# baurst/liso

Hardware: AMD Instinct MI355X
Metric: LISO train-step frames/sec (120k-pt clouds) (higher is better)
Workload: dtype bf16 (detector, BASELINE configs[2]) + f32 via bf16x3 MFMA (SLIM); north_star's 1e-3 on logits / flow is met by `parity_leg` (f32 via bf16x3 MFMA everywhere) and `fp32_exact_leg`, not by the bf16 detector

## Files before the change

include/liso_conv.h:

```cpp
#ifndef LISO_CONV_H
#define LISO_CONV_H

#include <stddef.h>
#include <stdint.h>

#ifdef __cplusplus
extern "C" {
#endif

#define LISO_CONV_MAX_TAPS 49
#define LISO_CONV_MAX_CLASSES 4
#define LISO_CONV_BF16 0
#define LISO_CONV_F32X3 1
#define LISO_CONV_F32 2
#define LISO_CONV_F16 3

#define LISO_ELEM_F32 0
#define LISO_ELEM_BF16 1
#define LISO_ELEM_F16 2

typedef struct {
    int batch, hi, wi, ci;
    int x_pix_stride;
    int ho, wo, co;
    int y_pix_stride, y_ch_off;
    int hv, wv;
    int isy, isx, osy, osx;
    int n_classes;
    int class_tap_begin[LISO_CONV_MAX_CLASSES + 1];
    int class_ooy[LISO_CONV_MAX_CLASSES], class_oox[LISO_CONV_MAX_CLASSES];
    int n_taps;
    int tap_dy[LISO_CONV_MAX_TAPS], tap_dx[LISO_CONV_MAX_TAPS];
    int tap_w[LISO_CONV_MAX_TAPS];
    int w_taps;
    int mode;
    int out_f32;
    int in_relu, out_relu;
    int in_affine_batch_stride;
    int wgrad_co;
} liso_conv_desc;

size_t liso_conv_packed_bytes(int k_channels, int n_channels, int taps, int mode);
int liso_conv_pack_weights(const float* src, int d0, int d1, int kh, int kw, int transposed, int for_dgrad, int mode,
                           void* dst, void* stream);

typedef struct {
    const float* src;
    void* dst;
    int d0, d1, kh, kw, transposed, for_dgrad, mode;
} liso_conv_pack_job;
int liso_conv_pack_weights_batched(const liso_conv_pack_job* jobs, int n_jobs, void* stream);

int liso_conv_stats_rows(const liso_conv_desc* d);

int liso_conv_kernel_kind(const liso_conv_desc* d);

int liso_conv_plan_info(const liso_conv_desc* d, int info[8]);

int liso_conv_forward(const liso_conv_desc* d, const void* x, const void* w_packed, const float* bias,
                      const float* in_scale, const float* in_shift, void* y, float* stats_partial,
                      const float* stats_shift, void* stream);

int liso_conv_forward_sparse(const liso_conv_desc* d, const void* x, const void* w_packed, const float* bias,
                             const float* in_scale, const float* in_shift, void* y, float* stats_partial,
                             const float* stats_shift, const float* occupancy, void* stream);

size_t liso_conv_wgrad_sparse_workspace_bytes(const liso_conv_desc* d);
int liso_conv_wgrad_sparse_f32(const liso_conv_desc* d, const float* x, const float* occupancy, const float* dy, int dy_pix_stride,
                               float* dw, float* dbias, void* workspace, size_t workspace_bytes, void* stream);

size_t liso_conv_wgrad_smallci_workspace_bytes(int batch, int h, int w, int co, int k);
int liso_conv_wgrad_smallci_f32(const float* x, long x_pix_stride, const float* dy, long dy_pix_stride, int batch, int h, int w, int co,
                                int k, float* dw, float* dbias, void* workspace, size_t workspace_bytes, void* stream);

size_t liso_conv_wgrad_workspace_bytes(const liso_conv_desc* d);
int liso_conv_wgrad(const liso_conv_desc* d, const void* x, const float* in_scale, const float* in_shift, const void* dy,
                    int dy_pix_stride, int transposed, float* dw, float* dbias, void* workspace, size_t workspace_bytes,
                    void* stream);

int liso_conv_bn_finalize(const float* stats_partial, int rows, int co, int co_pad, long n, const float* stats_shift,
                          const float* gamma, const float* beta, float* running_mean, float* running_var, float momentum,
                          float eps, float* stats, void* stream);

int liso_conv_in_finalize(const float* stats_partial, int rows_per_sample, int batch, int co, int co_pad, long n_per_sample,
                          const float* gamma, const float* beta, float eps, float* stats, void* stream);

int liso_residual_affine_relu_f32(const float* a, const float* a_scale, const float* a_shift, int a_stride, int a_relu, const float* b,
                                  const float* b_scale, const float* b_shift, int b_stride, int b_relu, float* out, int batch,
                                  long pixels, int c, void* stream);

#define LISO_CONV_OPT_SHARED_GPU 1
#define LISO_CONV_OPT_ROLES_CUS 2
int liso_conv_set_option(int option, int value);

int liso_sparse_conv_stat_groups(int hi, int wi, int co);
size_t liso_sparse_conv_workspace_bytes(int batch, int hi, int wi, int k, int co, int max_cells_per_sample, int for_dgrad);
int liso_sparse_conv_forward(const void* x, long x_pix_stride, int is_bf16, const float* occupancy, const void* w_packed,
                             const float* bias, int batch, int hi, int wi, int k, int co, int max_cells_per_sample, int relu, void* y,
                             float* stats_partial, const float* stats_shift, int* overflow, void* workspace, size_t workspace_bytes,
                             void* stream);
int liso_sparse_conv_dgrad(const void* dy, long dy_pix_stride, int is_bf16, const float* occupancy, const void* w_packed_dgrad, int batch,
                           int hi, int wi, int k, int co, int max_cells_per_sample, void* dx, long dx_pix_stride, int* overflow,
                           void* workspace, size_t workspace_bytes, int reuse_lists, void* stream);
size_t liso_sparse_stem_workspace_bytes(int batch, int hi, int wi, int max_cells_per_sample);
int liso_sparse_stem_forward_f32(const float* x, long x_pix_stride, const float* occupancy, const void* w_packed, const float* bias,
                                 int batch, int hi, int wi, int max_cells_per_sample, int relu, float* y, float* stats_partial,
                                 int* overflow, void* workspace, size_t workspace_bytes, void* stream);

#ifdef __cplusplus
}
#endif
#endif
```

liso_amd/_lib.py:

```python
import ctypes
import os

import torch

_HERE = os.path.dirname(os.path.abspath(__file__))
LIB_PATH = os.path.join(_HERE, "libliso_hip.so")

_lib = None


class LisoHipError(RuntimeError):
    pass


_ERRORS = {-1: "LISO_EINVAL (bad pointer/size)", -2: "LISO_EWORKSPACE (workspace too small)",
           -3: "LISO_ELAUNCH (HIP launch failed)"}


def _preload_torch_hip_runtime():
    tl = os.path.join(os.path.dirname(torch.__file__), "lib", "libamdhip64.so")
    if os.path.exists(tl):
        ctypes.CDLL(tl, mode=ctypes.RTLD_GLOBAL)


# ... 60 lines not shown

    def rows_view(t):
        assert t.dtype == torch.float32 and t.is_cuda
        if t.dim() == 1:
            assert t.stride(0) == 1 or t.numel() <= 1
            return 1, t.numel(), t.numel()
        inner = 1
        for k in range(t.dim() - 1, 0, -1):
            assert t.shape[k] == 1 or t.stride(k) == inner, (tuple(t.shape), t.stride())
            inner *= t.shape[k]
        return t.shape[0], inner, (t.stride(0) if t.shape[0] > 1 else inner)

    for i, (d, s_) in enumerate(jobs):
        assert tuple(d.shape) == tuple(s_.shape), (tuple(d.shape), tuple(s_.shape))
        r, c, dstr = rows_view(d)
        r2, c2, sstr = rows_view(s_)
        assert (r, c) == (r2, c2)
        dst[i], src[i], rows[i], rb[i], ds[i], ss[i] = d.data_ptr(), s_.data_ptr(), r, 4 * c, 4 * dstr, 4 * sstr
    with torch.cuda.device(jobs[0][0].device):
        check(lib().liso_multi_copy_rows(n, dst, src, rows, rb, ds, ss, stream_ptr()), "multi_copy_rows")


def require_cuda(*tensors):
    for t in tensors:
        if not t.is_cuda:
            raise LisoHipError("device op called with a CPU tensor; liso_amd has no CPU fallback")


_vp, _i, _f, _sz, _lg = ctypes.c_void_p, ctypes.c_int, ctypes.c_float, ctypes.c_size_t, ctypes.c_long

SIGNATURES = {
    "liso_iou3d_overlap_bev_f32": (_i, [_vp, _i, _vp, _i, _vp, _vp]),
    "liso_iou3d_iou_bev_f32": (_i, [_vp, _i, _vp, _i, _vp, _vp]),
    "liso_iou3d_nms_workspace_bytes": (_sz, [_i]),
    "liso_iou3d_nms_f32": (_i, [_vp, _i, _f, _vp, _vp, _vp, _sz, _vp]),
    "liso_iou3d_nms_normal_f32": (_i, [_vp, _i, _f, _vp, _vp, _vp, _sz, _vp]),
    "liso_iou3d_iou_bev_cpu_f32": (_i, [_vp, _i, _vp, _i, _vp]),
    "liso_pillars_voxelize_workspace_bytes": (_sz, [_vp, _i, _i]),
    "liso_pillars_voxelize_f32": (_i, [_vp, _vp, _i, _vp, _vp, _vp, _vp, _vp, _vp, _vp, _sz, _vp]),
    "liso_pfn_partials_bytes": (_sz, []),
    "liso_pfn_decorate_workspace_bytes": (_sz, [_i, _i]),
    "liso_pfn_decorate_f32": (_i, [_vp, _vp, _i, _vp, _vp, _vp, _vp, _vp, _vp, _vp, _vp, _sz, _vp]),
    "liso_pfn_bn_prepare_f32": (_i, [_vp, _vp, _vp, _i, _vp, _vp, _vp, _vp, _vp, _vp, _f, _f, _i, _vp, _vp, _vp, _vp]),
    "liso_pfn_forward_scatter": (_i, [_vp, _vp, _vp, _vp, _i, _vp, _vp, _vp, _vp, _i, _vp, _vp]),
    "liso_pfn_backward": (_i, [_vp, _vp, _vp, _vp, _i, _vp, _vp, _vp, _vp, _vp, _i, _vp, _i, _vp, _vp, _vp, _vp, _vp]),
    "liso_kabsch_workspace_bytes": (_sz, [_vp]),
    "liso_kabsch_trafos_f32": (_i, [_vp, _vp, _vp, _vp, _vp, _vp, _vp, _vp, _vp, _vp, _vp, _sz, _vp]),
    "liso_kabsch_trafos_counted_f32": (_i, [_vp, _vp, _vp, _vp, _vp, _vp, _vp, _vp, _vp, _vp, _vp, _vp, _sz, _vp]),
    "liso_symm_ortho_fwd_f64": (_i, [_vp, _i, _vp, _vp, _vp, _vp, _vp]),
    "liso_symm_ortho_bwd_f64": (_i, [_vp, _vp, _vp, _vp, _i, _vp, _vp]),
    "liso_weighted_moments_workspace_bytes": (_sz, [_i]),
    "liso_weighted_moments_fwd_f32": (_i, [_vp, _vp, _vp, _i, ctypes.c_long, _vp, _vp, _sz, _vp]),
    "liso_weighted_moments_bwd_f32": (_i, [_vp, _vp, _vp, _i, ctypes.c_long, _vp, _vp, _vp, _vp, _vp]),
    "liso_bev_dynamic_flow_workspace_bytes": (_sz, [_i, _i, _i]),
    "liso_bev_dynamic_flow_f32": (_i, [_vp, _i, _vp, _vp, _vp, _i, _vp, _i, _i, _i, _i, _vp, _vp, _vp, _sz, _vp]),
    "liso_odom_inverse_minus_eye_f64": (_i, [_vp, _i, _vp, _vp]),
    "liso_fit_box_z_workspace_bytes": (_sz, [_i, _i]),
    "liso_fit_box_z_f32": (_i, [_vp, _i, _i, _vp, _i, _vp, _i, _vp, _i, _f, _vp, _vp, _vp, _vp, _sz, _vp]),
    "liso_dbscan_components": (_i, [_vp, _vp, _vp, _vp, _vp, _vp, _vp, _vp, _vp]),
    "liso_dbscan_labels": (_i, [_vp, _vp, _vp, _vp, _vp, _vp, _vp, _vp, _vp, _vp]),
    "liso_region_props": (_i, [_vp, _i, _i, _i, _i, _vp, _vp, _vp]),
    "liso_region_props_workspace_bytes": (_sz, [_i, _i, _i, _i]),
    "liso_region_props_ws": (_i, [_vp, _i, _i, _i, _i, _vp, _vp, _vp, _sz, _vp]),
    "liso_corr_lookup_fwd_f32": (_i, [_vp, _vp, _vp, _vp, _vp, _vp]),
    "liso_corr_lookup_fwd_tiled_f32": (_i, [_vp, _vp, _vp, _vp, _vp, _vp]),
    "liso_corr_lookup_bwd_dvol_f32": (_i, [_vp, _vp, _vp, _vp, _vp]),
    "liso_corr_pyramid_fwd_f32": (_i, [_vp, _vp, _vp, _vp]),
    "liso_corr_pyramid_bwd_f32": (_i, [_vp, _vp, _vp, _vp]),
    "liso_corr_bwd_features_workspace_bytes": (_sz, [_vp]),
    "liso_corr_bwd_features_f32": (_i, [_vp, _i, _vp, _vp, _vp, _vp, _vp, _vp, _sz, _vp]),
    "liso_rows_combine_f32": (_i, [_lg, _i, _vp, _lg, _vp, _lg, _vp, _lg, _vp, _lg, _vp, _lg, _i, _vp]),
    "liso_gru_out_rows_train_f32": (_i, [_lg, _i, _vp, _lg, _vp, _vp, _lg, _vp, _lg, _vp]),
    "liso_gru_out_rows_bwd_f32": (_i, [_lg, _i, _vp, _lg, _vp, _vp, _lg, _vp, _lg, _vp, _lg, _vp, _vp, _vp]),
    "liso_gru_in_rows_bwd_f32": (_i, [_lg, _i, _vp, _lg, _vp, _lg, _vp, _vp, _vp, _lg, _vp, _lg, _vp, _vp]),
    "liso_raft_state_step_train_f32": (_i, [_i, _i, _vp, _vp, _vp, _vp, _vp, _vp, _vp, _vp, _vp]),
    "liso_raft_pack_output_grads_f32": (_i, [_lg, _i, _vp, _vp, _vp, _vp]),
    "liso_nearest_point_loss_fwd_f32": (_i, [_vp] * 8),
    "liso_nearest_point_loss_bwd_f32": (_i, [_vp] * 9),
    "liso_slim_decode_weights_fwd": (_i, [_vp] * 6 + [_i] + [_vp] * 4),
    "liso_slim_decode_weights_bwd": (_i, [_vp] * 9),
    "liso_slim_decode_points_fwd": (_i, [_vp] * 9),
    "liso_slim_decode_points_bwd": (_i, [_vp] * 11),
    "liso_slim_loss_workspace_bytes": (_sz, []),
    "liso_slim_static_points_loss_fwd": (_i, [_i, ctypes.c_long, _vp, _i, _vp, _vp, _vp, _vp, _vp, _vp, _sz, _vp]),
    "liso_slim_static_points_loss_bwd": (_i, [_i, ctypes.c_long, _vp, _i, _vp, _vp, _vp, _vp, _vp, _vp, _vp, _vp, _vp]),
    "liso_slim_knn_queries": (_i, [_i, _i, ctypes.c_long, _i, _vp, _i, _vp, _vp, _vp, _vp, _vp]),
    "liso_slim_nearest_point_loss_fwd": (_i, [_vp, _vp, _i, _vp, _vp, _vp, _i, _vp, _vp, _vp, _vp, _vp, _sz, _vp]),
    "liso_slim_nearest_point_loss_bwd": (_i, [_vp, _vp, _i, _vp, _vp, _vp, _i, _vp, _vp, _vp, _vp, _vp, _vp, _vp]),
    "liso_bev_gather_fwd_f32": (_i, [_vp, _vp, ctypes.c_long, _i, ctypes.c_float, _vp, _vp]),
    "liso_bev_gather_bwd_f32": (_i, [_vp, _vp, _vp, _vp, ctypes.c_long, _i, _vp, _vp, _vp]),
    "liso_gru_in_fwd_f32": (_i, [_vp, _vp, _vp, ctypes.c_long, _vp, _vp, _vp, _vp, _vp]),
    "liso_gru_in_bwd_f32": (_i, [_vp, _vp, ctypes.c_long, _vp, _vp, _vp, _vp, _vp, _vp, ctypes.c_long, _vp, _vp]),
    "liso_gru_out_fwd_f32": (_i, [ctypes.c_long, _vp, _vp, _vp, _vp, _vp]),
    "liso_gru_out_bwd_f32": (_i, [ctypes.c_long, _vp, _vp, _vp, _vp, _vp, _vp, _vp, _vp]),
    "liso_gru_in_rows_f32": (_i, [ctypes.c_long, _i, _vp, ctypes.c_long, _vp, ctypes.c_long, _vp, _vp, ctypes.c_long, _vp]),
    "liso_gru_out_rows_f32": (_i, [ctypes.c_long, _i, _vp, ctypes.c_long, _vp, _vp, ctypes.c_long, _vp]),
    "liso_multi_copy": (_i, [_i, _vp, _vp, _vp, _vp]),
    "liso_bev_lin_index": (_i, [_vp, _i, _vp, _i, ctypes.c_long, _i, _i, _vp, _vp]),
    "liso_channel_extrema_workspace_bytes": (_sz, []),
    "liso_channel_extrema_f32": (_i, [_vp, ctypes.c_long, _i, _i, _vp, _vp, _sz, _vp]),
    "liso_bev_plan_tile_lin": (_i, [_vp, _i, ctypes.c_long, _i, _i, _i, _i, _vp, _vp]),
    "liso_bev_plan_rank": (_i, [_vp, _vp, ctypes.c_long, _vp, _vp, _vp]),
    "liso_bev_plan_expand": (_i, [_vp, _vp, _vp, _i, ctypes.c_long, _i, _i, _i, _i, _vp, _vp, _vp, _vp]),
    "liso_raft_state_step_f32": (_i, [_i, _i, _vp, ctypes.c_long, _vp, _vp, _vp, _vp]),
    "liso_raft_upsample_scratch_bytes": (_sz, [_vp]),
    "liso_raft_upsample_outputs_fwd_f32": (_i, [_vp] * 5),
    "liso_raft_upsample_outputs_bwd_f32": (_i, [_vp, _vp, _vp, _sz, _vp, _vp, _vp]),
    "liso_centerloss_workspace_bytes": (_sz, [_vp]),
    "liso_centerloss_fwd_f32": (_i, [_vp] * 17 + [_sz, _vp]),
    "liso_centerloss_bwd_f32": (_i, [_vp] * 21),
    "liso_render_center_targets_f32": (_i, [_vp] * 12),
    "liso_conv_pack_weights_batched": (_i, [_vp, _i, _vp]),
    "liso_conv_in_finalize": (_i, [_vp, _i, _i, _i, _i, ctypes.c_long, _vp, _vp, _f, _vp, _vp]),
    "liso_residual_affine_relu_f32": (_i, [_vp, _vp, _vp, _i, _i, _vp, _vp, _vp, _i, _i, _vp, _i, ctypes.c_long, _i, _vp]),
    "liso_scan_workspace_bytes": (_sz, [_i, ctypes.c_long]),
    "liso_scan_inclusive_i32": (_i, [_vp, _i, ctypes.c_long, _vp, _vp, _sz, _vp]),
    "liso_mine_boxes_from_regions": (_i, [_vp, _i, _i, _vp, _i, _vp, _i, _f, _f, _vp, _vp, _vp, _vp, _vp, _vp]),
    "liso_mine_filter_compact": (_i, [_vp] * 21),
    "liso_mine_box_motion": (_i, [_vp, _i, _i, _vp, _vp, _vp, _vp]),
    "liso_mine_nms_workspace_bytes": (_sz, [_i, _i]),
    "liso_mine_nms_prepare": (_i, [_i, _i, _i] + [_vp] * 11 + [_sz, _vp]),
    "liso_mine_nms_finish": (_i, [_i, _i, _i] + [_vp] * 16),
    "liso_adamw_step_f32": (_i, [_vp, _vp, _vp, _vp, _sz] + [ctypes.c_double] * 5 + [ctypes.c_long, _vp]),
    "liso_adamw_step_scaled_f32": (_i, [_vp, _vp, _vp, _vp, _sz] + [ctypes.c_double] * 6 + [ctypes.c_long, _vp]),
    "liso_grad_nonfinite_f32": (_i, [_vp, _sz, _vp, _vp]),
    "liso_adamw_step_amp_f32": (_i, [_vp, _vp, _vp, _vp, _sz] + [ctypes.c_double] * 6 + [_vp, _vp]),
    "liso_loss_scale_update": (_i, [_vp, ctypes.c_double, ctypes.c_double, _i, _vp]),
    "liso_rmsprop_step_f32": (_i, [_vp, _vp, _vp, _sz] + [ctypes.c_double] * 4 + [_vp]),
    "liso_multi_copy_rows": (_i, [_i, _vp, _vp, _vp, _vp, _vp, _vp, _vp]),
    "liso_gather_f32": (_i, [_i, _vp, _vp, _vp, _vp]),
    "liso_bn_workspace_bytes": (_sz, [_i]),
    "liso_bn_relu_fwd": (_i, [_vp, _i, ctypes.c_long, _i, _vp, _vp, _vp, _vp, _f, _f, _i, _i, _vp, _vp, _vp, _sz, _vp]),
    "liso_in_workspace_bytes": (_sz, [_i, _i]),
    "liso_in_relu_fwd": (_i, [_vp, _i, _i, ctypes.c_long, _i, _vp, _vp, _f, _i, _vp, _vp, _vp, _sz, _vp]),
    "liso_in_relu_bwd": (_i, [_vp, _vp, _i, _i, ctypes.c_long, _i, _vp, _vp, _i, _vp, _vp, _vp, _vp, _sz, _vp]),
    "liso_in_relu_bwd_sum": (_i, [_vp, _vp, _i, _i, ctypes.c_long, _i, _vp, _vp, _i, _vp, _vp, _vp, _vp, _sz, _vp]),
    "liso_bn_relu_bwd": (_i, [_vp, _vp, _i, ctypes.c_long, _i, _vp, _vp, _i, _i, _vp, _vp, _vp, _vp, _sz, _vp]),
    "liso_bn_relu_bwd_strided": (_i, [_vp, ctypes.c_long, _vp, ctypes.c_long, _i, ctypes.c_long, _i, _vp, _vp, _i, _i, _vp, ctypes.c_long, _vp, _vp, _vp, _sz, _vp]),
    "liso_bn_relu_bwd_ticket": (_i, [_vp, _vp, _i, ctypes.c_long, _i, _vp, _vp, _i, _i, _vp, _vp, _vp, _vp, _sz, _vp, _vp]),
    "liso_knn_workspace_bytes": (_sz, [_vp, _i]),
    "liso_knn_build_f32": (_i, [_vp, _vp, _i, _i, _vp, _sz, _vp]),
    "liso_knn_sorted_ids": (_i, [_vp, _vp, _i, _vp, _vp]),
    "liso_knn_query_f32": (_i, [_vp, _vp, _vp, _vp, _i, _vp, _i, _i, _vp, _vp, _i, _vp]),
    "liso_conv_packed_bytes": (_sz, [_i, _i, _i, _i]),
    "liso_conv_pack_weights": (_i, [_vp, _i, _i, _i, _i, _i, _i, _i, _vp, _vp]),
    "liso_conv_stats_rows": (_i, [_vp]),
    "liso_conv_kernel_kind": (_i, [_vp]),
    "liso_conv_forward": (_i, [_vp] * 10),
    "liso_conv_set_option": (_i, [_i, _i]),
    "liso_conv_forward_sparse": (_i, [_vp] * 11),
    "liso_conv_plan_info": (_i, [_vp, _vp]),
    "liso_conv_wgrad_workspace_bytes": (_sz, [_vp]),
    "liso_conv_wgrad": (_i, [_vp, _vp, _vp, _vp, _vp, _i, _i, _vp, _vp, _vp, _sz, _vp]),
    "liso_conv_wgrad_sparse_workspace_bytes": (_sz, [_vp]),
    "liso_conv_wgrad_sparse_f32": (_i, [_vp, _vp, _vp, _vp, _i, _vp, _vp, _vp, _sz, _vp]),
    "liso_conv_wgrad_smallci_workspace_bytes": (_sz, [_i, _i, _i, _i, _i]),
    "liso_conv_wgrad_smallci_f32": (_i, [_vp, ctypes.c_long, _vp, ctypes.c_long, _i, _i, _i, _i, _i, _vp, _vp, _vp, _sz, _vp]),
    "liso_sparse_conv_stat_groups": (_i, [_i, _i, _i]),
    "liso_sparse_conv_workspace_bytes": (_sz, [_i, _i, _i, _i, _i, _i, _i]),
    "liso_sparse_conv_forward": (_i, [_vp, ctypes.c_long, _i, _vp, _vp, _vp, _i, _i, _i, _i, _i, _i, _i, _vp, _vp, _vp, _vp, _vp, _sz, _vp]),
    "liso_sparse_conv_dgrad": (_i, [_vp, ctypes.c_long, _i, _vp, _vp, _i, _i, _i, _i, _i, _i, _vp, ctypes.c_long, _vp, _vp, _sz, _i, _vp]),
    "liso_sparse_stem_workspace_bytes": (_sz, [_i, _i, _i, _i]),
    "liso_sparse_stem_forward_f32": (_i, [_vp, ctypes.c_long, _vp, _vp, _vp, _i, _i, _i, _i, _i, _vp, _vp, _vp, _vp, _sz, _vp]),
    "liso_conv_bn_finalize": (_i, [_vp, _i, _i, _i, ctypes.c_long, _vp, _vp, _vp, _vp, _vp, _f, _f, _vp, _vp]),
    "liso_points_in_boxes_workspace_bytes": (_sz, [_vp]),
    "liso_points_in_boxes_f32": (_i, [_vp] * 9 + [_sz, _vp]),
    "liso_match_greedy_f32": (_i, [_vp, ctypes.c_long, ctypes.c_long, _i, _i, _vp, _f, _vp, _vp, _vp, _vp, _vp, _vp, _vp]),
    "liso_fit_boxes_closeness_workspace_bytes": (_sz, [ctypes.c_long, _i]),
    "liso_fit_boxes_closeness_f32": (_i, [_vp, ctypes.c_long, _i, _vp, _vp, _i, _f, _vp, _vp, _vp, _sz, _vp]),
    "liso_bike_rollout_fwd_f32": (_i, [_i, _i, _vp, _vp, _vp, _vp, _f, _f, _f, _vp, _vp]),
    "liso_bike_rollout_bwd_f32": (_i, [_i, _i, _vp, _vp, _vp, _f, _f, _f, _vp, _vp, _vp, _vp, _vp, _vp]),
    "liso_smooth_tracks_jerk_f32": (_i, [_vp, _vp, _i, _i, _i, _f, _f, _vp, _vp]),
    "liso_flow_metrics_state_bytes": (_sz, []),
    "liso_flow_metrics_result_bytes": (_sz, []),
    "liso_flow_metrics_reset": (_i, [_vp, _vp]),
    "liso_flow_metrics_update": (_i, [_vp, _lg, _vp, _lg, _vp, _lg, _i, _vp, _lg, _vp, _lg, _vp, _lg, _vp, _vp, _vp, _vp, _i, _vp, _vp]),
    "liso_flow_metrics_read": (_i, [_vp, _vp, _vp]),
    "liso_bev_free_mask_workspace_bytes": (_sz, [_i, _i]),
    "liso_bev_free_mask": (_i, [_vp, ctypes.c_long, _i, _i, _i, _vp, _vp, _vp, _sz, _vp]),
    "liso_bev_select_free_cells": (_i, [_vp, _vp, _i, _i, _vp, _i, _vp, _vp]),
    "liso_snippet_paste": (_i, [_vp, ctypes.c_long, _vp, _vp, _vp, _vp, ctypes.c_double, ctypes.c_double, _i, _vp, _vp, _vp, _vp]),
}


CONV_MAX_TAPS, CONV_MAX_CLASSES, CONV_BF16, CONV_F32X3, CONV_F32, CONV_F16 = 49, 4, 0, 1, 2, 3
ELEM_F32, ELEM_BF16, ELEM_F16 = 0, 1, 2
_ELEM_CODES = {torch.float32: ELEM_F32, torch.bfloat16: ELEM_BF16, torch.float16: ELEM_F16}
LOSS_SCALE_STATE_BYTES = 32


def elem_code(dtype):
    code = _ELEM_CODES.get(dtype)
    if code is None:
        raise TypeError(f"no device kernel takes {dtype} tensors (float32, bfloat16 or float16)")
    return code


def is_half(dtype):
    return elem_code(dtype) != ELEM_F32
CONV_OPT_SHARED_GPU = 1
CONV_OPT_ROLES_CUS = 2


class ConvDesc(ctypes.Structure):
    _fields_ = [("batch", _i), ("hi", _i), ("wi", _i), ("ci", _i), ("x_pix_stride", _i), ("ho", _i), ("wo", _i), ("co", _i),
                ("y_pix_stride", _i), ("y_ch_off", _i), ("hv", _i), ("wv", _i), ("isy", _i), ("isx", _i), ("osy", _i), ("osx", _i),
                ("n_classes", _i), ("class_tap_begin", _i * (CONV_MAX_CLASSES + 1)), ("class_ooy", _i * CONV_MAX_CLASSES),
                ("class_oox", _i * CONV_MAX_CLASSES), ("n_taps", _i), ("tap_dy", _i * CONV_MAX_TAPS), ("tap_dx", _i * CONV_MAX_TAPS),
                ("tap_w", _i * CONV_MAX_TAPS), ("w_taps", _i), ("mode", _i), ("out_f32", _i), ("in_relu", _i), ("out_relu", _i),
                ("in_affine_batch_stride", _i), ("wgrad_co", _i)]


class ConvPackJob(ctypes.Structure):
    _fields_ = [("src", _vp), ("dst", _vp), ("d0", _i), ("d1", _i), ("kh", _i), ("kw", _i), ("transposed", _i), ("for_dgrad", _i),
                ("mode", _i)]


class KnnGrid(ctypes.Structure):
    _fields_ = [("x_min", _f), ("y_min", _f), ("cell", _f), ("nx", _i), ("ny", _i), ("z_min", _f), ("z_cell", _f), ("nz", _i)]


class CenterLossCfg(ctypes.Structure):
    _fields_ = [("batch", _i), ("h", _i), ("w", _i), ("res_x", _f), ("res_y", _f), ("z_min", _f), ("z_max", _f),
                ("sup_weight", _f), ("rot_reg_weight", _f)]


class NpLossCfg(ctypes.Structure):
    _fields_ = [("batch", _i), ("n", ctypes.c_long), ("n_b", ctypes.c_long), ("ext", _f * 4), ("fov_mode", _i), ("delta", _f)]


class SlimDecodeCfg(ctypes.Structure):
    _fields_ = [("samples", _i), ("n", ctypes.c_long), ("h", _i), ("w", _i), ("logit_mode", _i * 4), ("static_flow_zero", _i),
                ("dynamic_flow_zero", _i), ("overwrite_flow", _i), ("overwrite_logits", _i), ("non_rigid", _i), ("use_static_aggr", _i),
                ("dyn_grad_scale", _f), ("ext_lo", ctypes.c_double * 2), ("ext_span", ctypes.c_double * 2)]


class SlimDecodeOut(ctypes.Structure):
    FIELDS = ("dis_logit", "dis", "logits", "probs", "staticness", "dynamicness", "groundness", "dyn_flow", "stat_flow", "agg_flow", "saf_flow")
    _fields_ = [(k, _vp) for k in FIELDS] + [("flags", _vp)]


class SlimNpLossCfg(ctypes.Structure):
    _fields_ = [("samples", _i), ("clouds", _i), ("n", ctypes.c_long), ("n_b", ctypes.c_long), ("ext", _f * 4), ("fov_mode", _i), ("delta", _f)]


class BoxPtsCfg(ctypes.Structure):
    _fields_ = [("batch", _i), ("n", ctypes.c_long), ("k", _i), ("point_stride", _i), ("precision", _i), ("dims_bloat", _f)]


class GruCfg(ctypes.Structure):
    _fields_ = [("batch", _i), ("ch", _i), ("cx", _i), ("hw", ctypes.c_long)]


class UpsampleCfg(ctypes.Structure):
    _fields_ = [("n_it", _i), ("batch2", _i), ("dirs", _i), ("h", _i), ("w", _i), ("factor", _i), ("flow_scale", _f)]


class MineFilterCfg(ctypes.Structure):
    _fields_ = [("batch", _i), ("k", _i), ("min_points", _i), ("aspect_ratio_max", ctypes.c_double), ("max_box_len_m", ctypes.c_double),
                ("min_box_area_m2", ctypes.c_double), ("min_box_volume_m3", ctypes.c_double), ("park_invalid", _i)]


class TargetsCfg(ctypes.Structure):
    _fields_ = [("batch", _i), ("n_boxes", _i), ("h", _i), ("w", _i), ("range_x", _f), ("range_y", _f)]


class DbscanCfg(ctypes.Structure):
    _fields_ = [("batch", _i), ("gx", _i), ("gy", _i), ("window", _i), ("min_samples", _i), ("eps", _f), ("flow_weight", _f)]


class CorrCfg(ctypes.Structure):
    _fields_ = [("batch", _i), ("h", _i), ("w", _i), ("dim", _i), ("levels", _i), ("radius", _i)]


class KabschCfg(ctypes.Structure):
    _fields_ = [("batch", _i), ("n_points", _i), ("n_slots", _i), ("point_stride", _i), ("flow_stride", _i),
                ("slope", _f), ("scale_fg", _f), ("scale_bg", _f), ("softness", _i)]


class PillarCfg(ctypes.Structure):
    _fields_ = [("x_min", _f), ("y_min", _f), ("z_min", _f), ("vx", _f), ("vy", _f), ("vz", _f), ("gx", _i),
                ("gy", _i), ("max_points", _i), ("max_voxels", _i), ("n_channels", _i)]


class _Everything:
    def __contains__(self, name):
        return True


class KernelTimer:

    def __init__(self):
        self.enabled = set()
        self.events = {}
        self.units = {}
        self.bytes = {}
        self.weights = {}
        self.weight = 1.0

    def enable(self, name):
        self.enabled.add(name)
        self.events.setdefault(name, [])

    def enable_all(self):
        self.enabled = _Everything()

    def disable_all(self):
        self.enabled = set()

    def launch(self, name, fn, units=None, nbytes=None):
        if name not in self.enabled:
            return fn()
        a, b = torch.cuda.Event(enable_timing=True), torch.cuda.Event(enable_timing=True)
        a.record()
        r = fn()
        b.record()
        self.events.setdefault(name, []).append((a, b))
        self.weights.setdefault(name, []).append(float(self.weight))
        if units is not None:
            self.units.setdefault(name, []).append(units)
        if nbytes is not None:
            self.bytes.setdefault(name, []).append(nbytes)
        return r

    def mean_units(self, name):
        u = self.units.get(name, [])
        return sum(u) / len(u) if u else None

    def durations_ms(self, name):
        torch.cuda.synchronize()
        return [a.elapsed_time(b) for a, b in self.events.get(name, [])]

    def weighted_total_ms(self, name):
        return sum(d * w for d, w in zip(self.durations_ms(name), self.weights.get(name, [])))

    def reset(self):
        for k in self.events:
            self.events[k] = []
        self.units = {}
        self.bytes = {}
        self.weights = {}


TIMER = KernelTimer()


def _declare(l):
    for name, (res, args) in SIGNATURES.items():
        fn = getattr(l, name)
        fn.restype = res
        fn.argtypes = args
```

liso_amd/csrc/conv_wgrad.hip:

```cpp
#include <hip/hip_runtime.h>
#include <stdint.h>
#include <stdlib.h>

#include "../../include/liso_conv.h"
#include "../../include/liso_iou3d.h"
#include "elem16.h"
#include "per_device.h"

namespace {

typedef __bf16 bf8 __attribute__((ext_vector_type(8)));
typedef float f16v __attribute__((ext_vector_type(16)));
typedef short s4 __attribute__((ext_vector_type(4)));
typedef s4 __attribute__((address_space(3))) * lds_s4_ptr;

constexpr int kThreads = 256;
constexpr int TW = 32;
constexpr int CT = 64;
constexpr int PSB = CT * 2 + 64;
constexpr int PS32 = CT * 4 + 16;

struct WgArgs {
    const void* x;
    const float* in_scale;
    const float* in_shift;
    const void* dy;
    float* slab;
    float* bias_slab;
    int dy_pix_stride;
    int ci_t, co_t;
    int n_groups;
    int grp_cls[LISO_CONV_MAX_TAPS], grp_begin[LISO_CONV_MAX_TAPS], grp_cnt[LISO_CONV_MAX_TAPS];
    int cls_dy0[LISO_CONV_MAX_CLASSES], cls_dx0[LISO_CONV_MAX_CLASSES];
    int cls_inh[LISO_CONV_MAX_CLASSES], cls_inw[LISO_CONV_MAX_CLASSES];
    int tiles_x, tiles_y, n_tiles, splits;
    int x_plane_bytes;
    int psx;
    int th;
    int ci_w;
    int pipelined;
    int compact;
#ifdef LISO_WGRAD_STAMPS
    unsigned long long* stamps;
#endif
};

__device__ __forceinline__ unsigned pack_bf16(float a, float b) {
    const __bf16 x = (__bf16)a, y = (__bf16)b;
    return (unsigned)__builtin_bit_cast(unsigned short, x) | ((unsigned)__builtin_bit_cast(unsigned short, y) << 16);
}
__device__ __forceinline__ float bf16_lo(unsigned w) { return __uint_as_float(w << 16); }
__device__ __forceinline__ float bf16_hi(unsigned w) { return __uint_as_float(w & 0xffff0000u); }
__device__ __forceinline__ float round_bf16(float v) { return (float)(__bf16)v; }

__device__ __forceinline__ bf8 tr_pair(const unsigned char* p0, const unsigned char* p1) {
    const s4 a = __builtin_amdgcn_ds_read_tr16_b64_v4i16((lds_s4_ptr)p0);
    const s4 b = __builtin_amdgcn_ds_read_tr16_b64_v4i16((lds_s4_ptr)p1);
    typedef short s8 __attribute__((ext_vector_type(8)));
    const s8 v = {a[0], a[1], a[2], a[3], b[0], b[1], b[2], b[3]};
    return __builtin_bit_cast(bf8, v);
}

template <int MODE, int TG>
__global__ __launch_bounds__(kThreads, 2) void conv_wgrad_kernel(const liso_conv_desc d, const WgArgs a) {
    using E = typename liso_e16::Elem<MODE>::T;
    constexpr bool X3 = MODE == LISO_CONV_F32X3;
    constexpr bool F32 = MODE == LISO_CONV_F32;
    constexpr bool FIN = X3 || F32;
    constexpr int PLANES = X3 ? 2 : 1;
    constexpr int PSYM = F32 ? PS32 : PSB;
    constexpr int PSY = PSB;
    constexpr int XB = TG >= 9 ? 4 : 8;
    extern __shared__ __attribute__((aligned(16))) unsigned char smem[];
    const int tid = threadIdx.x, wave = tid >> 6, lane = tid & 63;
    int t = blockIdx.x;
    const int split = t % a.splits;
    t /= a.splits;
    const int cot = t % a.co_t;
    t /= a.co_t;
    const int cit = t % a.ci_t;
    const int grp = t / a.ci_t;
    const int cls = a.grp_cls[grp], tb = a.grp_begin[grp], tcnt = a.grp_cnt[grp];
    const int dy0 = a.cls_dy0[cls], dx0 = a.cls_dx0[cls], in_h = a.cls_inh[cls], in_w = a.cls_inw[cls];
    const int PSX = a.psx;
    const int npix = in_h * in_w;
    const float inv_w = 1.0f / (float)in_w;
    const int ooy = d.class_ooy[cls], oox = d.class_oox[cls];
    const int ci0 = cit * CT, co0 = cot * CT;

    unsigned char* xs = smem;
    unsigned char* ys = smem + a.x_plane_bytes * PLANES;
    const int TH = a.th, MPIX = TH * TW;
    const int y_plane = MPIX * PSYM;

    const int g = lane >> 4, q = (lane & 15) >> 2, p = lane & 3;
    const int ci_half = wave >> 1, co_half = wave & 1;
    const int a_lane = (8 * (g >> 1) + q) * d.isx * PSX + (ci_half * 32 + 16 * (g & 1) + 4 * p) * 2;
    const int b_lane = (8 * (g >> 1) + q) * PSY + (co_half * 32 + 16 * (g & 1) + 4 * p) * 2;

    f16v acc[TG];
#pragma unroll
    for (int i = 0; i < TG; i++)
#pragma unroll
        for (int e = 0; e < 16; e++) acc[i][e] = 0.0f;
    float bsum[8];
#pragma unroll
    for (int e = 0; e < 8; e++) bsum[e] = 0.0f;
    const bool want_bias = a.bias_slab != nullptr && cit == 0 && tb == d.class_tap_begin[cls];

    const int gdy = a.compact ? d.tap_dy[tb] - dy0 : 0;
    const int row_mul = a.compact ? d.isy : 1;
    const int row_step = a.compact ? 1 : d.isy;
    int toff[TG];
#pragma unroll
    for (int i = 0; i < TG; i++) {
        const int tp = tb + (i < tcnt ? i : 0);
        toff[i] = ((d.tap_dy[tp] - dy0 - gdy) * in_w + (d.tap_dx[tp] - dx0)) * PSX;
    }

    constexpr int YB = 4;
    const int c8 = tid & 7, p0 = tid >> 3, pstep = kThreads / 8;
    uint4 xv[XB], yv[YB];
    unsigned xok = 0u, yok = 0u;
    float sc[8], sh[8];
    const bool pro = !FIN && a.in_scale != nullptr;
    if constexpr (!FIN) {
        const int ch = ci0 + c8 * 8;
        if (pro) {
#pragma unroll
            for (int e = 0; e < 8; e++) {
                sc[e] = ch < d.ci ? a.in_scale[ch + e] : 0.0f;
                sh[e] = ch < d.ci ? a.in_shift[ch + e] : 0.0f;
            }
        }
    }
    auto tile_origin = [&](int tile, int& b, int& ty, int& tx) {
        tx = tile % a.tiles_x;
        tile /= a.tiles_x;
        ty = tile % a.tiles_y;
        b = tile / a.tiles_y;
    };
    auto load_x = [&](int tile, int pix_begin) {
        int b, ty, tx;
        tile_origin(tile, b, ty, tx);
        const int iy0 = ty * TH * d.isy + dy0, ix0 = tx * TW * d.isx + dx0;
        const int ch = ci0 + c8 * 8;
        const bool ch_ok = ch < d.ci;
        const unsigned short* xg = (const unsigned short*)a.x + (long)b * d.hi * d.wi * d.x_pix_stride;
        const int pfirst = pix_begin + p0;
        int ly = (int)(((float)pfirst + 0.5f) * inv_w);
        int lx = pfirst - ly * in_w;
        const int step_y = pstep / in_w, step_x = pstep - step_y * in_w;
        xok = 0u;
#pragma unroll
        for (int u = 0; u < XB; u++) {
// ... 152 lines not shown
    } else
    for (int tile = split; tile < a.n_tiles; tile += a.splits) {
        int tt = tile;
        const int tx = tt % a.tiles_x;
        tt /= a.tiles_x;
        const int ty = tt % a.tiles_y;
        const int b = tt / a.tiles_y;
        const int iy0 = ty * TH * d.isy + dy0, ix0 = tx * TW * d.isx + dx0;
        const long x_img = (long)b * d.hi * d.wi;
        const long y_img = (long)b * d.ho * d.wo * a.dy_pix_stride;
        __syncthreads();
        if constexpr (!FIN) {
            (void)iy0; (void)ix0; (void)x_img; (void)y_img;
            for (int pix0 = 0; pix0 < npix; pix0 += XB * pstep) {
                load_x(tile, pix0);
                store_x(pix0);
            }
            load_y(tile);
            store_y();
        } else {
            const int c4 = tid & 15, p0 = tid >> 4, pstep = kThreads / 16;
            const int ch = ci0 + c4 * 4;
            const bool ch_ok = ch < d.ci;
            const bool pro = a.in_scale != nullptr;
            float sc[4], sh[4];
            if (pro) {
#pragma unroll
                for (int e = 0; e < 4; e++) {
                    sc[e] = ch_ok ? a.in_scale[ch + e] : 0.0f;
                    sh[e] = ch_ok ? a.in_shift[ch + e] : 0.0f;
                }
            }
            const float* xg = (const float*)a.x + x_img * d.x_pix_stride;
            unsigned char* xs_lo = xs + a.x_plane_bytes;
            int ly = (int)(((float)p0 + 0.5f) * inv_w);
            int lx = p0 - ly * in_w;
            const int step_y = pstep / in_w, step_x = pstep - step_y * in_w;
            for (int pix0 = p0; pix0 < npix; pix0 += XB * pstep) {
                float4 v[XB];
                bool ok[XB];
#pragma unroll
                for (int u = 0; u < XB; u++) {
                    const int pix = pix0 + u * pstep;
                    const int iy = iy0 + gdy + ly * row_mul, ix = ix0 + lx;
                    ok[u] = pix < npix && ch_ok && (unsigned)iy < (unsigned)d.hi && (unsigned)ix < (unsigned)d.wi;
                    const int off = ok[u] ? (iy * d.wi + ix) * d.x_pix_stride + ch : 0;
                    lx += step_x;
                    ly += step_y;
                    if (lx >= in_w) {
                        lx -= in_w;
                        ly++;
                    }
                    v[u] = *reinterpret_cast<const float4*>(xg + off);
                }
#pragma unroll
                for (int u = 0; u < XB; u++) {
                    const int pix = pix0 + u * pstep;
                    if (pix >= npix) continue;
                    float f[4] = {v[u].x, v[u].y, v[u].z, v[u].w};
                    unsigned hi2[2], lo2[2];
#pragma unroll
                    for (int e = 0; e < 4; e++) {
                        if (pro) {
                            f[e] = fmaf(f[e], sc[e], sh[e]);
                            if (d.in_relu) f[e] = fmaxf(f[e], 0.0f);
                        }
                        if (!ok[u]) f[e] = 0.0f;
                    }
                    if constexpr (F32) {
                        *reinterpret_cast<float4*>(xs + pix * PSX + c4 * 16) = make_float4(f[0], f[1], f[2], f[3]);
                        continue;
                    }
#pragma unroll
                    for (int e = 0; e < 2; e++) {
                        const float h0 = round_bf16(f[2 * e]), h1 = round_bf16(f[2 * e + 1]);
                        hi2[e] = pack_bf16(h0, h1);
                        lo2[e] = pack_bf16(f[2 * e] - h0, f[2 * e + 1] - h1);
                    }
                    *reinterpret_cast<uint2*>(xs + pix * PSX + c4 * 8) = make_uint2(hi2[0], hi2[1]);
                    *reinterpret_cast<uint2*>(xs_lo + pix * PSX + c4 * 8) = make_uint2(lo2[0], lo2[1]);
                }
            }
            const float* yg = (const float*)a.dy;
            const int chy = co0 + c4 * 4;
            const bool chy_ok = chy < d.co;
            for (int u = 0; u < MPIX / (kThreads / 16); u++) {
                const int m = p0 + u * pstep;
                const int vy = ty * TH + (m >> 5), vx = tx * TW + (m & 31);
                const int oy = vy * d.osy + ooy, ox = vx * d.osx + oox;
                const bool ok = chy_ok && vy < d.hv && vx < d.wv && oy < d.ho && ox < d.wo;
                const int off = ok ? (oy * d.wo + ox) * a.dy_pix_stride + chy : 0;
                float4 v = *reinterpret_cast<const float4*>(yg + y_img + off);
                float f[4] = {v.x, v.y, v.z, v.w};
                unsigned hi2[2], lo2[2];
#pragma unroll
                for (int e = 0; e < 4; e++) {
                    if (!ok) f[e] = 0.0f;
                    if (want_bias) bsum[e] += f[e];
                }
                if constexpr (F32) {
                    *reinterpret_cast<float4*>(ys + m * PS32 + c4 * 16) = make_float4(f[0], f[1], f[2], f[3]);
                    continue;
                }
#pragma unroll
                for (int e = 0; e < 2; e++) {
                    const float h0 = round_bf16(f[2 * e]), h1 = round_bf16(f[2 * e + 1]);
                    hi2[e] = pack_bf16(h0, h1);
                    lo2[e] = pack_bf16(f[2 * e] - h0, f[2 * e + 1] - h1);
                }
                *reinterpret_cast<uint2*>(ys + m * PSY + c4 * 8) = make_uint2(hi2[0], hi2[1]);
                *reinterpret_cast<uint2*>(ys + y_plane + m * PSY + c4 * 8) = make_uint2(lo2[0], lo2[1]);
            }
        }
        __syncthreads();
        mfma_tile();
    }
    const int r = lane & 31, h = lane >> 5;
    const long cip = (long)a.ci_t * CT, cop = (long)a.co_t * CT;
#pragma unroll
    for (int i = 0; i < TG; i++) {
        if (i < tcnt) {
            const int wt = d.tap_w[tb + i];
            float* base = a.slab + (((long)split * d.w_taps + wt) * cip + ci0 + ci_half * 32) * cop + co0 + co_half * 32 + r;
            if (co0 + co_half * 32 + r < (d.wgrad_co > 0 ? d.wgrad_co : d.co)) {
                const int rows_left = d.ci - (ci0 + ci_half * 32);
#pragma unroll
                for (int e = 0; e < 16; e++) {
                    const int row = (e & 3) + 8 * (e >> 2) + 4 * h;
                    if (row < rows_left) base[(long)row * cop] = acc[i][e];
                }
            }
        }
    }
    if (want_bias) {
        __syncthreads();
        float* red = reinterpret_cast<float*>(smem);
        constexpr int NCH = FIN ? 4 : 8;
        constexpr int NGR = FIN ? 16 : 8;
#pragma unroll
        for (int e = 0; e < NCH; e++) red[tid * NCH + e] = bsum[e];
        __syncthreads();
        if (tid < CT) {
            const int grp_c = tid / NCH, e = tid % NCH;
            float s = 0.0f;
            for (int pp = 0; pp < kThreads / NGR; pp++) s += red[(pp * NGR + grp_c) * NCH + e];
            a.bias_slab[((long)cls * a.splits + split) * cop + co0 + tid] = s;
        }
    }
}

constexpr int kRsThreads = 512;
constexpr int RPS = 128;

template <int MODE, int TH, int S, int CIW>
__global__ __launch_bounds__(kRsThreads, 1) void conv_wgrad_rs3_kernel(const liso_conv_desc d, const WgArgs a) {
    using E = typename liso_e16::Elem<MODE>::T;
    constexpr bool X3 = MODE == LISO_CONV_F32X3;
    constexpr int PLANES = X3 ? 2 : 1;
    constexpr int IW = (TW - 1) * S + 3, IH = (TH - 1) * S + 3;
    constexpr int NPX = IH * IW;
    constexpr int NSLOT = (NPX + 3) / 4 * 4;
    constexpr int CPP = X3 ? 16 : 8;
    constexpr int PSL = 256 / CPP;
    constexpr int CPPX = CPP * CIW / 64;
    constexpr int PSLX = 256 / CPPX;
    constexpr int XB = (NPX + PSLX - 1) / PSLX;
    constexpr int YB = TH * TW / PSL;
    constexpr int X_PLANE = NSLOT * RPS, Y_PLANE = TH * TW * RPS;
    constexpr int X_BYTES = PLANES * X_PLANE;
    constexpr int BUF = X_BYTES + PLANES * Y_PLANE;
    constexpr int NE = X3 ? 4 : 8;
    extern __shared__ __attribute__((aligned(16))) unsigned char smem[];
    const int tid = threadIdx.x, wave = tid >> 6, lane = tid & 63;
    int t = blockIdx.x;
    const int split = t % a.splits;
    t /= a.splits;
    const int cot = t % a.co_t;
    const int cit = t / a.co_t;
    const int ci0 = cit * CIW, co0 = cot * CT;
    const long cip = (long)a.ci_t * CIW, cop = (long)a.co_t * CT;
    const int n_mine = split < a.n_tiles ? (a.n_tiles - split + a.splits - 1) / a.splits : 0;

    if (wave >= 4) {
        const int ltid = tid - 256;
        const int cc = ltid % CPP, p0 = ltid / CPP;
        const int ccx = ltid % CPPX, p0x = ltid / CPPX;
        uint4 xv[XB], yv[YB];
        unsigned xok = 0u, yok = 0u;
        float sc[NE], sh[NE];
        float bsum[NE];
#pragma unroll
        for (int e = 0; e < NE; e++) bsum[e] = 0.0f;
        const bool want_bias = a.bias_slab != nullptr && cit == 0;
        const bool pro = a.in_scale != nullptr;
        const int ch = ci0 + ccx * NE, chy = co0 + cc * NE;
        const bool ch_ok = ch < d.ci, chy_ok = chy < d.co;
        if (pro) {
#pragma unroll
            for (int e = 0; e < NE; e++) {
                sc[e] = ch_ok ? a.in_scale[ch + e] : 0.0f;
                sh[e] = ch_ok ? a.in_shift[ch + e] : 0.0f;
            }
        }
        int rel[XB];
        unsigned lyx[XB];
#pragma unroll
        for (int u = 0; u < XB; u++) {
            const int pix = p0x + u * PSLX;
            const int ly = pix / IW, lx = pix - ly * IW;
            rel[u] = (ly * d.wi + lx) * d.x_pix_stride;
            lyx[u] = (unsigned)ly | ((unsigned)lx << 8) | (pix < NPX && ch_ok ? 0x10000u : 0u);
        }
        auto load_tile = [&](int tile) {
            const int tx = tile % a.tiles_x;
            const int tq = tile / a.tiles_x;
            const int ty = tq % a.tiles_y, b = tq / a.tiles_y;
            const int iy0 = ty * TH * S - 1, ix0 = tx * TW * S - 1;
            const long xbase = (long)b * d.hi * d.wi * d.x_pix_stride + ch;
            const int org = (iy0 * d.wi + ix0) * d.x_pix_stride;
            const bool inner = iy0 >= 0 && iy0 + IH <= d.hi && ix0 >= 0 && ix0 + IW <= d.wi;
            xok = 0u;
#pragma unroll
            for (int u = 0; u < XB; u++) {
                bool ok = (lyx[u] >> 16) != 0u;
                if (!inner) {
                    const int iy = iy0 + (int)(lyx[u] & 0xffu), ix = ix0 + (int)((lyx[u] >> 8) & 0xffu);
                    ok = ok && (unsigned)iy < (unsigned)d.hi && (unsigned)ix < (unsigned)d.wi;
                }
                xok |= ok ? (1u << u) : 0u;
                const long off = xbase + (ok ? org + rel[u] : 0);
                if constexpr (X3)
                    xv[u] = *reinterpret_cast<const uint4*>((const float*)a.x + off);
                else
                    xv[u] = *reinterpret_cast<const uint4*>((const unsigned short*)a.x + off);
            }
            const long ybase = (long)b * d.ho * d.wo * a.dy_pix_stride + chy;
            yok = 0u;
#pragma unroll
            for (int u = 0; u < YB; u++) {
                const int m = p0 + u * PSL;
                const int oy = ty * TH + (m >> 5), ox = tx * TW + (m & 31);
                const bool ok = chy_ok && oy < d.ho && ox < d.wo;
                yok |= ok ? (1u << u) : 0u;
                const long off = ybase + (ok ? (long)(oy * d.wo + ox) * a.dy_pix_stride : 0);
                if constexpr (X3)
                    yv[u] = *reinterpret_cast<const uint4*>((const float*)a.dy + off);
                else
                    yv[u] = *reinterpret_cast<const uint4*>((const unsigned short*)a.dy + off);
            }
        };
        auto store_tile = [&](unsigned char* buf) {
            unsigned char* xs = buf;
            unsigned char* ys = buf + X_BYTES;
#pragma unroll
            for (int u = 0; u < XB; u++) {
                const int pix = p0x + u * PSLX;
                if (pix >= NPX) continue;
                const int swz = S == 1 ? ((pix >> 1) & 1) << 6 : ((pix >> 2) & 1) << 6;
                const int slot = S == 1 ? pix : pix ^ ((pix >> 1) & 1);
                if constexpr (X3) {
                    float f[4] = {__uint_as_float(xv[u].x), __uint_as_float(xv[u].y), __uint_as_float(xv[u].z), __uint_as_float(xv[u].w)};
                    unsigned hi2[2], lo2[2];
#pragma unroll
                    for (int e = 0; e < 4; e++) {
                        if (pro) {
                            f[e] = fmaf(f[e], sc[e], sh[e]);
                            if (d.in_relu) f[e] = fmaxf(f[e], 0.0f);
                        }
                        if (!((xok >> u) & 1u)) f[e] = 0.0f;
                    }
#pragma unroll
                    for (int e = 0; e < 2; e++) {
                        const float h0 = round_bf16(f[2 * e]), h1 = round_bf16(f[2 * e + 1]);
                        hi2[e] = pack_bf16(h0, h1);
                        lo2[e] = pack_bf16(f[2 * e] - h0, f[2 * e + 1] - h1);
                    }
                    *reinterpret_cast<uint2*>(xs + slot * RPS + ((ccx * 8) ^ swz)) = make_uint2(hi2[0], hi2[1]);
                    *reinterpret_cast<uint2*>(xs + X_PLANE + slot * RPS + ((ccx * 8) ^ swz)) = make_uint2(lo2[0], lo2[1]);
                } else {
                    uint4 o = xv[u];
                    if (pro) {
                        unsigned w[4] = {o.x, o.y, o.z, o.w};
#pragma unroll
                        for (int e = 0; e < 4; e++) {
                            float f0 = fmaf(E::lo(w[e]), sc[2 * e], sh[2 * e]);
                            float f1 = fmaf(E::hi(w[e]), sc[2 * e + 1], sh[2 * e + 1]);
                            if (d.in_relu) {
                                f0 = fmaxf(f0, 0.0f);
                                f1 = fmaxf(f1, 0.0f);
                            }
                            w[e] = E::pack(f0, f1);
                        }
                        o = make_uint4(w[0], w[1], w[2], w[3]);
                    }
                    if (!((xok >> u) & 1u)) o = make_uint4(0u, 0u, 0u, 0u);
                    *reinterpret_cast<uint4*>(xs + slot * RPS + ((ccx * 16) ^ swz)) = o;
                }
            }
#pragma unroll
            for (int u = 0; u < YB; u++) {
                const int m = p0 + u * PSL;
                const int swz = ((m >> 1) & 1) << 6;
                uint4 v = yv[u];
                if (!((yok >> u) & 1u)) v = make_uint4(0u, 0u, 0u, 0u);
                if constexpr (X3) {
                    const float f[4] = {__uint_as_float(v.x), __uint_as_float(v.y), __uint_as_float(v.z), __uint_as_float(v.w)};
                    unsigned hi2[2], lo2[2];
#pragma unroll
                    for (int e = 0; e < 2; e++) {
                        const float h0 = round_bf16(f[2 * e]), h1 = round_bf16(f[2 * e + 1]);
                        hi2[e] = pack_bf16(h0, h1);
                        lo2[e] = pack_bf16(f[2 * e] - h0, f[2 * e + 1] - h1);
                    }
                    *reinterpret_cast<uint2*>(ys + m * RPS + ((cc * 8) ^ swz)) = make_uint2(hi2[0], hi2[1]);
                    *reinterpret_cast<uint2*>(ys + Y_PLANE + m * RPS + ((cc * 8) ^ swz)) = make_uint2(lo2[0], lo2[1]);
                    if (want_bias) {
#pragma unroll
                        for (int e = 0; e < 4; e++) bsum[e] += f[e];
                    }
                } else {
                    *reinterpret_cast<uint4*>(ys + m * RPS + ((cc * 16) ^ swz)) = v;
                    if (want_bias) {
                        const unsigned w[4] = {v.x, v.y, v.z, v.w};
#pragma unroll
                        for (int e = 0; e < 4; e++) {
                            bsum[2 * e] += E::lo(w[e]);
                            bsum[2 * e + 1] += E::hi(w[e]);
                        }
                    }
                }
            }
        };
#ifdef LISO_WGRAD_STAMPS
        unsigned long long ws_store = 0, ws_load = 0, ws_bar = 0, ws_t;
        const unsigned long long ws_k0 = __builtin_amdgcn_s_memtime();
#define WSTAMP_BEGIN ws_t = __builtin_amdgcn_s_memtime();
#define WSTAMP_END(acc) { const unsigned long long ws_n = __builtin_amdgcn_s_memtime(); acc += ws_n - ws_t; ws_t = ws_n; }
#else
#define WSTAMP_BEGIN
#define WSTAMP_END(acc)
#endif
        if (n_mine > 0) {
            load_tile(split);
            store_tile(smem);
            if (n_mine > 1) load_tile(split + a.splits);
        }
        __syncthreads();
#ifdef LISO_WGRAD_STAMPS
        const unsigned long long ws_k1 = __builtin_amdgcn_s_memtime();
#endif
        for (int k = 0; k < n_mine; k++) {
            WSTAMP_BEGIN
            if (k + 1 < n_mine) {
                store_tile(smem + ((k + 1) & 1) * BUF);
                WSTAMP_END(ws_store)
                if (k + 2 < n_mine) load_tile(split + (k + 2) * a.splits);
                WSTAMP_END(ws_load)
            }
            __syncthreads();
            WSTAMP_END(ws_bar)
        }
#ifdef LISO_WGRAD_STAMPS
        if (ltid == 0 && a.stamps) {
            unsigned long long* o = a.stamps + (size_t)blockIdx.x * 16 + 8;
            o[0] = ws_k1 - ws_k0; o[1] = ws_store; o[2] = ws_load; o[3] = ws_bar; o[4] = (unsigned long long)n_mine;
        }
#endif
        if (want_bias) {
            float* red = reinterpret_cast<float*>(smem);
#pragma unroll
            for (int e = 0; e < NE; e++) red[ltid * NE + e] = bsum[e];
        }
        __syncthreads();
        if (want_bias && ltid < CT) {
            const float* red = reinterpret_cast<const float*>(smem);
            const int grp_c = ltid / NE, e = ltid % NE;
            float s_ = 0.0f;
            for (int pp = 0; pp < PSL; pp++) s_ += red[(pp * CPP + grp_c) * NE + e];
            a.bias_slab[(long)split * cop + co0 + ltid] = s_;
        }
        if constexpr (CIW == 32) __syncthreads();
        return;
    }
    const int g = lane >> 4, q = (lane & 15) >> 2, p = lane & 3;
    const int ci_half = CIW == 64 ? wave >> 1 : 0, co_half = wave & 1;
    const int c_lo = CIW == 64 ? 0 : wave >> 1, c_hi = CIW == 64 ? 2 : (wave >> 1) + 1;
    constexpr int NAL = S == 1 ? 4 : 8;
    int a_lane[NAL];
#pragma unroll
    for (int m = 0; m < NAL; m++) {
        const int off = S * (8 * (g >> 1) + q), pm = m + S * q;
        const int slot_off = S == 1 ? off : (off + ((pm ^ ((pm >> 1) & 1)) - pm));
        const int swz = S == 1 ? ((pm >> 1) & 1) << 6 : ((pm >> 2) & 1) << 6;
        a_lane[m] = slot_off * RPS + ((ci_half * 64 + 32 * (g & 1) + 8 * p) ^ swz);
    }
    const int b_lane = (8 * (g >> 1) + q) * RPS + ((co_half * 64 + 32 * (g & 1) + 8 * p) ^ (((q >> 1) & 1) << 6));

    f16v acc[9];
#pragma unroll
    for (int i = 0; i < 9; i++)
#pragma unroll
        for (int e = 0; e < 16; e++) acc[i][e] = 0.0f;

    auto mma = [&](int i, const bf8& ah, const bf8& al, const bf8& bh, const bf8& bl) {
        if constexpr (X3) {
            acc[i] = __builtin_amdgcn_mfma_f32_32x32x16_bf16(al, bh, acc[i], 0, 0, 0);
            acc[i] = __builtin_amdgcn_mfma_f32_32x32x16_bf16(ah, bl, acc[i], 0, 0, 0);
        }
        acc[i] = E::mfma(ah, bh, acc[i]);
    };

#ifdef LISO_WGRAD_STAMPS
    unsigned long long ms_mul = 0, ms_bar = 0, ms_t;
    const unsigned long long ms_k0 = __builtin_amdgcn_s_memtime();
#endif
    __syncthreads();
#ifdef LISO_WGRAD_STAMPS
    const unsigned long long ms_k1 = __builtin_amdgcn_s_memtime();
    ms_t = ms_k1;
#endif
    for (int k = 0; k < n_mine; k++) {
        const unsigned char* xs = smem + (k & 1) * BUF;
        const unsigned char* ys = xs + X_BYTES;
#pragma unroll
        for (int c = c_lo; c < c_hi; c++) {
            bf8 bf[3], bl[3];
#pragma unroll
            for (int r = 0; r < IH; r++) {
                bf8 af[3], al[3];
#pragma unroll
                for (int kx = 0; kx < 3; kx++) {
                    const int base = r * IW + 16 * S * c + kx;
                    const unsigned char* ap = xs + base * RPS + a_lane[base & (NAL - 1)];
                    af[kx] = tr_pair(ap, ap + 4 * S * RPS);
                    if constexpr (X3) al[kx] = tr_pair(ap + X_PLANE, ap + X_PLANE + 4 * S * RPS);
                }
                if ((S == 1 && r < TH) || (S == 2 && (r & 1) == 0 && r / 2 < TH)) {
                    const int o = r / S;
                    const unsigned char* bp = ys + (o * TW + 16 * c) * RPS + b_lane;
                    bf[o % 3] = tr_pair(bp, bp + 4 * RPS);
                    if constexpr (X3) bl[o % 3] = tr_pair(bp + Y_PLANE, bp + Y_PLANE + 4 * RPS);
                }
#pragma unroll
                for (int ky = 0; ky < 3; ky++) {
                    if ((r - ky) % S != 0) continue;
                    const int o = (r - ky) / S;
                    if (r - ky >= 0 && o < TH) {
#pragma unroll
                        for (int kx = 0; kx < 3; kx++) mma(ky * 3 + kx, af[kx], al[kx], bf[o % 3], bl[o % 3]);
                    }
                }
            }
        }
#ifdef LISO_WGRAD_STAMPS
        { const unsigned long long n_ = __builtin_amdgcn_s_memtime(); ms_mul += n_ - ms_t; ms_t = n_; }
#endif
        __syncthreads();
#ifdef LISO_WGRAD_STAMPS
        { const unsigned long long n_ = __builtin_amdgcn_s_memtime(); ms_bar += n_ - ms_t; ms_t = n_; }
#endif
    }
    __syncthreads();
#ifdef LISO_WGRAD_STAMPS
    const unsigned long long ms_k2 = __builtin_amdgcn_s_memtime();
#endif
    if constexpr (CIW == 32) {
        float* hand = reinterpret_cast<float*>(smem + 8192) + (size_t)(wave & 1) * 9 * 16 * 64;
        if (wave >= 2) {
#pragma unroll
            for (int i = 0; i < 9; i++)
#pragma unroll
                for (int e = 0; e < 16; e++) hand[(i * 16 + e) * 64 + lane] = acc[i][e];
        }
        __syncthreads();
        if (wave >= 2) return;
#pragma unroll
        for (int i = 0; i < 9; i++)
#pragma unroll
            for (int e = 0; e < 16; e++) acc[i][e] += hand[(i * 16 + e) * 64 + lane];
    }
    const int r = lane & 31, h = lane >> 5;
#pragma unroll
    for (int i = 0; i < 9; i++) {
        const int wt = d.tap_w[i];
        float* base = a.slab + (((long)split * d.w_taps + wt) * cip + ci0 + ci_half * 32) * cop + co0 + co_half * 32 + r;
        if (co0 + co_half * 32 + r < (d.wgrad_co > 0 ? d.wgrad_co : d.co)) {
            const int rows_left = d.ci - (ci0 + ci_half * 32);
#pragma unroll
            for (int e = 0; e < 16; e++) {
                const int row = (e & 3) + 8 * (e >> 2) + 4 * h;
                if (row < rows_left) base[(long)row * cop] = acc[i][e];
            }
        }
    }
#ifdef LISO_WGRAD_STAMPS
    __builtin_amdgcn_s_waitcnt(0x0F70);
    if (tid == 0 && a.stamps) {
        unsigned long long* o = a.stamps + (size_t)blockIdx.x * 16;
        const unsigned long long ms_k3 = __builtin_amdgcn_s_memtime();
        o[0] = ms_k1 - ms_k0; o[1] = ms_mul; o[2] = ms_bar; o[3] = ms_k2 - ms_k0; o[4] = ms_k3 - ms_k2; o[5] = ms_k3 - ms_k0;
    }
#endif
}

template <int PARTS>
__global__ __launch_bounds__(256) void wgrad_reduce_kernel(const float* __restrict__ slab, const float* __restrict__ bias_slab,
                                                           int splits, int bias_rows, int taps, int ci, int co, long cip, long cop,
                                                           int transposed, float* __restrict__ dw, float* __restrict__ dbias) {
    constexpr int RPB = 16 / PARTS;
    __shared__ float4 red[16][16];
    const int c4 = threadIdx.x & 15, part = PARTS == 16 ? threadIdx.x >> 4 : 0, rib = PARTS == 16 ? 0 : threadIdx.x >> 4;
    const int n_tiles = (co + 63) / 64;
    const long rows = (long)taps * ci;
    const long row_blocks = (rows + RPB - 1) / RPB;
    const long bid = blockIdx.x;
    const bool is_bias = bid >= row_blocks * n_tiles;
    if (is_bias && !dbias) return;
    const int ntile = (int)(is_bias ? bid - row_blocks * n_tiles : bid % n_tiles);
    const long row = is_bias ? 0 : (bid / n_tiles) * RPB + rib;
    const bool row_ok = is_bias ? rib == 0 : row < rows;
    const int k = (int)(row % ci), tap = (int)(row / ci);
    const int n = ntile * 64 + c4 * 4;
    const int count = is_bias ? bias_rows : splits;
    const float* src = is_bias ? bias_slab + n : slab + ((long)tap * cip + k) * cop + n;
    const long stride = is_bias ? cop : (long)taps * cip * cop;
    float4 s = make_float4(0.0f, 0.0f, 0.0f, 0.0f);
    if (n < co && row_ok) {
        int sp = part;
        for (; sp + 3 * PARTS < count; sp += 4 * PARTS) {
            const float4 v0 = *reinterpret_cast<const float4*>(src + (long)sp * stride);
            const float4 v1 = *reinterpret_cast<const float4*>(src + (long)(sp + PARTS) * stride);
            const float4 v2 = *reinterpret_cast<const float4*>(src + (long)(sp + 2 * PARTS) * stride);
            const float4 v3 = *reinterpret_cast<const float4*>(src + (long)(sp + 3 * PARTS) * stride);
            s.x = (((s.x + v0.x) + v1.x) + v2.x) + v3.x;
            s.y = (((s.y + v0.y) + v1.y) + v2.y) + v3.y;
            s.z = (((s.z + v0.z) + v1.z) + v2.z) + v3.z;
            s.w = (((s.w + v0.w) + v1.w) + v2.w) + v3.w;
        }
        for (; sp < count; sp += PARTS) {
            const float4 v = *reinterpret_cast<const float4*>(src + (long)sp * stride);
            s.x += v.x; s.y += v.y; s.z += v.z; s.w += v.w;
        }
    }
    if constexpr (PARTS == 16) {
        red[part][c4] = s;
        __syncthreads();
#pragma unroll
        for (int w = 8; w >= 1; w >>= 1) {
            if (part < w) {
                const float4 o = red[part + w][c4];
                s.x += o.x; s.y += o.y; s.z += o.z; s.w += o.w;
                red[part][c4] = s;
            }
            __syncthreads();
        }
    }
    if (part == 0 && n < co && row_ok) {
        const float v[4] = {s.x, s.y, s.z, s.w};
#pragma unroll
        for (int e = 0; e < 4; e++) {
            if (n + e >= co) break;
            if (is_bias)
                dbias[n + e] = v[e];
            else
                dw[transposed ? (((long)k * co + n + e) * taps + tap) : (((long)(n + e) * ci + k) * taps + tap)] = v[e];
        }
    }
}

int launch_reduce(const float* slab, const float* bias_slab, int splits, int bias_rows, int taps, int ci, int co_w, long cip, long cop,
                  int transposed, float* dw, float* dbias, hipStream_t st) {
    const long rows = (long)taps * ci;
    const int n_tiles = (co_w + 63) / 64;
    if (splits > 16) {
        const long blocks = (rows + (dbias ? 1 : 0)) * n_tiles;
        wgrad_reduce_kernel<16><<<(int)blocks, 256, 0, st>>>(slab, bias_slab, splits, bias_rows, taps, ci, co_w, cip, cop, transposed, dw, dbias);
    } else {
        const long blocks = ((rows + 15) / 16 + (dbias ? 1 : 0)) * n_tiles;
        wgrad_reduce_kernel<1><<<(int)blocks, 256, 0, st>>>(slab, bias_slab, splits, bias_rows, taps, ci, co_w, cip, cop, transposed, dw, dbias);
    }
    return hipGetLastError() == hipSuccess ? LISO_OK : LISO_ELAUNCH;
}

int round_up(int v, int m) { return (v + m - 1) / m * m; }

struct WgPlan {
    int tg, lds, splits, blocks;
    size_t slab_bytes, bias_bytes;
    WgArgs a;
};

bool make_plan_impl(const liso_conv_desc& d, WgPlan* p, bool compact) {
    if (d.mode == LISO_CONV_F16) {
        liso_conv_desc e = d;
        e.mode = LISO_CONV_BF16;
        return make_plan_impl(e, p, compact);
    }
    if (d.batch <= 0 || d.ci <= 0 || d.co <= 0 || d.n_classes < 1 || d.n_classes > LISO_CONV_MAX_CLASSES) return false;
    if (d.n_taps < 1 || d.n_taps > LISO_CONV_MAX_TAPS || d.class_tap_begin[0] != 0 || d.class_tap_begin[d.n_classes] != d.n_taps)
        return false;
    if (d.mode != LISO_CONV_BF16 && d.mode != LISO_CONV_F32X3 && d.mode != LISO_CONV_F32) return false;
    const bool f32 = d.mode == LISO_CONV_F32;
    const bool x3 = d.mode == LISO_CONV_F32X3 || f32;
    const int vec = x3 ? 4 : 8;
    if (d.ci % vec || d.co % vec || d.x_pix_stride % vec) return false;
    const int planes = (x3 && !f32) ? 2 : 1;
    const int psx = f32 ? PS32 : PSB, psy = f32 ? PS32 : PSB;
    WgArgs& a = p->a;
    a.ci_t = (d.ci + CT - 1) / CT;
    a.co_t = (d.co + CT - 1) / CT;
    a.tiles_x = (d.wv + TW - 1) / TW;
    int max_cls_taps = 0, TH = 4;
    int th_fit = 0;
    for (int pass = 0; pass < 2 && !th_fit; pass++)
        for (int th = 4; th >= 1 && !th_fit; th >>= 1) {
            int mp = 0;
            for (int c = 0; c < d.n_classes; c++) {
                int y0 = 1 << 30, y1 = -(1 << 30), x0 = 1 << 30, x1 = -(1 << 30);
                for (int t = d.class_tap_begin[c]; t < d.class_tap_begin[c + 1]; t++) {
                    y0 = d.tap_dy[t] < y0 ? d.tap_dy[t] : y0;
                    y1 = d.tap_dy[t] > y1 ? d.tap_dy[t] : y1;
                    x0 = d.tap_dx[t] < x0 ? d.tap_dx[t] : x0;
                    x1 = d.tap_dx[t] > x1 ? d.tap_dx[t] : x1;
                }
                const int np = (compact ? th : (th - 1) * d.isy + (y1 - y0) + 1) * ((TW - 1) * d.isx + (x1 - x0) + 1);
                mp = np > mp ? np : mp;
            }
            const int lds = planes * (round_up(mp * psx, 16) + th * TW * psy);
            if (lds <= (pass == 0 ? 79 : 158) * 1024) th_fit = th;
        }
    if (!th_fit) return false;
    TH = th_fit;
    a.th = TH;
    a.tiles_y = (d.hv + TH - 1) / TH;
    a.n_tiles = d.batch * a.tiles_y * a.tiles_x;
    int max_pix = 0;
    for (int c = 0; c < d.n_classes; c++) {
        int y0 = 1 << 30, y1 = -(1 << 30), x0 = 1 << 30, x1 = -(1 << 30);
        const int nt = d.class_tap_begin[c + 1] - d.class_tap_begin[c];
        if (nt < 1) return false;
        max_cls_taps = nt > max_cls_taps ? nt : max_cls_taps;
        for (int t = d.class_tap_begin[c]; t < d.class_tap_begin[c + 1]; t++) {
            y0 = d.tap_dy[t] < y0 ? d.tap_dy[t] : y0;
            y1 = d.tap_dy[t] > y1 ? d.tap_dy[t] : y1;
            x0 = d.tap_dx[t] < x0 ? d.tap_dx[t] : x0;
            x1 = d.tap_dx[t] > x1 ? d.tap_dx[t] : x1;
            if (d.tap_w[t] < 0 || d.tap_w[t] >= d.w_taps) return false;
        }
        a.cls_dy0[c] = y0;
        a.cls_dx0[c] = x0;
        a.cls_inh[c] = compact ? TH : (TH - 1) * d.isy + (y1 - y0) + 1;
        a.cls_inw[c] = (TW - 1) * d.isx + (x1 - x0) + 1;
        const int np = a.cls_inh[c] * a.cls_inw[c];
        max_pix = np > max_pix ? np : max_pix;
    }
    a.psx = psx;
    a.compact = compact ? 1 : 0;
    a.pipelined = 0;
    a.x_plane_bytes = round_up(max_pix * a.psx, 16);
    p->lds = planes * (a.x_plane_bytes + TH * TW * psy);
    const long cc = (long)a.ci_t * a.co_t;
    auto groups = [&](int tg) {
        int n = 0;
        for (int c = 0; c < d.n_classes; c++) n += (d.class_tap_begin[c + 1] - d.class_tap_begin[c] + tg - 1) / tg;
        return n;
    };
    const long slab_per_split = (long)d.w_taps * a.ci_t * CT * a.co_t * CT * sizeof(float);
    long slab_mb = 24;
    if (const char* e = getenv("LISO_WGRAD_SLAB_MB")) slab_mb = atol(e) > 0 ? atol(e) : slab_mb;
    long split_cap = (slab_mb << 20) / slab_per_split;
    long min_tiles = x3 ? 2 : 4;
    if (const char* e = getenv("LISO_WGRAD_MIN_TILES")) min_tiles = atol(e) > 0 ? atol(e) : min_tiles;
    const long by_tiles = a.n_tiles >= min_tiles ? a.n_tiles / min_tiles : 1;
    split_cap = split_cap < 1 ? 1 : (split_cap > by_tiles ? by_tiles : split_cap);
    long target = 512;
    if (const char* e = getenv("LISO_WGRAD_BLOCKS")) target = atol(e) > 0 ? atol(e) : target;
    const bool rows7 = max_cls_taps == 49 && d.n_classes == 1;
    const int tg_opts[3] = {rows7 ? 7 : 9, rows7 ? 1 : 3, 1};
    long best_blocks = -1;
    p->tg = 1;
    for (int k = ((!rows7 && (x3 || compact)) ? 1 : 0); k < 3; k++) {
        const int tg = tg_opts[k];
        if (tg > 1 && max_cls_taps == 1) continue;
        const long per_split = cc * groups(tg);
        long s = (target + per_split - 1) / per_split;
        s = s < 1 ? 1 : (s > split_cap ? split_cap : s);
        const long blocks = per_split * s;
        if (blocks >= 256 || (rows7 && tg == 7)) {
            p->tg = tg;
            break;
        }
        if (blocks > best_blocks) {
            best_blocks = blocks;
            p->tg = tg;
        }
    }
    if (const char* e = getenv("LISO_WGRAD_TG")) {
        const int v = atoi(e);
        if ((v == 9 && !x3 && !compact && !rows7) || (v == 3 && !rows7) || v == 1 || (v == 7 && rows7)) p->tg = v;
    }
    {
        const int xb = p->tg >= 9 ? 4 : 8;
        a.pipelined = (!x3 && max_pix <= xb * (kThreads / 8)) ? 1 : 0;
        if (const char* e = getenv("LISO_WGRAD_PIPE")) a.pipelined = a.pipelined && atoi(e) != 0;
    }
    a.n_groups = 0;
    for (int c = 0; c < d.n_classes; c++)
        for (int t = d.class_tap_begin[c]; t < d.class_tap_begin[c + 1]; t += p->tg) {
            if (a.n_groups >= LISO_CONV_MAX_TAPS) return false;
            a.grp_cls[a.n_groups] = c;
            a.grp_begin[a.n_groups] = t;
            const int left = d.class_tap_begin[c + 1] - t;
            a.grp_cnt[a.n_groups] = left < p->tg ? left : p->tg;
            if (compact)
                for (int q = 1; q < a.grp_cnt[a.n_groups]; q++)
                    if (d.tap_dy[t + q] != d.tap_dy[t]) return false;
            a.n_groups++;
        }
    const long per_split = cc * a.n_groups;
    long s = (target + per_split - 1) / per_split;
// ... 137 lines not shown
        __syncthreads();
        for (int j = 0; j < ns; j++) {
            const float xv = xs[j][ci];
            const float4 y0 = *reinterpret_cast<const float4*>(&ys[j][co8]), y1 = *reinterpret_cast<const float4*>(&ys[j][co8 + 4]);
            const float4 y2 = *reinterpret_cast<const float4*>(&ys[j][co8 + 8]), y3 = *reinterpret_cast<const float4*>(&ys[j][co8 + 12]);
            acc[0] = fmaf(xv, y0.x, acc[0]); acc[1] = fmaf(xv, y0.y, acc[1]); acc[2] = fmaf(xv, y0.z, acc[2]); acc[3] = fmaf(xv, y0.w, acc[3]);
            acc[4] = fmaf(xv, y1.x, acc[4]); acc[5] = fmaf(xv, y1.y, acc[5]); acc[6] = fmaf(xv, y1.z, acc[6]); acc[7] = fmaf(xv, y1.w, acc[7]);
            acc[8] = fmaf(xv, y2.x, acc[8]); acc[9] = fmaf(xv, y2.y, acc[9]); acc[10] = fmaf(xv, y2.z, acc[10]); acc[11] = fmaf(xv, y2.w, acc[11]);
            acc[12] = fmaf(xv, y3.x, acc[12]); acc[13] = fmaf(xv, y3.y, acc[13]); acc[14] = fmaf(xv, y3.z, acc[14]); acc[15] = fmaf(xv, y3.w, acc[15]);
        }
    }
    if (ci < d.ci) {
        float* o = a.slab + (((long)split * d.w_taps + d.tap_w[tap]) * 64 + ci) * 64 + co8;
#pragma unroll
        for (int e = 0; e < 16; e += 4)
            if (co8 + e < d.co) *reinterpret_cast<float4*>(o + e) = make_float4(acc[e], acc[e + 1], acc[e + 2], acc[e + 3]);
    }
}

__global__ __launch_bounds__(256) void dy_colsum_kernel(const float* __restrict__ dy, long n_pix, int pix_stride, int co, long per_block,
                                                        float* __restrict__ bias_slab) {
    __shared__ float4 red4[256];
    const long p0 = (long)blockIdx.x * per_block, p1 = p0 + per_block < n_pix ? p0 + per_block : n_pix;
    if ((co & 3) == 0 && (pix_stride & 3) == 0 && (((uintptr_t)dy) & 15) == 0) {
        const int lanes = co >> 2, rowsl = 256 / lanes;
        const int c4 = threadIdx.x % lanes, pr = threadIdx.x / lanes;
        float4 acc = make_float4(0.f, 0.f, 0.f, 0.f);
        if (pr < rowsl) {
            long p = p0 + pr;
            for (; p + 3L * rowsl < p1; p += 4L * rowsl) {
                float4 v[4];
#pragma unroll
                for (int u = 0; u < 4; u++) v[u] = *reinterpret_cast<const float4*>(dy + (p + (long)u * rowsl) * pix_stride + c4 * 4);
#pragma unroll
                for (int u = 0; u < 4; u++) { acc.x += v[u].x; acc.y += v[u].y; acc.z += v[u].z; acc.w += v[u].w; }
            }
            for (; p < p1; p += rowsl) {
                const float4 v = *reinterpret_cast<const float4*>(dy + p * pix_stride + c4 * 4);
                acc.x += v.x; acc.y += v.y; acc.z += v.z; acc.w += v.w;
            }
        }
        red4[threadIdx.x] = acc;
        __syncthreads();
        if ((int)threadIdx.x < 64) {
            float s_ = 0.0f;
            if ((int)threadIdx.x < co) {
                const int l = threadIdx.x >> 2, e = threadIdx.x & 3;
                for (int q = 0; q < rowsl; q++) {
                    const float4 v = red4[q * lanes + l];
                    s_ += e == 0 ? v.x : e == 1 ? v.y : e == 2 ? v.z : v.w;
                }
            }
            bias_slab[(long)blockIdx.x * 64 + threadIdx.x] = s_;
        }
        return;
    }
    float* red = reinterpret_cast<float*>(red4);
    const int c = threadIdx.x & 63, part = threadIdx.x >> 6;
    float s = 0.0f;
    if (c < co)
        for (long p = p0 + part; p < p1; p += 4) s += dy[p * pix_stride + c];
    red[part * 64 + c] = s;
    __syncthreads();
    if (part == 0) bias_slab[(long)blockIdx.x * 64 + c] = (red[c] + red[64 + c]) + (red[128 + c] + red[192 + c]);
}

constexpr int kSpBiasRows = 256;

size_t sparse_layout(const liso_conv_desc& d, size_t* off_rowcnt, size_t* off_rowoff, size_t* off_cells, size_t* off_slab, size_t* off_bias) {
    const size_t rows = (size_t)d.batch * d.hi;
    size_t o = 0;
    auto take = [&](size_t bytes) {
        const size_t at = o;
        o += (bytes + 255) / 256 * 256;
        return at;
    };
    *off_rowcnt = take(rows * 4);
    *off_rowoff = take((rows + 1) * 4);
    *off_cells = take(rows * d.wi * 4);
    *off_slab = take((size_t)kSpSplits * d.w_taps * 64 * 64 * 4);
    *off_bias = take((size_t)kSpBiasRows * 64 * 4);
    return o;
}

bool sparse_ok(const liso_conv_desc& d) {
    return d.batch > 0 && d.n_classes == 1 && d.osy == 1 && d.osx == 1 && d.ci <= 64 && d.co <= 64 && d.ci % 4 == 0 && d.co % 4 == 0 &&
           d.x_pix_stride % 4 == 0 && d.n_taps >= 1 && d.n_taps <= LISO_CONV_MAX_TAPS && d.n_taps == d.w_taps &&
           (d.mode == LISO_CONV_F32X3 || d.mode == LISO_CONV_F32) && (long)d.batch * d.hi * d.wi < (1l << 31) &&
           (long)d.batch * d.hi <= 1024l * 64 && d.in_affine_batch_stride == 0;
}

struct Rs3Plan {
    int th, stride, lds, blocks;
    size_t slab_bytes, bias_bytes;
    WgArgs a;
};

bool make_rs3_plan(const liso_conv_desc& d, Rs3Plan* p) {
    if (const char* e = getenv("LISO_WGRAD_RS3"))
        if (atoi(e) == 0) return false;
    if (d.mode == LISO_CONV_F16) {
        liso_conv_desc e = d;
        e.mode = LISO_CONV_BF16;
        return make_rs3_plan(e, p);
    }
    if ((d.mode != LISO_CONV_BF16 && d.mode != LISO_CONV_F32X3) || d.n_classes != 1 || d.n_taps != 9 || d.w_taps != 9) return false;
    const bool x3 = d.mode == LISO_CONV_F32X3;
    const int vec = x3 ? 4 : 8;
    const int S = d.isy;
    if ((S != 1 && S != 2) || d.isx != S || d.osy != 1 || d.osx != 1 || d.in_affine_batch_stride != 0) return false;
    if (S == 2 && (x3 || getenv("LISO_WGRAD_RS3_S2_OFF"))) return false;
    if (d.hv != d.ho || d.wv != d.wo || d.ho != (d.hi - 1) / S + 1 || d.wo != (d.wi - 1) / S + 1 || d.batch <= 0) return false;
    if (d.ci % vec || d.co % vec || d.x_pix_stride % vec || d.class_tap_begin[0] != 0 || d.class_tap_begin[1] != 9) return false;
    for (int t = 0; t < 9; t++)
        if (d.tap_dy[t] != t / 3 - 1 || d.tap_dx[t] != t % 3 - 1 || d.tap_w[t] < 0 || d.tap_w[t] >= 9) return false;
    WgArgs& a = p->a;
    a.ci_w = (S == 1 && d.ci <= 32) ? 32 : CT;
    if (const char* e = getenv("LISO_WGRAD_CIW")) a.ci_w = (atoi(e) == 32 && S == 1) ? 32 : CT;
    a.ci_t = (d.ci + a.ci_w - 1) / a.ci_w;
    a.co_t = (d.co + CT - 1) / CT;
    const long cc = (long)a.ci_t * a.co_t;
    long want = 256 / cc;
    if (const char* e = getenv("LISO_WGRAD_BLOCKS")) want = (atol(e) > 0 ? atol(e) : 256) / cc;
    want = want < 1 ? 1 : want;
    a.tiles_x = (d.wo + TW - 1) / TW;
    const long tiles8 = (long)d.batch * ((d.ho + 7) / 8) * a.tiles_x;
    int th = tiles8 >= 4 * want ? 8 : 4;
    if (const char* e = getenv("LISO_WGRAD_TH")) th = atoi(e) == 8 ? 8 : atoi(e) == 4 ? 4 : th;
    if (x3 || S == 2) th = 3;
    p->stride = S;
    a.th = th;
    a.tiles_y = (d.ho + th - 1) / th;
    a.n_tiles = d.batch * a.tiles_y * a.tiles_x;
    long min_tiles = 4;
    if (const char* e = getenv("LISO_WGRAD_RS3_MIN_TILES")) min_tiles = atol(e) > 0 ? atol(e) : min_tiles;
    long s = a.n_tiles / min_tiles;
    s = s > want ? want : s;
    s = s < 1 ? 1 : s;
    a.splits = (int)s;
    a.n_groups = 1;
    p->th = th;
    p->blocks = (int)(cc * s);
    const int npx = ((th - 1) * S + 3) * ((TW - 1) * S + 3);
    p->lds = 2 * (x3 ? 2 : 1) * ((npx + 3) / 4 * 4 + th * TW) * RPS;
    p->slab_bytes = (size_t)s * 9 * a.ci_t * a.ci_w * a.co_t * CT * sizeof(float);
    p->bias_bytes = (size_t)s * a.co_t * CT * sizeof(float);
    return true;
}

#ifdef LISO_WGRAD_STAMPS
unsigned long long* g_wgrad_stamps = nullptr;
#endif

template <int MODE, int TH, int S, int CIW = 64>
int launch_rs3(const liso_conv_desc& d, const Rs3Plan& p, hipStream_t st) {
    static liso_dev::PerDeviceFlag attr_set;
    if (!liso_dev::lds_opt_in(attr_set, (const void*)conv_wgrad_rs3_kernel<MODE, TH, S, CIW>, 160 * 1024)) return LISO_ELAUNCH;
#ifdef LISO_WGRAD_STAMPS
    if (!g_wgrad_stamps && hipMalloc((void**)&g_wgrad_stamps, 4096 * 16 * 8) != hipSuccess) return LISO_ELAUNCH;
    (void)hipMemsetAsync(g_wgrad_stamps, 0, 4096 * 16 * 8, st);
    Rs3Plan q = p;
    q.a.stamps = p.blocks <= 4096 ? g_wgrad_stamps : nullptr;
    conv_wgrad_rs3_kernel<MODE, TH, S, CIW><<<q.blocks, kRsThreads, q.lds, st>>>(d, q.a);
    return hipGetLastError() == hipSuccess ? LISO_OK : LISO_ELAUNCH;
#endif
    conv_wgrad_rs3_kernel<MODE, TH, S, CIW><<<p.blocks, kRsThreads, p.lds, st>>>(d, p.a);
    return hipGetLastError() == hipSuccess ? LISO_OK : LISO_ELAUNCH;
}

}

constexpr int kSmallCi = 4;

template <int K>
__global__ __launch_bounds__(256) void wgrad_smallci_kernel(const float* __restrict__ x, long xps, const float* __restrict__ dy, long gps,
                                                            int batch, int h, int w, int co, int rows_per_block,
                                                            float* __restrict__ partial, float* __restrict__ bias_partial) {
    extern __shared__ float4 xs[];
    constexpr int P = K / 2;
    const int lane = threadIdx.x & 63, ci = threadIdx.x >> 6;
    const int c = blockIdx.y * 64 + lane;
    const int wp = w + K - 1;
    float* gs = reinterpret_cast<float*>(xs + K * wp);
    float acc[K][K];
#pragma unroll
    for (int a = 0; a < K; a++)
#pragma unroll
        for (int b = 0; b < K; b++) acc[a][b] = 0.f;
    float bsum = 0.f;
    const long rows = (long)batch * h;
    const long r0 = (long)blockIdx.x * rows_per_block, r1 = r0 + rows_per_block < rows ? r0 + rows_per_block : rows;
    const float* xs_f = reinterpret_cast<const float*>(xs);
    for (long r = r0; r < r1; r++) {
        const int b = (int)(r / h), y = (int)(r % h);
        __syncthreads();
        const float* g = dy + (((long)b * h + y) * w) * gps;
        for (int i = threadIdx.x; i < w * 64; i += 256) {
            const int px = i >> 6, cc = blockIdx.y * 64 + (i & 63);
            gs[i] = cc < co ? g[(long)px * gps + cc] : 0.f;
        }
        for (int i = threadIdx.x; i < K * wp; i += 256) {
            const int ky = i / wp, px = i % wp;
            const int yy = y + ky - P, xx = px - P;
            float4 v = make_float4(0.f, 0.f, 0.f, 0.f);
            if (yy >= 0 && yy < h && xx >= 0 && xx < w) v = *reinterpret_cast<const float4*>(x + (((long)b * h + yy) * w + xx) * xps);
            xs[i] = v;
        }
        __syncthreads();
        float win[K][K];
#pragma unroll
        for (int ky = 0; ky < K; ky++)
#pragma unroll
            for (int col = 0; col < K - 1; col++) win[ky][col] = xs_f[(ky * wp + col) * 4 + ci];
        for (int px0 = 0; px0 < w; px0 += K) {
#pragma unroll
            for (int j = 0; j < K; j++) {
                const int col = px0 + j + K - 1;
                const int cc = col < wp ? col : wp - 1;
                const float gv = px0 + j < w ? gs[(px0 + j) * 64 + lane] : 0.f;
#pragma unroll
                for (int ky = 0; ky < K; ky++) win[ky][(j + K - 1) % K] = xs_f[(ky * wp + cc) * 4 + ci];
#pragma unroll
                for (int ky = 0; ky < K; ky++)
#pragma unroll
                    for (int kx = 0; kx < K; kx++) acc[ky][kx] = fmaf(win[ky][(j + kx) % K], gv, acc[ky][kx]);
                bsum += gv;
            }
        }
    }
    const int cop = gridDim.y * 64;
    float* pt = partial + (((size_t)blockIdx.x * kSmallCi + ci) * K * K) * cop + c;
#pragma unroll
    for (int ky = 0; ky < K; ky++)
#pragma unroll
        for (int kx = 0; kx < K; kx++) pt[(size_t)(ky * K + kx) * cop] = acc[ky][kx];
    if (ci == 0 && bias_partial) bias_partial[(size_t)blockIdx.x * cop + c] = bsum;
}

__global__ __launch_bounds__(512) void wgrad_smallci_reduce_kernel(const float* __restrict__ partial, const float* __restrict__ bias_partial,
                                                                   int nblk, int kk, int co, int cop, float* __restrict__ dw,
                                                                   float* __restrict__ db) {
    __shared__ float sm[8][64];
    const int i = blockIdx.x * 64 + threadIdx.x, q = threadIdx.y;
    const int n = kSmallCi * kk * cop;
    const float* src = nullptr;
    size_t stride = 0;
    if (i < n) { src = partial + i; stride = (size_t)n; }
    else if (bias_partial && i - n < cop) { src = bias_partial + (i - n); stride = (size_t)cop; }
    float s = 0.f;
    if (src) {
        int b = q;
        for (; b + 56 < nblk; b += 64) {
            float v[8];
#pragma unroll
            for (int u = 0; u < 8; u++) v[u] = src[(size_t)(b + 8 * u) * stride];
#pragma unroll
            for (int u = 0; u < 8; u++) s += v[u];
        }
        for (; b < nblk; b += 8) s += src[(size_t)b * stride];
    }
    sm[q][threadIdx.x] = s;
    __syncthreads();
    if (q != 0 || !src) return;
    s = 0.f;
#pragma unroll
    for (int u = 0; u < 8; u++) s += sm[u][threadIdx.x];
    if (i < n) {
        const int c = i % cop, t = (i / cop) % kk, ci = i / (cop * kk);
        if (c < co) dw[((size_t)c * kSmallCi + ci) * kk + t] = s;
    } else if (db && i - n < co) {
        db[i - n] = s;
    }
}

inline bool smallci_layout(int batch, int h, int w, int co, int k, int* nblk, int* rpb, size_t* part_bytes, size_t* bias_bytes, int* lds) {
    if (batch < 1 || h < 1 || w < 1 || co < 1 || co > 1024 || (k != 3 && k != 5 && k != 7)) return false;
    const long rows = (long)batch * h;
    long nb = rows < 512 ? rows : 512;
    const long per = (rows + nb - 1) / nb;
    nb = (rows + per - 1) / per;
    const int cop = (co + 63) / 64 * 64;
    *nblk = (int)nb;
    *rpb = (int)per;
    *part_bytes = (size_t)nb * kSmallCi * k * k * cop * sizeof(float);
    *bias_bytes = (size_t)nb * cop * sizeof(float);
    *lds = k * (w + k - 1) * (int)sizeof(float4) + w * 64 * (int)sizeof(float);
    return *lds <= 64 * 1024;
}


extern "C" {

size_t liso_conv_wgrad_workspace_bytes(const liso_conv_desc* d) {
    if (!d) return 0;
    Rs3Plan r;
    if (make_rs3_plan(*d, &r)) return r.slab_bytes + r.bias_bytes;
    WgPlan p;
    if (!make_plan(*d, &p)) return 0;
    return p.slab_bytes + p.bias_bytes;
}

size_t liso_conv_wgrad_sparse_workspace_bytes(const liso_conv_desc* d) {
    if (!d || !sparse_ok(*d)) return 0;
    size_t a, b, c, e, f;
    return sparse_layout(*d, &a, &b, &c, &e, &f);
}

int liso_conv_wgrad_sparse_f32(const liso_conv_desc* d, const float* x, const float* occupancy, const float* dy, int dy_pix_stride,
                               float* dw, float* dbias, void* workspace, size_t workspace_bytes, void* stream) {
    if (!d || !x || !occupancy || !dy || !dw || !workspace) return LISO_EINVAL;
    if (!sparse_ok(*d) || dy_pix_stride % 4 || dy_pix_stride < d->co || (((uintptr_t)x | (uintptr_t)dy) & 15)) return LISO_EINVAL;
    size_t o_cnt, o_off, o_cells, o_slab, o_bias;
    if (workspace_bytes < sparse_layout(*d, &o_cnt, &o_off, &o_cells, &o_slab, &o_bias)) return LISO_EWORKSPACE;
    hipStream_t st = (hipStream_t)stream;
    char* ws = (char*)workspace;
    const int rows = d->batch * d->hi;
    cells_count_kernel<<<rows, 256, 0, st>>>(occupancy, d->wi, (int*)(ws + o_cnt));
    cells_scan_kernel<<<1, 1024, 0, st>>>((const int*)(ws + o_cnt), rows, (int*)(ws + o_off));
    cells_fill_kernel<<<rows, 64, 0, st>>>(occupancy, d->wi, (const int*)(ws + o_off), (int*)(ws + o_cells));
    SpArgs a;
    a.x = x;
    a.dy = dy;
    a.cells = (const int*)(ws + o_cells);
    a.n_cells = (const int*)(ws + o_off) + rows;
    a.slab = (float*)(ws + o_slab);
    a.dy_pix_stride = dy_pix_stride;
    a.pad = 0;
    wgrad_sparse_kernel<<<dim3(d->n_taps, kSpSplits), 256, 0, st>>>(*d, a);
    if (dbias) {
        const long n_pix = (long)d->batch * d->ho * d->wo;
        const long per = (n_pix + kSpBiasRows - 1) / kSpBiasRows;
        dy_colsum_kernel<<<kSpBiasRows, 256, 0, st>>>(dy, n_pix, dy_pix_stride, d->co, per, (float*)(ws + o_bias));
    }
    if (hipGetLastError() != hipSuccess) return LISO_ELAUNCH;
    return launch_reduce((const float*)(ws + o_slab), (const float*)(ws + o_bias), kSpSplits, kSpBiasRows, d->w_taps, d->ci, d->co, 64, 64, 0,
                         dw, dbias, st);
}

int liso_conv_wgrad(const liso_conv_desc* d, const void* x, const float* in_scale, const float* in_shift, const void* dy,
                    int dy_pix_stride, int transposed, float* dw, float* dbias, void* workspace, size_t workspace_bytes,
                    void* stream) {
    if (!d || !x || !dy || !dw || !workspace) return LISO_EINVAL;
    if ((in_scale == nullptr) != (in_shift == nullptr)) return LISO_EINVAL;
    const bool h16 = d->mode == LISO_CONV_F16;
    const int vec = (d->mode == LISO_CONV_BF16 || h16) ? 8 : 4;
    if (dy_pix_stride % vec || dy_pix_stride < d->co || (((uintptr_t)x | (uintptr_t)dy) & 15)) return LISO_EINVAL;
    if (d->wgrad_co < 0 || d->wgrad_co > d->co) return LISO_EINVAL;
    Rs3Plan r3;
    if (make_rs3_plan(*d, &r3)) {
        if (workspace_bytes < r3.slab_bytes + r3.bias_bytes) return LISO_EWORKSPACE;
        r3.a.x = x;
        r3.a.in_scale = in_scale;
        r3.a.in_shift = in_shift;
        r3.a.dy = dy;
        r3.a.dy_pix_stride = dy_pix_stride;
        r3.a.slab = (float*)workspace;
        r3.a.bias_slab = dbias ? (float*)((char*)workspace + r3.slab_bytes) : nullptr;
        hipStream_t st3 = (hipStream_t)stream;
        int rc3;
        if (h16 && r3.a.ci_w == 32)
            rc3 = r3.th == 8 ? launch_rs3<LISO_CONV_F16, 8, 1, 32>(*d, r3, st3) : launch_rs3<LISO_CONV_F16, 4, 1, 32>(*d, r3, st3);
        else if (h16)
            rc3 = r3.stride == 2 ? launch_rs3<LISO_CONV_F16, 3, 2>(*d, r3, st3)
                  : r3.th == 8   ? launch_rs3<LISO_CONV_F16, 8, 1>(*d, r3, st3)
                                 : launch_rs3<LISO_CONV_F16, 4, 1>(*d, r3, st3);
        else if (r3.a.ci_w == 32)
            rc3 = d->mode == LISO_CONV_F32X3 ? launch_rs3<LISO_CONV_F32X3, 3, 1, 32>(*d, r3, st3)
                  : r3.th == 8           ? launch_rs3<LISO_CONV_BF16, 8, 1, 32>(*d, r3, st3)
                                         : launch_rs3<LISO_CONV_BF16, 4, 1, 32>(*d, r3, st3);
        else
            rc3 = d->mode == LISO_CONV_F32X3 ? launch_rs3<LISO_CONV_F32X3, 3, 1>(*d, r3, st3)
                  : r3.stride == 2       ? launch_rs3<LISO_CONV_BF16, 3, 2>(*d, r3, st3)
                  : r3.th == 8           ? launch_rs3<LISO_CONV_BF16, 8, 1>(*d, r3, st3)
                                         : launch_rs3<LISO_CONV_BF16, 4, 1>(*d, r3, st3);
        if (rc3 != LISO_OK) return rc3;
        const int co_w3 = d->wgrad_co > 0 ? d->wgrad_co : d->co;
        return launch_reduce(r3.a.slab, r3.a.bias_slab, r3.a.splits, r3.a.splits, d->w_taps, d->ci, co_w3, (long)r3.a.ci_t * r3.a.ci_w,
                             (long)r3.a.co_t * CT, transposed, dw, dbias, st3);
    }
    WgPlan p;
    if (!make_plan(*d, &p)) return LISO_EINVAL;
    if (workspace_bytes < p.slab_bytes + p.bias_bytes) return LISO_EWORKSPACE;
    p.a.x = x;
    p.a.in_scale = in_scale;
    p.a.in_shift = in_shift;
    p.a.dy = dy;
    p.a.dy_pix_stride = dy_pix_stride;
    p.a.slab = (float*)workspace;
    p.a.bias_slab = dbias ? (float*)((char*)workspace + p.slab_bytes) : nullptr;
    hipStream_t st = (hipStream_t)stream;
    int rc;
    if (d->mode == LISO_CONV_F32)
        rc = p.tg == 7 ? launch<LISO_CONV_F32, 7>(*d, p, st) : p.tg == 3 ? launch<LISO_CONV_F32, 3>(*d, p, st) : launch<LISO_CONV_F32, 1>(*d, p, st);
    else if (d->mode == LISO_CONV_F32X3)
        rc = p.tg == 7   ? launch<LISO_CONV_F32X3, 7>(*d, p, st)
             : p.tg == 3 ? launch<LISO_CONV_F32X3, 3>(*d, p, st)
                         : launch<LISO_CONV_F32X3, 1>(*d, p, st);
    else if (h16)
        rc = p.tg == 9   ? launch<LISO_CONV_F16, 9>(*d, p, st)
             : p.tg == 7 ? launch<LISO_CONV_F16, 7>(*d, p, st)
             : p.tg == 3 ? launch<LISO_CONV_F16, 3>(*d, p, st)
                         : launch<LISO_CONV_F16, 1>(*d, p, st);
    else
        rc = p.tg == 9   ? launch<LISO_CONV_BF16, 9>(*d, p, st)
             : p.tg == 7 ? launch<LISO_CONV_BF16, 7>(*d, p, st)
             : p.tg == 3 ? launch<LISO_CONV_BF16, 3>(*d, p, st)
                         : launch<LISO_CONV_BF16, 1>(*d, p, st);
    if (rc != LISO_OK) return rc;
    if (d->wgrad_co < 0 || d->wgrad_co > d->co) return LISO_EINVAL;
    const int co_w = d->wgrad_co > 0 ? d->wgrad_co : d->co;
    return launch_reduce(p.a.slab, p.a.bias_slab, p.splits, p.splits * d->n_classes, d->w_taps, d->ci, co_w, (long)p.a.ci_t * CT,
                         (long)p.a.co_t * CT, transposed, dw, dbias, st);
}

size_t liso_conv_wgrad_smallci_workspace_bytes(int batch, int h, int w, int co, int k) {
    int nblk, rpb, lds;
    size_t pb, bb;
    if (!smallci_layout(batch, h, w, co, k, &nblk, &rpb, &pb, &bb, &lds)) return 0;
    return pb + bb;
}

int liso_conv_wgrad_smallci_f32(const float* x, long x_pix_stride, const float* dy, long dy_pix_stride, int batch, int h, int w, int co,
                                int k, float* dw, float* dbias, void* workspace, size_t workspace_bytes, void* stream) {
    int nblk, rpb, lds;
    size_t pb, bb;
    if (!x || !dy || !dw || !workspace || x_pix_stride < kSmallCi || dy_pix_stride < co || (((uintptr_t)x) & 15) || (x_pix_stride & 3))
        return LISO_EINVAL;
    if (!smallci_layout(batch, h, w, co, k, &nblk, &rpb, &pb, &bb, &lds)) return LISO_EINVAL;
    if (workspace_bytes < pb + bb) return LISO_EWORKSPACE;
    float* partial = (float*)workspace;
    float* bias_partial = dbias ? (float*)((char*)workspace + pb) : nullptr;
    const int tiles = (co + 63) / 64, cop = tiles * 64;
    hipStream_t st = (hipStream_t)stream;
    const dim3 grid((unsigned)nblk, (unsigned)tiles);
#define LISO_SMALLCI(K) \
    hipLaunchKernelGGL(wgrad_smallci_kernel<K>, grid, dim3(256), lds, st, x, x_pix_stride, dy, dy_pix_stride, batch, h, w, co, rpb, partial, bias_partial)
    if (k == 7) LISO_SMALLCI(7);
    else if (k == 5) LISO_SMALLCI(5);
    else LISO_SMALLCI(3);
#undef LISO_SMALLCI
    const int n = kSmallCi * k * k * cop + (dbias ? cop : 0);
    hipLaunchKernelGGL(wgrad_smallci_reduce_kernel, dim3((n + 63) / 64), dim3(64, 8), 0, st, partial, bias_partial, nblk, k * k, co, cop, dw, dbias);
    return hipGetLastError() == hipSuccess ? LISO_OK : LISO_ELAUNCH;
}

}

#ifdef LISO_WGRAD_STAMPS
extern "C" int liso_wgrad_stamps_read(unsigned long long* host_out, int blocks) {
    if (!g_wgrad_stamps || blocks > 4096) return LISO_EINVAL;
    return hipMemcpy(host_out, g_wgrad_stamps, (size_t)blocks * 16 * 8, hipMemcpyDeviceToHost) == hipSuccess ? LISO_OK : LISO_ELAUNCH;
}
#endif
```

liso_amd/trainer.py:

```python
import contextlib
import os

import torch
import torch.distributed as dist

from liso_amd import _lib as L

from liso_amd.losses.centerpoint_loss import centerpoint_loss, rotation_vec_on_unit_circle
from liso_amd.networks.simple_net.simple_net import BoxLearner


def get_optimizer_scheduler(cfg, box_predictor, total_steps=None, flat=False):
    if flat:
        from liso_amd.utils.flat_adamw import FlatAdamW

        opt = FlatAdamW(box_predictor.parameters(), lr=cfg.optimization.learning_rate, weight_decay=0.01)
    else:
        opt = torch.optim.AdamW(box_predictor.parameters(), lr=cfg.optimization.learning_rate, weight_decay=0.01)
    common = dict(optimizer=opt, max_lr=cfg.optimization.learning_rate, pct_start=0.4, base_momentum=0.85, max_momentum=0.95,
                  div_factor=10.0)
    source = cfg.data.setdefault("train_on_box_source", "gt")
    if source == "gt":
        sched = torch.optim.lr_scheduler.OneCycleLR(total_steps=(total_steps or cfg.optimization.num_training_steps) + 2, **common)
    elif source == "mined":
        assert cfg.optimization.rounds.active, "assuming this"
        rounds = cfg.optimization.rounds
        sched = torch.optim.lr_scheduler.OneCycleLR(
            total_steps=(total_steps or rounds.steps_per_round * rounds.drop_net_weights_every_nth_round) + 2, final_div_factor=10,
            **common)
    else:
        raise NotImplementedError(source)
    return opt, sched


def get_slim_optimizer_scheduler(slim_cfg, params, flat=False):
    from liso_amd.utils.learning_rate import get_polynomial_decay_schedule_with_warmup

    if slim_cfg.optimizer == "rmsprop" and flat:
        from liso_amd.utils.flat_adamw import FlatRMSprop

        opt = FlatRMSprop(list(params), lr=slim_cfg.learning_rate.initial)
    elif slim_cfg.optimizer == "rmsprop":
        opt = torch.optim.RMSprop(params, lr=slim_cfg.learning_rate.initial)
    elif slim_cfg.optimizer == "adam":
        opt = torch.optim.Adam(params, lr=slim_cfg.learning_rate.initial)
    else:
        raise AssertionError("only rmsprop/adam supported")
    sched = get_polynomial_decay_schedule_with_warmup(
        optimizer=opt, num_warmup_steps=slim_cfg.learning_rate.warm_up.step_length,
        num_training_steps=slim_cfg.iterations.train, lr_end=slim_cfg.learning_rate.initial * 0.05)
    return opt, sched


def gather_gradients(device, params, add=False):
    from liso_amd import _lib as L
    import ctypes

    jobs = []
    for p_, flat in params:
        g = p_.grad
        p_.grad = flat
        if g is None or g is flat:
            continue
        if add or g.dtype != torch.float32 or g.stride() != flat.stride() or g.shape != flat.shape:
            flat.add_(g) if add else flat.copy_(g)
            continue
        jobs.append((g, flat))
    if not jobs:
        return []
    n = len(jobs)
    src = (ctypes.c_void_p * n)(*[g.data_ptr() for g, _ in jobs])
    dst = (ctypes.c_void_p * n)(*[f.data_ptr() for _, f in jobs])
    cnt = (ctypes.c_size_t * n)(*[g.numel() for g, _ in jobs])
    with torch.cuda.device(device):
        L.check(L.lib().liso_gather_f32(n, src, dst, cnt, L.stream_ptr()), "gather_f32")
    return [g for g, _ in jobs]


_SIDE_STREAMS = {}


def side_stream(device, role, priority=0):
    key = (device.index if device.index is not None else torch.cuda.current_device(), role)
    st = _SIDE_STREAMS.get(key)
    if st is None:
        st = _SIDE_STREAMS[key] = torch.cuda.Stream(device=device, priority=priority)
    return st


class DetectorTrainer:
    def __init__(self, cfg, device, compute_dtype=torch.float32, total_steps=None, fused_loss=None, use_graph=False, exact=None,
                 grad_buckets=None, loss_scale="default"):
        from liso_amd.losses import fused_centerpoint

        self.cfg, self.device = cfg, device
        if device.type == "cuda":
            from liso_amd.utils import mfma_conv as _MC
            _MC._sparse_flag(device)
        self.use_graph = bool(use_graph) and device.type == "cuda"
        self._graph, self._graph2, self._graph_sig, self._capture_stream = None, None, None, None
        self._wgrad_stream = None
        self.fused_loss = (fused_centerpoint.supports(cfg) and device.type == "cuda") if fused_loss is None else fused_loss
        self.net = BoxLearner(cfg).to(device)
        self.net.model.set_compute_dtype(compute_dtype)
        from liso_amd.utils import mfma_conv as MC
        if exact is not None:
            MC.set_fp32_mode("exact" if exact else "x3")
        if self.use_graph and not self.fused_loss:
            from liso_amd.utils.graph_safety import require_node_replay

            require_node_replay("DetectorTrainer(use_graph=True) without the fused loss")
        self.model = self.net
        self.world = dist.get_world_size() if dist.is_available() and dist.is_initialized() else 1
        self.optimizer, self.lr_scheduler = get_optimizer_scheduler(cfg, self.net, total_steps, flat=device.type == "cuda")
        self.loss_scaler = None
        if loss_scale == "default":
            loss_scale = "dynamic" if compute_dtype == torch.float16 else None
        if loss_scale is not None:
            if compute_dtype != torch.float16:
                raise ValueError(f"loss scaling is for fp16 training (compute_dtype {compute_dtype})")
            if device.type != "cuda":
                raise ValueError("fp16 training runs on the device kernels only")
            from liso_amd.utils.loss_scale import DeviceLossScale

            if loss_scale == "dynamic":
                self.loss_scaler = DeviceLossScale(device)
            elif isinstance(loss_scale, (int, float)) and not isinstance(loss_scale, bool):
                self.loss_scaler = DeviceLossScale(device, init_scale=float(loss_scale), dynamic=False)
            else:
                raise ValueError(f"loss_scale: 'dynamic', a number or None, got {loss_scale!r}")
            self.optimizer.loss_scale = self.loss_scaler
        if self.world > 1 and not self.use_graph:
            self.model = torch.nn.parallel.DistributedDataParallel(
                self.net, device_ids=[device.index] if device.type == "cuda" else None, bucket_cap_mb=64,
                broadcast_buffers=False, gradient_as_bucket_view=device.type != "cuda")
        self.n_grad_buckets = 1
        if self.use_graph:
            self._flat_grad = self.optimizer.flat_grad
            if self.world > 1:
                for t in list(self.net.parameters()) + list(self.net.buffers()):
                    dist.broadcast(t.data, src=0)
                self.optimizer.grad_scale = 1.0 / self.world
                self._setup_gradient_buckets(grad_buckets)
            elif grad_buckets == 2:
                self._setup_gradient_buckets(2)
        from liso_amd.networks.centerpoint.fused_bn import defer_batch_counters
        self._bn_counters = defer_batch_counters(self.net.model.rpn) + defer_batch_counters(self.net.model.center_head)

    def _setup_gradient_buckets(self, grad_buckets):
        from liso_amd.utils import mfma_conv as MC

        rpn = self.net.model.rpn
        if grad_buckets is None:
            grad_buckets = int(os.environ.get("LISO_GRAD_BUCKETS", "2"))
        if grad_buckets < 2 or len(rpn.blocks) < 2 or not hasattr(self.optimizer, "offsets"):
            return
        first = next(rpn.blocks[1].parameters())
        split = self.optimizer.offsets[id(first)]
        order = [id(p_) for p_ in self.net.parameters() if p_.requires_grad]
        assert all(self.optimizer.offsets[i] < split for i in order[:order.index(id(first))])
        assert all(self.optimizer.offsets[i] >= split for i in order[order.index(id(first)):])
        self._bucket_split = int(split)
        self._grad_cut = MC.GradCut()
        self.n_grad_buckets = 2

    def _reduce_gradients(self, rest_of_backward):
        if getattr(self, "skip_collective", False):
            rest_of_backward()
            return
        if self.n_grad_buckets < 2:
            rest_of_backward()
            dist.all_reduce(self._flat_grad)
            return
        w1 = dist.all_reduce(self._flat_grad[self._bucket_split:], async_op=True)
        rest_of_backward()
        w2 = dist.all_reduce(self._flat_grad[:self._bucket_split], async_op=True)
        w1.wait()
        w2.wait()

    def loss(self, pcls, targets, canvas=None):
        if self.model.training:
            from liso_amd.networks.centerpoint.fused_bn import step_batch_counters
            step_batch_counters(self._bn_counters)
        cfg = self.cfg
        sup = cfg.loss.supervised.supervised_on_clusters
        gt_maps = {a: targets[a] for a in sup.attrs}
        mask = targets["center_bool_mask"]
        if self.fused_loss:
            from liso_amd.losses.fused_centerpoint import fused_centerpoint_loss

            _, _, raw, _ = self.model(None, pcls, None, centermaps_gt=None, decode=False, canvas=canvas)
            total, losses = fused_centerpoint_loss(
                cfg=cfg, raw_box_maps=raw, gt_maps=gt_maps, gt_center_mask=mask,
                ignore_region_is_true_mask=targets.get("ignore_region_is_true_mask", None),
                pillar_center_coors_m=self.net.pillar_center_coors_m)
            return total, losses, None
        pred_boxes, decoded, activated, aux = self.model(None, pcls, None, centermaps_gt=None)
        ignore = targets.get("ignore_region_is_true_mask", torch.zeros_like(mask))
        losses = centerpoint_loss(loss_cfg=cfg.loss, raw_activated_pred_box_maps=activated, decoded_pred_box_maps=decoded,
                                  gt_maps=gt_maps, gt_center_mask=mask,
                                  rotation_loss_weights_map=torch.ones_like(gt_maps["probs"]),
                                  box_prediction_cfg=cfg.box_prediction, ignore_region_is_true_mask=ignore)
        total = 0.0
        for v in losses.values():
            total = total + sup.weight * v
        rr = cfg.box_prediction.rotation_representation
        if rr.method == "vector":
            total = total + rotation_vec_on_unit_circle(activated) * rr.regul_weight
        return total, losses, pred_boxes

    def step(self, pcls, targets, prep=None):
        self.model.train()
        if self.use_graph:
            return self._graph_step(pcls, targets, prep)
        self.optimizer.zero_grad(set_to_none=True)
        total, losses, _ = self.loss(pcls, targets)
        self._backward(total)
        self.optimizer.step()
        self.lr_scheduler.step()
        return total.detach()

    def _backward(self, total):
        if self.loss_scaler is None:
            total.backward()
        else:
            total.backward(self.loss_scaler.seed)

    def loss_scale_stats(self):
        return None if self.loss_scaler is None else self.loss_scaler.stats()

    def eager_pass(self, pcls, targets):
        self.model.train()
        saved = [p.grad for p in self.net.parameters()]
        for p in self.net.parameters():
            p.grad = None
        bufs = {k: v.clone() for k, v in self.net.state_dict().items() if "running" in k or "num_batches" in k}
        ctx = self.model.no_sync() if hasattr(self.model, "no_sync") else contextlib.nullcontext()
        with ctx:
            total, _, _ = self.loss(pcls, targets)
            self._backward(total)
        with torch.no_grad():
            for k, v in self.net.state_dict().items():
                if k in bufs:
                    v.copy_(bufs[k])
        for p, g in zip(self.net.parameters(), saved):
            p.grad = g
        return total.detach()

    def _pillars(self, pcls, out=None, prep=None):
        bev, occ = self.net.model.pfn(pcl_t0=pcls, img_t0=None, out=out, prep=prep)
        return bev, occ

    def _capture(self, pcls, targets):
        dev = self.device
        buffers = {k: v.clone() for k, v in self.net.state_dict().items() if v.is_floating_point() or v.dtype == torch.long}
        with torch.no_grad():
            bev, occ = self._pillars(pcls)
        self._static_bev = bev.detach().clone().requires_grad_(True)
        self._static_occ = occ.detach().clone()
        self._static_bev.grad = None
        self._static_targets = {k: v.to(dev).clone() for k, v in targets.items()}
        quiet = hasattr(torch.autograd.graph, "set_warn_on_accumulate_grad_stream_mismatch")
        if quiet:
            torch.autograd.graph.set_warn_on_accumulate_grad_stream_mismatch(False)
        if self._capture_stream is None:
            self._capture_stream = side_stream(dev, "flow")
        if self._wgrad_stream is None and os.environ.get("LISO_WGRAD_SIDE", "0") == "1":
            self._wgrad_stream = side_stream(dev, "wgrad")
        side = self._capture_stream
        side.wait_stream(torch.cuda.current_stream(dev))

        from liso_amd.utils import mfma_conv as MC

        self._pack_jobs = None
        self._gather_params = None

        cut = self._grad_cut if self.n_grad_buckets == 2 else None
        rpn = self.net.model.rpn

        def body(part=None):
            if part in (None, 1):
                self._flat_grad.zero_()
                self._static_bev.grad = None
                if self._pack_jobs:
                    self._step_packs = MC.batched_pack(self._pack_jobs)
            MC.set_step_packs(getattr(self, "_step_packs", None))
            det_cus = MC.roles_cus(getattr(self, "roles_cus", 0))
            det_cus.__enter__()
            MC.set_direct_grads(True, keep_touched=part == 2)
            gathered = self._gather_params or []
            for p_, _ in gathered:
                p_.grad = None
            try:
                if part in (None, 1):
                    rpn.grad_cut = cut
                    try:
                        total, _, _ = self.loss(None, self._static_targets, canvas=(self._static_bev, self._static_occ))
                    finally:
                        rpn.grad_cut = None
                    with MC.wgrad_side(self._wgrad_stream):
                        self._backward(total)
                    self._body_loss = total.detach()
                if cut is not None and part in (None, 2):
                    with MC.wgrad_side(self._wgrad_stream):
                        cut.finish()
            finally:
                det_cus.__exit__(None, None, None)
                MC.set_step_packs(None)
                MC.set_direct_grads(False, keep_touched=True)
                self._gather_gradients(gathered, add=part == 2)
            return self._body_loss

        self._gather_params = None
        with torch.cuda.stream(side):
            MC.record_pack_jobs(True)
            body()
            self._pack_jobs = MC.record_pack_jobs(False)
            if os.environ.get("LISO_GATHER_GRADS", "1") != "0":
                in_place = MC.direct_touched()
                outside = {id(p_) for p_ in self.net.model.pfn.parameters()}
                self._gather_params = [(p_, p_.grad) for p_ in self.net.parameters()
                                       if p_.requires_grad and p_.grad is not None and id(p_) not in in_place and id(p_) not in outside]
            body()
        torch.cuda.current_stream(dev).wait_stream(side)
        with torch.no_grad():
            for k, v in self.net.state_dict().items():
                if k in buffers:
                    v.copy_(buffers[k])
        self._graph, self._graph2 = torch.cuda.CUDAGraph(), None
        if cut is None:
            with torch.cuda.graph(self._graph, stream=side):
                self._static_loss = body()
        else:
            with torch.cuda.graph(self._graph, stream=side):
                self._static_loss = body(1)
            self._graph2 = torch.cuda.CUDAGraph()
            with torch.cuda.graph(self._graph2, stream=side, pool=self._graph.pool()):
                body(2)
        with torch.no_grad():
            for k, v in self.net.state_dict().items():
                if k in buffers:
                    v.copy_(buffers[k])
        if quiet:
            torch.autograd.graph.set_warn_on_accumulate_grad_stream_mismatch(True)

    def _gather_gradients(self, params, add=False):
        self._gather_keepalive = gather_gradients(self.device, params, add)

    def _graph_step(self, pcls, targets, prep=None):
        tsig = targets.shapes() if isinstance(targets, _BatchedTargets) else tuple((k, tuple(v.shape), v.dtype) for k, v in sorted(targets.items()))
        sig = (len(pcls), tsig)
        if self._graph is None or sig != self._graph_sig:
            self._graph = None
            self._capture(pcls, targets)
            self._graph_sig = sig
        bev, occ = self._pillars(pcls, out=(self._static_bev.detach().permute(0, 2, 3, 1), self._static_occ), prep=prep)
        with torch.no_grad():
            stage = []
            if isinstance(targets, _BatchedTargets):
                off = {}
                for t in targets.per_sample:
                    for k, v in t.items():
                        o = off.get(k, 0)
                        stage.append((self._static_targets[k][o:o + v.shape[0]], v))
                        off[k] = o + v.shape[0]
            else:
                for k, v in targets.items():
                    stage.append((self._static_targets[k], v))
            L.multi_copy(stage)
        self._graph.replay()

        def rest_of_backward():
            if self._graph2 is not None:
                self._graph2.replay()
            if bev.requires_grad:
                bev.backward(self._static_bev.grad)

        if self.world > 1:
            self._reduce_gradients(rest_of_backward)
        else:
            rest_of_backward()
        self.optimizer.step()
        self.lr_scheduler.step()
        return self._static_loss.clone()


class SlimTrainer:

    def __init__(self, cfg, device, num_train_samples=1000, use_graph=False, channels_last=False, exact=None):
        from liso_amd.slim.model.slim import SLIM
        if exact is not None:
            from liso_amd.utils import mfma_conv as MC
            MC.set_fp32_mode("exact" if exact else "x3")
        self.cfg, self.slim_cfg, self.device = cfg, cfg.SLIM, device
        if device.type == "cuda":
            from liso_amd.utils import mfma_conv as _MC
            _MC._sparse_flag(device)
        self.net = SLIM(cfg, num_train_samples=num_train_samples).to(device)
        if channels_last:
            self.net.raft_network.to(memory_format=torch.channels_last)
        self.model = self.net
        self.use_graph = bool(use_graph) and device.type == "cuda"
        self.world = dist.get_world_size() if dist.is_available() and dist.is_initialized() else 1
        if self.world > 1 and not self.use_graph:
            self.model = torch.nn.parallel.DistributedDataParallel(
                self.net, device_ids=[device.index] if device.type == "cuda" else None, bucket_cap_mb=64,
                broadcast_buffers=False, gradient_as_bucket_view=True)
        flat = device.type == "cuda" and self.model is self.net and os.environ.get("LISO_FLAT_RMSPROP", "1") != "0"
        self.optimizer, self.lr_scheduler = get_slim_optimizer_scheduler(self.slim_cfg, self.net.parameters(), flat=flat)
        self._flat_opt = hasattr(self.optimizer, "flat_grad")
        import numpy as np
        half = 0.5 * np.array(cfg.data.bev_range_m, dtype=np.float32)
        self.bev_extent = np.concatenate([-half, half], axis=0)
        self._graph, self._graph_sig = None, None
        if self.use_graph:
            from liso_amd.utils.graph_safety import require_node_replay

            require_node_replay("SlimTrainer(use_graph=True)")
            self.net.raft_network.defer_update_block_wgrad = "direct"
            params = [p for p in self.net.parameters() if p.requires_grad]
            if self._flat_opt:
                self._flat_grad = self.optimizer.flat_grad
            else:
                self._flat_grad = torch.zeros(sum(p.numel() for p in params), dtype=torch.float32, device=device)
                off = 0
                for p in params:
                    p.grad = self._flat_grad[off:off + p.numel()].view_as(p)
                    off += p.numel()
            outside = {id(p) for p in self.net.raft_network.pp_layer.parameters()} if hasattr(self.net.raft_network, "pp_layer") else set()
            self._gather_params = [(p, p.grad) for p in params if id(p) not in outside] \
                if os.environ.get("LISO_GATHER_GRADS", "1") != "0" else []
            if self.world > 1:
                for t in list(self.net.parameters()) + list(self.net.buffers()):
                    dist.broadcast(t.data, src=0)

    def _inputs(self, sample_t0, sample_t1):
        pc1, m1 = sample_t0["pcl_ta"]["pcl"].to(self.device), sample_t0["pcl_ta"]["pcl_is_valid"].to(self.device)
        pc2, m2 = sample_t1["pcl_ta"]["pcl"].to(self.device), sample_t1["pcl_ta"]["pcl_is_valid"].to(self.device)
        return pc1, m1, pc2, m2

    def loss(self, sample_t0, sample_t1, all_valid=None, canvases=None, gather_plan=None):
        from liso_amd.slim.slim_loss.knn_graph import KnnIndex
        from liso_amd.slim.slim_loss.slim_loss_adaptor import selfsupervisedSlimSingleScaleLoss

        pc1, m1, pc2, m2 = self._inputs(sample_t0, sample_t1)
        if all_valid is None:
            all_valid = (bool(m1.all()), bool(m2.all()))
        ext = [float(v) for v in self.bev_extent]
        idx1 = [KnnIndex(pc1[b][:, :3], extent=ext, all_rows_finite=True) for b in range(pc1.shape[0])] if all_valid[0] else None
        idx2 = [KnnIndex(pc2[b][:, :3], extent=ext, all_rows_finite=True) for b in range(pc2.shape[0])] if all_valid[1] else None
        if canvases is None:
            preds_fw, preds_bw = self.model(sample_t0, sample_t1, None)
        else:
            preds_fw, preds_bw = self.model(sample_t0, sample_t1, None, canvases=canvases, gather_plan=gather_plan)
        kw = dict(moving_thresh_module=self.net.moving_dynamicness_threshold, loss_cfg=self.slim_cfg.losses.unsupervised,
                  model_cfg=self.slim_cfg.model, bev_extent=self.bev_extent, metrics_collector={})
        stacked = getattr(self.net, "stacked_predictions", None)
# ... 785 lines not shown
```

liso_amd/utils/mfma_conv.py:

```python
import ctypes
import os
import weakref

import torch

from liso_amd import _lib as L


def on_device(x):
    if not x.is_cuda:
        return False
    L.elem_code(x.dtype)
    return True


class ConvSpec:

    def __init__(self, kh, kw, stride=1, padding=0, transposed=False):
        self.kh, self.kw, self.stride, self.padding, self.transposed = int(kh), int(kw), int(stride), int(padding), bool(transposed)

    @staticmethod
    def of(conv):
        st = conv.stride[0] if isinstance(conv.stride, (tuple, list)) else conv.stride
        pd = conv.padding[0] if isinstance(conv.padding, (tuple, list)) else conv.padding
# ... 7 lines not shown


_FP32_MODE = "exact" if os.environ.get("LISO_CONV_FP32", "x3") == "exact" else "x3"


def set_fp32_mode(mode):
    global _FP32_MODE
    assert mode in ("x3", "exact"), mode
    prev, _FP32_MODE = _FP32_MODE, mode
    return prev


def fp32_mode():
    return _FP32_MODE


class fp32_arithmetic:

    def __init__(self, mode):
        self.mode = mode

    def __enter__(self):
        self.prev = set_fp32_mode(self.mode)
        return self

    def __exit__(self, *exc):
        set_fp32_mode(self.prev)
        return False


def _mode(dtype):
    if dtype == torch.bfloat16:
        return L.CONV_BF16
    if dtype == torch.float16:
        return L.CONV_F16
    if dtype == torch.float32:
        return L.CONV_F32 if _FP32_MODE == "exact" else L.CONV_F32X3
    raise L.LisoHipError(f"mfma conv: unsupported dtype {dtype}")


def _base_desc(B, hi, wi, ci, x_ps, ho, wo, co, y_ps, y_off, mode, out_f32, in_relu, out_relu, w_taps):
    d = L.ConvDesc()
    d.batch, d.hi, d.wi, d.ci, d.x_pix_stride = B, hi, wi, ci, x_ps
    d.ho, d.wo, d.co, d.y_pix_stride, d.y_ch_off = ho, wo, co, y_ps, y_off
    d.mode, d.out_f32, d.in_relu, d.out_relu, d.w_taps = mode, int(out_f32), int(in_relu), int(out_relu), w_taps
    return d


_DESC_CACHE = {}
_COPY_LOG = None


def _cached(fn):
    def wrapper(spec, *args, **kw):
        key = (fn.__name__, spec.kh, spec.kw, spec.stride, spec.padding, spec.transposed, args, tuple(sorted(kw.items())))
        d = _DESC_CACHE.get(key)
        if d is None:
            d = _DESC_CACHE[key] = fn(spec, *args, **kw)
        return d
    return wrapper


@_cached
def gather_desc(spec, B, hi, wi, ci, x_ps, ho, wo, co, y_ps, y_off, mode, out_f32=False, in_relu=False, out_relu=False):
    d = _base_desc(B, hi, wi, ci, x_ps, ho, wo, co, y_ps, y_off, mode, out_f32, in_relu, out_relu, spec.kh * spec.kw)
    d.hv, d.wv, d.isy, d.isx, d.osy, d.osx = ho, wo, spec.stride, spec.stride, 1, 1
    d.n_classes = 1
    d.class_tap_begin[0], d.class_tap_begin[1] = 0, spec.kh * spec.kw
    d.n_taps = spec.kh * spec.kw
    assert d.n_taps <= L.CONV_MAX_TAPS
    for ky in range(spec.kh):
        for kx in range(spec.kw):
            t = ky * spec.kw + kx
            d.tap_dy[t], d.tap_dx[t], d.tap_w[t] = ky - spec.padding, kx - spec.padding, t
    return d


@_cached
def scatter_desc(spec, B, hi, wi, ci, x_ps, ho, wo, co, y_ps, y_off, mode, out_f32=False, in_relu=False, out_relu=False):
    s, p = spec.stride, spec.padding
    d = _base_desc(B, hi, wi, ci, x_ps, ho, wo, co, y_ps, y_off, mode, out_f32, in_relu, out_relu, spec.kh * spec.kw)
    d.hv, d.wv = (ho + s - 1) // s, (wo + s - 1) // s
    d.isy, d.isx, d.osy, d.osx = 1, 1, s, s
    n, cls = 0, 0
    d.class_tap_begin[0] = 0
    for py in range(s):
        for px in range(s):
            taps = [(ky, kx) for ky in range(spec.kh) for kx in range(spec.kw) if (py + p - ky) % s == 0 and (px + p - kx) % s == 0]
            if not taps:
                continue
            for ky, kx in taps:
                assert n < L.CONV_MAX_TAPS
                d.tap_dy[n], d.tap_dx[n], d.tap_w[n] = (py + p - ky) // s, (px + p - kx) // s, ky * spec.kw + kx
                n += 1
            d.class_ooy[cls], d.class_oox[cls] = py, px
            cls += 1
            d.class_tap_begin[cls] = n
    assert cls <= L.CONV_MAX_CLASSES
    d.n_classes, d.n_taps = cls, n
    d.sparse_output = cls < s * s
    return d


def _pix_stride(v):
    B, H, W, C = v.shape
    if W > 1:
        return v.stride(2)
    if H > 1:
        return v.stride(1)
    if B > 1:
        return v.stride(0)
    return C


def as_nhwc(t, vec):
    v = t.permute(0, 2, 3, 1)
    B, H, W, C = v.shape
    ps = _pix_stride(v)
    regular = (v.stride(3) == 1 or C == 1) and ps >= C and (W == 1 or v.stride(2) == ps) and (H == 1 or v.stride(1) == W * ps) and \
        (B == 1 or v.stride(0) == H * W * ps) and ps % vec == 0 and v.data_ptr() % 16 == 0
    if not regular:
        if _COPY_LOG is not None:
            import traceback
            fr = [f"{f.name}:{f.lineno}" for f in traceback.extract_stack(limit=7)[:-1] if "mfma_conv" not in f.filename][-3:]
            _COPY_LOG[(tuple(t.shape), tuple(t.stride()), tuple(fr))] = _COPY_LOG.get((tuple(t.shape), tuple(t.stride()), tuple(fr)), 0) + 1
        v = t.contiguous(memory_format=torch.channels_last).permute(0, 2, 3, 1)
        if v.stride(3) != 1 and C > 1:
            v = v.contiguous()
        ps = C
    return v, ps


_PACK_CACHE = {}


_SHARED_DEPTH = [0]


class shared_gpu:

    def __enter__(self):
        _SHARED_DEPTH[0] += 1
        if _SHARED_DEPTH[0] == 1:
            L.check(L.lib().liso_conv_set_option(L.CONV_OPT_SHARED_GPU, 1), "conv_set_option")
        return self

    def __exit__(self, *exc):
        _SHARED_DEPTH[0] -= 1
        if _SHARED_DEPTH[0] == 0:
            L.check(L.lib().liso_conv_set_option(L.CONV_OPT_SHARED_GPU, 0), "conv_set_option")
        return False


_WGRAD_SIDE = None


class wgrad_side:

    def __init__(self, stream):
        self.stream = stream

    def __enter__(self):
        global _WGRAD_SIDE
        self.prev = _WGRAD_SIDE
        _WGRAD_SIDE = {"stream": self.stream, "keep": [], "used": False} if self.stream is not None else None
        return self

    def __exit__(self, *exc):
        global _WGRAD_SIDE
        st, _WGRAD_SIDE = _WGRAD_SIDE, self.prev
        if st is not None and st["used"]:
            torch.cuda.current_stream(st["stream"].device).wait_stream(st["stream"])
            st["keep"].clear()
        return False


class roles_cus:

    def __init__(self, n):
        self.n = int(n)

    def __enter__(self):
        if self.n:
            L.check(L.lib().liso_conv_set_option(L.CONV_OPT_ROLES_CUS, self.n), "conv_set_option")
        return self

    def __exit__(self, *exc):
        if self.n:
            L.check(L.lib().liso_conv_set_option(L.CONV_OPT_ROLES_CUS, 0), "conv_set_option")
        return False


_PACK_RECORD = None
_STEP_PACKS = None


def record_pack_jobs(on=True):
    global _PACK_RECORD
    if on:
        _PACK_RECORD = {}
        return None
    jobs, _PACK_RECORD = list((_PACK_RECORD or {}).values()), None
    return jobs


def batched_pack(jobs):
    out, arr = {}, (L.ConvPackJob * len(jobs))()
    keep = []
    for i, (key, weight, spec, for_dgrad, mode) in enumerate(jobs):
        w = weight.detach()
        if w.dtype != torch.float32 or not w.is_contiguous():
            w = w.float().contiguous()
        keep.append(w)
        d0, d1 = w.shape[0], w.shape[1]
        same = spec.transposed == bool(for_dgrad)
        K, N = (d1, d0) if same else (d0, d1)
        dst = torch.empty(L.lib().liso_conv_packed_bytes(K, N, spec.kh * spec.kw, mode), dtype=torch.uint8, device=w.device)
        arr[i] = L.ConvPackJob(w.data_ptr(), dst.data_ptr(), d0, d1, spec.kh, spec.kw, int(spec.transposed), int(bool(for_dgrad)), mode)
        out[key] = dst
    if jobs:
        with torch.cuda.device(jobs[0][1].device):
            L.check(L.lib().liso_conv_pack_weights_batched(arr, len(jobs), L.stream_ptr()), "conv_pack_weights_batched")
    return out


def set_step_packs(packs):
    global _STEP_PACKS
    _STEP_PACKS = packs


def pack_weights(weight, spec, for_dgrad, mode):
    L.require_cuda(weight)
    if not isinstance(weight, torch.nn.Parameter):
        return _pack_weights(weight, spec, for_dgrad, mode)
    pkey = (id(weight), spec.kh, spec.kw, spec.transposed, bool(for_dgrad), mode)
    if _STEP_PACKS is not None and pkey in _STEP_PACKS:
        return _STEP_PACKS[pkey]
    if _PACK_RECORD is not None:
        _PACK_RECORD[pkey] = (pkey, weight, spec, bool(for_dgrad), mode)
    if weight.requires_grad and torch.cuda.is_current_stream_capturing():
        return _pack_weights(weight, spec, for_dgrad, mode)
    key = (id(weight), spec.transposed, bool(for_dgrad), mode)
    hit = _PACK_CACHE.get(key)
    if hit is not None and hit[0]() is weight and hit[1] == weight._version and hit[2] == weight.data_ptr():
        return hit[3]
    out = _pack_weights(weight, spec, for_dgrad, mode)
    _PACK_CACHE[key] = (weakref.ref(weight, lambda _r, k=key: _PACK_CACHE.pop(k, None)), weight._version, weight.data_ptr(), out)
    return out


def _pack_weights(weight, spec, for_dgrad, mode):
    w = weight.detach()
    if w.dtype != torch.float32 or not w.is_contiguous():
        w = w.float().contiguous()
    d0, d1 = w.shape[0], w.shape[1]
    same = spec.transposed == bool(for_dgrad)
    K, N = (d1, d0) if same else (d0, d1)
    nbytes = L.lib().liso_conv_packed_bytes(K, N, spec.kh * spec.kw, mode)
    out = torch.empty(nbytes, dtype=torch.uint8, device=w.device)
    with torch.cuda.device(w.device):
        L.check(L.lib().liso_conv_pack_weights(L.ptr(w), d0, d1, spec.kh, spec.kw, int(spec.transposed), int(bool(for_dgrad)), mode,
                                               L.ptr(out), L.stream_ptr()), "conv_pack_weights")
    return out


def _half_mode(mode):
    return mode in (L.CONV_BF16, L.CONV_F16)


def _vec(mode):
    return 8 if _half_mode(mode) else 4


def _timer_name(mode, kind, d=None):
    name = ("conv_bf16_" if mode == L.CONV_BF16 else "conv_f16_" if mode == L.CONV_F16 else "conv_f32x3_" if mode == L.CONV_F32X3
            else "conv_f32_") + kind
    if d is not None and L.TIMER.enabled:
        kind = L.lib().liso_conv_kernel_kind(ctypes.byref(d))
        name += "_roles" if kind == 1 else "_direct" if kind in (2, 3) else ""
    return name


def _flops(d):
    taps = d.n_taps if d.n_classes == 1 else d.n_taps / d.n_classes
    return 2.0 * d.batch * d.ho * d.wo * d.co * d.ci * taps


def _bytes(d, wgrad=False):
    es = 2 if _half_mode(d.mode) else 4
    w = d.w_taps * d.ci * d.co
    if wgrad:
        return d.batch * (d.hi * d.wi * d.ci + d.ho * d.wo * d.co) * es + 4 * w
    out_es = 4 if (d.out_f32 or not _half_mode(d.mode)) else 2
    return d.batch * (d.hi * d.wi * d.ci * es + d.ho * d.wo * d.co * out_es) + w * (2 if _half_mode(d.mode) else 4)


def conv_forward(x, weight, bias, spec, in_scale=None, in_shift=None, in_relu=False, out_relu=False, out_dtype=None,
                 want_stats=False, stats_shift=None, packed=None, affine_batch_stride=0, occupancy=None, out=None):
    L.require_cuda(x, weight)
    mode = _mode(x.dtype)
    xv, xps = as_nhwc(x, _vec(mode))
    B, hi, wi, ci = xv.shape
    co = weight.shape[1] if spec.transposed else weight.shape[0]
    ho, wo = spec.out_hw(hi, wi)
    out_dtype = out_dtype or x.dtype
    if not _half_mode(mode):
        assert out_dtype == torch.float32
    else:
        assert out_dtype in (x.dtype, torch.float32), "16-bit convolutions write their own dtype or fp32"
    out_f32 = out_dtype == torch.float32
    if out is not None:
        buf, y_off = out
        assert buf.is_contiguous() and tuple(buf.shape[:3]) == (B, ho, wo) and buf.dtype == out_dtype and y_off + co <= buf.shape[3], \
            (tuple(buf.shape), (B, ho, wo, co), y_off)
        y_ps = buf.shape[3]
        assert y_ps % _vec(mode) == 0 and y_off % 8 == 0
        y_base, y = buf, buf[..., y_off:y_off + co]
    else:
        y = torch.empty((B, ho, wo, co), dtype=out_dtype, device=x.device)
        y_base, y_ps, y_off = y, co, 0
    build = scatter_desc if spec.transposed else gather_desc
    d = build(spec, B, hi, wi, ci, xps, ho, wo, co, y_ps, y_off, mode, out_f32, in_relu, out_relu)
    if affine_batch_stride:
        d = L.ConvDesc.from_buffer_copy(d)
        d.in_affine_batch_stride = int(affine_batch_stride)
    if packed is None:
        packed = pack_weights(weight, spec, False, mode)
    lib = L.lib()
    stats = None
    if want_stats:
        rows = lib.liso_conv_stats_rows(ctypes.byref(d))
        if rows <= 0:
            raise L.LisoHipError("conv_forward: unsupported geometry")
        stats = torch.empty((rows, 2, (co + 63) // 64 * 64), dtype=torch.float32, device=x.device)
    b = bias.detach() if bias is not None else None
    if b is not None and (b.dtype != torch.float32 or not b.is_contiguous()):
        b = b.float().contiguous()
    occ = None
    if occupancy is not None and in_scale is None and spec.transposed is False:
        occ = occupancy
        assert occ.dtype == torch.float32 and occ.is_contiguous() and occ.numel() == B * hi * wi, (occ.shape, occ.dtype)
    with torch.cuda.device(x.device):
        L.check(L.TIMER.launch(_timer_name(mode, "fwd", d), lambda: lib.liso_conv_forward_sparse(
            ctypes.byref(d), L.ptr(xv), L.ptr(packed), L.ptr(b) if b is not None else None,
            L.ptr(in_scale) if in_scale is not None else None, L.ptr(in_shift) if in_shift is not None else None, L.ptr(y_base),
            L.ptr(stats) if stats is not None else None, L.ptr(stats_shift) if stats_shift is not None else None,
            L.ptr(occ) if occ is not None else None, L.stream_ptr()),
            units=_flops(d), nbytes=_bytes(d)), "conv_forward")
    return y.permute(0, 3, 1, 2), stats


def _pad_out_channels(dy, weight, spec, vec):
    co = dy.shape[1]
    pad = (-co) % vec
    if pad == 0:
        return dy, weight
    dy = torch.nn.functional.pad(dy, (0, 0, 0, 0, 0, pad))
    if weight is not None:
        weight = torch.nn.functional.pad(weight.detach(), (0, 0, 0, 0, 0, pad) if spec.transposed else (0, 0, 0, 0, 0, 0, 0, pad))
    return dy, weight


def conv_dgrad(dy, weight, spec, x_shape, out_dtype=None, packed=None):
    L.require_cuda(dy, weight)
    mode = _mode(dy.dtype)
    dy, weight = _pad_out_channels(dy, weight if packed is None else None, spec, _vec(mode))
    gv, gps = as_nhwc(dy, _vec(mode))
    B, ho, wo, co = gv.shape
    _, ci, hi, wi = x_shape
    out_dtype = out_dtype or dy.dtype
    out_f32 = out_dtype == torch.float32
    build = gather_desc if spec.transposed else scatter_desc
    d = build(spec, B, ho, wo, co, gps, hi, wi, ci, ci, 0, mode, out_f32, False, False)
    alloc = torch.zeros if getattr(d, "sparse_output", False) else torch.empty
    if not spec.transposed and ((ho - 1) * spec.stride - spec.padding + spec.kh < hi or (wo - 1) * spec.stride - spec.padding + spec.kw < wi):
        alloc = torch.zeros
    dx = alloc((B, hi, wi, ci), dtype=out_dtype, device=dy.device)
    if packed is None:
        packed = pack_weights(weight, spec, True, mode)
    with torch.cuda.device(dy.device):
        L.check(L.TIMER.launch(_timer_name(mode, "dgrad", d), lambda: L.lib().liso_conv_forward(
            ctypes.byref(d), L.ptr(gv), L.ptr(packed), None, None, None, L.ptr(dx), None, None, L.stream_ptr()), units=_flops(d), nbytes=_bytes(d)),
            "conv_dgrad")
    return dx.permute(0, 3, 1, 2)


def conv_wgrad(x, dy, weight_shape, spec, in_scale=None, in_shift=None, in_relu=False, want_bias=True, out_dw=None, out_db=None,
               co_true=None):
    L.require_cuda(x, dy)
    if (x.shape[1] == 4 and x.dtype == torch.float32 and not spec.transposed and spec.stride == 1 and spec.kh == spec.kw and spec.kh in (5, 7)
            and spec.padding == spec.kh // 2 and in_scale is None and tuple(weight_shape[1:]) == (4, spec.kh, spec.kw)
            and os.environ.get("LISO_WGRAD_SMALLCI", "1") != "0"):
        res = _conv_wgrad_smallci(x, dy, weight_shape, spec, want_bias, out_dw, out_db, co_true)
        if res is not None:
            return res
    mode = _mode(x.dtype)
    if dy.dtype != x.dtype:
        dy = dy.to(x.dtype)
    if co_true is None:
        co_true = dy.shape[1]
        dy, _ = _pad_out_channels(dy, None, spec, _vec(mode))
    xv, xps = as_nhwc(x, _vec(mode))
    gv, gps = as_nhwc(dy, _vec(mode))
    B, hi, wi, ci = xv.shape
    _, ho, wo, co = gv.shape
    build = scatter_desc if spec.transposed else gather_desc
    d = build(spec, B, hi, wi, ci, xps, ho, wo, co, co, 0, mode, True, in_relu, False)
    if co != co_true:
        d = L.ConvDesc.from_buffer_copy(d)
        d.wgrad_co = co_true
    lib = L.lib()
    nbytes = lib.liso_conv_wgrad_workspace_bytes(ctypes.byref(d))
    if nbytes == 0:
        return None
    ws = torch.empty(nbytes, dtype=torch.uint8, device=x.device)
    dw = out_dw if out_dw is not None else torch.empty(weight_shape, dtype=torch.float32, device=x.device)
    db = (out_db if out_db is not None else torch.empty(co_true, dtype=torch.float32, device=x.device)) if want_bias else None
    with torch.cuda.device(x.device):
        L.check(L.TIMER.launch(_timer_name(mode, "wgrad"), lambda: lib.liso_conv_wgrad(
            ctypes.byref(d), L.ptr(xv), L.ptr(in_scale) if in_scale is not None else None,
            L.ptr(in_shift) if in_shift is not None else None, L.ptr(gv), gps, int(spec.transposed), L.ptr(dw),
            L.ptr(db) if db is not None else None, L.ptr(ws), nbytes, L.stream_ptr()), units=_flops(d), nbytes=_bytes(d, True)), "conv_wgrad")
    return dw, db


def _conv_wgrad_smallci(x, dy, weight_shape, spec, want_bias, out_dw, out_db, co_true):
    if dy.dtype != torch.float32:
        dy = dy.float()
    xv, xps = as_nhwc(x, 4)
    gv, gps = as_nhwc(dy, 4)
    B, hi, wi, _ = xv.shape
    co = co_true if co_true is not None else gv.shape[3]
    if gv.shape[1:3] != (hi, wi) or weight_shape[0] != co:
        return None
    lib = L.lib()
    nbytes = lib.liso_conv_wgrad_smallci_workspace_bytes(B, hi, wi, co, spec.kh)
    if nbytes == 0:
        return None
    ws = torch.empty(nbytes, dtype=torch.uint8, device=x.device)
    dw = out_dw if out_dw is not None else torch.empty(weight_shape, dtype=torch.float32, device=x.device)
    db = (out_db if out_db is not None else torch.empty(co, dtype=torch.float32, device=x.device)) if want_bias else None
    with torch.cuda.device(x.device):
        L.check(L.TIMER.launch("conv_wgrad_smallci", lambda: lib.liso_conv_wgrad_smallci_f32(
            L.ptr(xv), xps, L.ptr(gv), gps, B, hi, wi, co, spec.kh, L.ptr(dw), L.ptr(db) if db is not None else None, L.ptr(ws), nbytes,
            L.stream_ptr()), units=2.0 * B * hi * wi * co * 4 * spec.kh * spec.kw), "conv_wgrad_smallci")
    return dw, db


def conv_wgrad_sparse(x, occupancy, dy, weight_shape, spec, want_bias=True):
    L.require_cuda(x, dy, occupancy)
    if x.dtype != torch.float32 or spec.transposed or occupancy.dtype != torch.float32:
        return None
    if dy.dtype != torch.float32:
        dy = dy.float()
    xv, xps = as_nhwc(x, 4)
    gv, gps = as_nhwc(dy, 4)
    B, hi, wi, ci = xv.shape
    _, ho, wo, co = gv.shape
    occ = occupancy.contiguous()
    if occ.numel() != B * hi * wi:
        return None
    d = gather_desc(spec, B, hi, wi, ci, xps, ho, wo, co, co, 0, _mode(x.dtype), True, False, False)
    lib = L.lib()
    nbytes = lib.liso_conv_wgrad_sparse_workspace_bytes(ctypes.byref(d))
    if nbytes == 0:
        return None
    ws = torch.empty(nbytes, dtype=torch.uint8, device=x.device)
    dw = torch.empty(weight_shape, dtype=torch.float32, device=x.device)
    db = torch.empty(co, dtype=torch.float32, device=x.device) if want_bias else None
    with torch.cuda.device(x.device):
        L.check(L.TIMER.launch("conv_wgrad_sparse", lambda: lib.liso_conv_wgrad_sparse_f32(
            ctypes.byref(d), L.ptr(xv), L.ptr(occ), L.ptr(gv), gps, L.ptr(dw), L.ptr(db) if db is not None else None, L.ptr(ws), nbytes,
            L.stream_ptr()), units=_flops(d), nbytes=_bytes(d, True)), "conv_wgrad_sparse")
    return dw, db


def supported(x, weight, spec):
    if not x.is_cuda or x.dtype not in (torch.bfloat16, torch.float16, torch.float32):
        return False
    vec = 8 if L.is_half(x.dtype) else 4
    ci = x.shape[1]
    co = weight.shape[1] if spec.transposed else weight.shape[0]
    if ci % vec or spec.kh * spec.kw > L.CONV_MAX_TAPS:
        return False
    if spec.transposed and (spec.kh != spec.stride or spec.padding != 0):
        return False
    return co >= 1


class BnFold:

    def __init__(self, groups, relu=True, training=True):
        self.groups, self.relu, self.training = list(groups), bool(relu), bool(training)
        self._ss = None

    @property
    def channels(self):
        return sum(g["gamma"].shape[0] for g in self.groups)

    def scale_shift(self):
        if self._ss is None:
            if len(self.groups) == 1:
                st, C = self.groups[0]["stats"], self.groups[0]["gamma"].shape[0]
                self._ss = (st[:C], st[C:2 * C])
            else:
                self._ss = (torch.cat([g["stats"][:g["gamma"].shape[0]] for g in self.groups]).contiguous(),
                            torch.cat([g["stats"][g["gamma"].shape[0]:2 * g["gamma"].shape[0]] for g in self.groups]).contiguous())
        return self._ss

    def group(self, k):
        return BnFold([self.groups[k]], self.relu, self.training)

    @staticmethod
    def cat(folds):
        assert all(f.relu == folds[0].relu and f.training == folds[0].training for f in folds)
        return BnFold([g for f in folds for g in f.groups], folds[0].relu, folds[0].training)

    def params(self):
        return [t for g in self.groups for t in (g["gamma"], g["beta"])]


def finalize_bn(stats_partial, n_pixels, bn, stats_shift=None, channel_offset=0):
    C = bn.num_features
    stats = torch.empty(4 * C, dtype=torch.float32, device=stats_partial.device)
    rows, _, cop = stats_partial.shape
    mom = bn.momentum if bn.momentum is not None else 0.1
    track = bn.track_running_stats and bn.training
    part = ctypes.c_void_p(stats_partial.data_ptr() + 4 * channel_offset)
    with torch.cuda.device(stats_partial.device):
        L.check(L.lib().liso_conv_bn_finalize(
            part, rows, C, cop, int(n_pixels), L.ptr(stats_shift) if stats_shift is not None else None,
            L.ptr(bn.weight), L.ptr(bn.bias), L.ptr(bn.running_mean) if track else None, L.ptr(bn.running_var) if track else None,
            float(mom), float(bn.eps), L.ptr(stats), L.stream_ptr()), "conv_bn_finalize")
    return BnFold([{"stats": stats, "gamma": bn.weight, "beta": bn.bias}], True, True)


def eval_bn_fold(bn, relu=True):
    with torch.no_grad():
        invstd = torch.rsqrt(bn.running_var.float() + bn.eps)
        scale = bn.weight.detach().float() * invstd
        shift = bn.bias.detach().float() - bn.running_mean.float() * scale
        stats = torch.cat([scale, shift, bn.running_mean.float(), invstd]).contiguous()
    return BnFold([{"stats": stats, "gamma": bn.weight, "beta": bn.bias}], relu, False)


_DIRECT_GRADS = False
_DIRECT_TOUCHED = set()


def set_direct_grads(on, keep_touched=False):
    global _DIRECT_GRADS
    _DIRECT_GRADS = bool(on)
    if not keep_touched:
        _DIRECT_TOUCHED.clear()


def direct_touched():
    return set(_DIRECT_TOUCHED)


def _direct_target(p):
    if not _DIRECT_GRADS or not isinstance(p, torch.nn.Parameter):
        return None
    g = p.grad
    if g is None or g.dtype != torch.float32 or not g.is_contiguous() or g.shape != p.shape or id(p) in _DIRECT_TOUCHED:
        return None
    _DIRECT_TOUCHED.add(id(p))
    return g


_BN_TICKETS = {}


def _bn_ticket(key, device):
    if os.environ.get("LISO_BN_TICKET", "0") != "1":
        return None
    ent = _BN_TICKETS.get(device.index)
    if ent is None:
        if torch.cuda.is_current_stream_capturing():
            return None
        ent = _BN_TICKETS[device.index] = [torch.zeros(4096, dtype=torch.int32, device=device), {}]
    slot = ent[1].get(key)
    if slot is None:
        if len(ent[1]) >= ent[0].numel():
            return None
        slot = ent[1][key] = len(ent[1])
    return ent[0][slot:slot + 1]


def _rows_view(t, vec):
    v = t.permute(0, 2, 3, 1)
    B, H, W, C = v.shape
    ps = _pix_stride(v)
    regular = (v.stride(3) == 1 or C == 1) and ps >= C and (W == 1 or v.stride(2) == ps) and (H == 1 or v.stride(1) == W * ps) and \
        (B == 1 or v.stride(0) == H * W * ps) and ps % vec == 0 and v.data_ptr() % 16 == 0
    return (v, ps) if regular else (None, 0)


def _bn_backward_group(g, x_raw, grp, relu, training, out=None):
    C = grp["gamma"].shape[0]
    vec = 8 if L.is_half(x_raw.dtype) else 4
    xv, xs = _rows_view(x_raw, vec)
    if xv is None:
        xv, xs = x_raw.permute(0, 2, 3, 1).contiguous(), C
    if g.dtype != xv.dtype:
        g = g.to(xv.dtype)
    gv, gs = _rows_view(g, vec)
    if gv is None:
        gv, gs = g.permute(0, 2, 3, 1).contiguous(), C
    M = xv.numel() // C
    lib = L.lib()
    dxv, ds = _rows_view(out, vec) if out is not None else (None, 0)
    if dxv is None:
        dxv, ds = torch.empty(xv.shape, dtype=xv.dtype, device=xv.device), C
    tg, tb = _direct_target(grp["gamma"]), _direct_target(grp["beta"])
    direct = tg is not None and tb is not None
    gg = tg if direct else torch.empty(C, dtype=torch.float32, device=xv.device)
    gb = tb if direct else torch.empty(C, dtype=torch.float32, device=xv.device)
    nbytes = lib.liso_bn_workspace_bytes(C)
    ws = torch.empty(nbytes, dtype=torch.uint8, device=xv.device)
    bf = L.elem_code(xv.dtype)
    units = 5 * M * C * xv.element_size()
    with torch.cuda.device(xv.device):
        if (xs, gs, ds) != (C, C, C):
            L.check(L.TIMER.launch("bn_bwd", lambda: lib.liso_bn_relu_bwd_strided(
                L.ptr(gv), gs, L.ptr(xv), xs, bf, M, C, L.ptr(grp["gamma"]), L.ptr(grp["stats"]), int(training), int(relu), L.ptr(dxv), ds,
                L.ptr(gg), L.ptr(gb), L.ptr(ws), nbytes, L.stream_ptr()), units=units), "bn_relu_bwd_strided")
        else:
            args = (L.ptr(gv), L.ptr(xv), bf, M, C, L.ptr(grp["gamma"]), L.ptr(grp["stats"]), int(training), int(relu), L.ptr(dxv), L.ptr(gg),
                    L.ptr(gb), L.ptr(ws), nbytes)
            ticket = _bn_ticket(grp.get("ticket_key", id(grp["gamma"])), xv.device)
            if ticket is not None:
                L.check(L.TIMER.launch("bn_bwd", lambda: lib.liso_bn_relu_bwd_ticket(*args, L.ptr(ticket), L.stream_ptr()), units=units),
                        "bn_relu_bwd_ticket")
            else:
                L.check(L.TIMER.launch("bn_bwd", lambda: lib.liso_bn_relu_bwd(*args, L.stream_ptr()), units=units), "bn_relu_bwd")
    return dxv.permute(0, 3, 1, 2), (None if direct else gg), (None if direct else gb)


def _bn_backward(g, x_raw, fold):
    if len(fold.groups) == 1:
        dx, gg, gb = _bn_backward_group(g, x_raw, fold.groups[0], fold.relu, fold.training)
        return dx, [gg, gb]
    Cs = [grp["gamma"].shape[0] for grp in fold.groups]
    if sum(Cs) > 256:
        B, _, H, W = x_raw.shape
        dx_full = torch.empty((B, H, W, sum(Cs)), dtype=x_raw.dtype, device=x_raw.device).permute(0, 3, 1, 2)
        grads, a = [], 0
        for grp in fold.groups:
            C = grp["gamma"].shape[0]
            dx, gg, gb = _bn_backward_group(g[:, a:a + C], x_raw[:, a:a + C], grp, fold.relu, fold.training, out=dx_full[:, a:a + C])
            if dx.data_ptr() != dx_full[:, a:a + C].data_ptr():
                dx_full[:, a:a + C].copy_(dx)
            grads += [gg, gb]
            a += C
        return dx_full, grads
    gam = torch.cat([grp["gamma"].detach() for grp in fold.groups])
    stats = torch.cat([grp["stats"][k * c:(k + 1) * c] for k in range(4) for grp, c in zip(fold.groups, Cs)])
    dx, gg, gb = _bn_backward_group(g, x_raw, {"gamma": gam, "beta": None, "stats": stats, "ticket_key": id(fold.groups[0]["gamma"])},
                                    fold.relu, fold.training)
    grads, a = [], 0
    for c in Cs:
        grads += [gg[a:a + c], gb[a:a + c]]
        a += c
    return dx, grads


class _FusedConv(torch.autograd.Function):
    @staticmethod
    def forward(ctx, x_raw, weight, bias, meta, *fold_params):
        spec, fold = meta["spec"], meta["fold"]
        sc, sh = fold.scale_shift() if fold is not None else (None, None)
        occ = meta.get("occupancy") if fold is None else None
        res = None
        if occ is not None and meta.get("out_dtype") in (None, x_raw.dtype):
            res = _sparse_stem(x_raw, occ, weight, bias, spec, "batch" if meta.get("want_stats", False) else "none",
                               meta.get("out_relu", False), stats_shift=meta.get("stats_shift"))
        sparse_ws = None
        if res is not None:
            y, part, sparse_ws = res
        else:
            y, part = conv_forward(x_raw, weight, bias, spec, sc, sh, in_relu=fold.relu if fold is not None else False,
                                   out_relu=meta.get("out_relu", False), out_dtype=meta.get("out_dtype"),
                                   want_stats=meta.get("want_stats", False), stats_shift=meta.get("stats_shift"), occupancy=occ,
                                   out=meta.get("out"))
        meta["stats_partial"] = part
        relu = bool(meta.get("out_relu", False))
        ctx.save_for_backward(x_raw, weight, y if relu else None)
        ctx.meta = {"spec": spec, "fold": fold, "has_bias": bias is not None, "n_fold_params": len(fold_params), "relu": relu,
                    "bias_param": bias if isinstance(bias, torch.nn.Parameter) else None, "occupancy": occ, "sparse_ws": sparse_ws}
        return y

    @staticmethod
    def backward(ctx, dy):
        x_raw, weight, y = ctx.saved_tensors
        spec, fold = ctx.meta["spec"], ctx.meta["fold"]
        if dy.dtype != x_raw.dtype:
            dy = dy.to(x_raw.dtype)
        if ctx.meta["relu"]:
            dy = torch.ops.aten.threshold_backward(dy, y, 0.0)
        sc, sh = fold.scale_shift() if fold is not None else (None, None)
        dw = db = dx = None
        fold_grads = [None] * ctx.meta["n_fold_params"]
        co_true = dy.shape[1]
        if co_true % _vec(_mode(dy.dtype)):
            dy, _ = _pad_out_channels(dy, None, spec, _vec(_mode(dy.dtype)))
        if ctx.needs_input_grad[1] or (ctx.meta["has_bias"] and ctx.needs_input_grad[2]):
            tw = _direct_target(weight)
            tb = _direct_target(ctx.meta["bias_param"]) if tw is not None and ctx.meta["has_bias"] else None
            if ctx.meta["has_bias"] and tb is None:
                tw = None
            res = None
            if ctx.meta.get("occupancy") is not None and co_true == dy.shape[1]:
                res = conv_wgrad_sparse(x_raw, ctx.meta["occupancy"], dy, tuple(weight.shape), spec, want_bias=ctx.meta["has_bias"])
                tw = None if res is not None else tw
            if res is None:
                side = _WGRAD_SIDE if (tw is not None and dy.is_cuda) else None
                if side is not None:
                    ev = torch.cuda.Event()
                    ev.record(torch.cuda.current_stream(dy.device))
                    with torch.cuda.stream(side["stream"]):
                        side["stream"].wait_event(ev)
                        res = conv_wgrad(x_raw, dy, tuple(weight.shape), spec, sc, sh, in_relu=fold.relu if fold is not None else False,
                                         want_bias=ctx.meta["has_bias"], out_dw=tw, out_db=tb, co_true=co_true)
                    side["keep"].append((x_raw, dy, sc, sh))
                    side["used"] = True
                else:
                    res = conv_wgrad(x_raw, dy, tuple(weight.shape), spec, sc, sh, in_relu=fold.relu if fold is not None else False,
                                     want_bias=ctx.meta["has_bias"], out_dw=tw, out_db=tb, co_true=co_true)
            if res is None:
                raise NotImplementedError(f"liso_amd: no device weight-gradient kernel for {tuple(weight.shape)} stride {spec.stride} "
                                          f"on {tuple(x_raw.shape)} {x_raw.dtype}")
            else:
                dw, db = res
                if tw is not None and dw is tw:
                    dw, db = None, None
            if dw is not None:
                dw = dw.to(weight.dtype)
            if db is not None:
                db = db.to(weight.dtype)
        if ctx.needs_input_grad[0] or any(ctx.needs_input_grad[4:]):
            g = None
            if ctx.meta.get("occupancy") is not None and fold is None and co_true == dy.shape[1]:
                g = _sparse_dgrad(dy, ctx.meta["occupancy"], weight, spec, tuple(x_raw.shape), x_raw.dtype, lists=ctx.meta.get("sparse_ws"))
            if g is None:
                g = conv_dgrad(dy, weight, spec, tuple(x_raw.shape))
            if fold is not None:
                dx, fold_grads = _bn_backward(g, x_raw, fold)
            else:
                dx = g
        return (dx, dw, db, None, *fold_grads)


def fused_conv(x_raw, fold, conv, out_bn=None, out_dtype=None, out_relu=False, spec=None, occupancy=None, out=None):
    convs = list(conv) if isinstance(conv, (list, tuple)) else [conv]
    bns = (list(out_bn) if isinstance(out_bn, (list, tuple)) else [out_bn]) if out_bn is not None else None
    spec = spec or ConvSpec.of(convs[0])
    if len(convs) == 1:
        weight, bias = convs[0].weight, convs[0].bias
    elif torch.is_grad_enabled() and any(c.weight.requires_grad for c in convs):
        weight = torch.cat([c.weight for c in convs], dim=0)
        bias = torch.cat([c.bias for c in convs], dim=0) if convs[0].bias is not None else None
    else:
        key = tuple((id(c), c.weight._version, c.weight.data_ptr(), None if c.bias is None else c.bias._version) for c in convs)
        hit = getattr(convs[0], "_liso_merged_weights", None)
        if hit is None or hit[0] != key:
            w = torch.nn.Parameter(torch.cat([c.weight.detach() for c in convs], dim=0), requires_grad=False)
            b = torch.cat([c.bias.detach() for c in convs], dim=0) if convs[0].bias is not None else None
            hit = convs[0]._liso_merged_weights = (key, w, b)
        weight, bias = hit[1], hit[2]
    training_bn = bns is not None and (bns[0].training or not bns[0].track_running_stats)
    meta = {"spec": spec, "fold": fold, "out_dtype": out_dtype, "want_stats": training_bn, "out_relu": out_relu, "occupancy": occupancy,
            "out": out if occupancy is None else None}
    if training_bn and len(bns) == 1 and bns[0].track_running_stats:
        meta["stats_shift"] = bns[0].running_mean
    params = fold.params() if fold is not None else []
    y = _FusedConv.apply(x_raw, weight, bias, meta, *params)
    if bns is None:
        return y, None
    if not training_bn:
        return y, BnFold.cat([eval_bn_fold(b, relu=True) for b in bns])
    n = y.shape[0] * y.shape[2] * y.shape[3]
    folds, off = [], 0
    for b in bns:
        if b.training and b.track_running_stats and not getattr(b, "_liso_counter_deferred", False):
            b.num_batches_tracked += 1
        folds.append(finalize_bn(meta["stats_partial"], n, b, meta.get("stats_shift"), channel_offset=off))
        off += b.num_features
    return y, BnFold.cat(folds)


class InFold:

    def __init__(self, stats, channels, relu=True):
        self.stats, self.channels, self.relu = stats, int(channels), bool(relu)

    @property
    def scale(self):
        return self.stats

    @property
    def shift(self):
        return self.stats[:, self.channels:]

    @property
    def stride(self):
        return 4 * self.channels


def _norm_kind(norm):
    if isinstance(norm, torch.nn.Sequential) and len(norm) == 0:
        return "none"
    if isinstance(norm, torch.nn.InstanceNorm2d) and not norm.track_running_stats:
        return "instance"
    return None


@torch.no_grad()
def conv_in(x_raw, fold, conv, norm, relu=True, spec=None, occupancy=None):
    spec = spec or ConvSpec.of(conv)
    kind = _norm_kind(norm)
    kw = {}
    if fold is not None:
        kw = dict(in_scale=fold.scale, in_shift=fold.shift, in_relu=fold.relu, affine_batch_stride=fold.stride)
    if fold is None and occupancy is not None:
        res = _sparse_stem(x_raw, occupancy, conv.weight, conv.bias, spec, kind, relu)
        if res is not None:
            y, part, _ = res
            if kind == "none":
                return y, None
            return y, _in_fold_from_partial(y, part, norm, relu)
        kw["occupancy"] = occupancy
    if kind == "none":
        y, _ = conv_forward(x_raw, conv.weight, conv.bias, spec, out_relu=relu, **kw)
        return y, None
    y, part = conv_forward(x_raw, conv.weight, conv.bias, spec, want_stats=True, **kw)
    return y, _in_fold_from_partial(y, part, norm, relu)


def _in_fold_from_partial(y, part, norm, relu):
    B, C, H, W = y.shape
    stats = torch.empty((B, 4 * C), dtype=torch.float32, device=y.device)
    rows, _, cop = part.shape
    with torch.cuda.device(y.device):
        L.check(L.lib().liso_conv_in_finalize(L.ptr(part), rows // B, B, C, cop, H * W,
                                              L.ptr(norm.weight) if norm.affine else None, L.ptr(norm.bias) if norm.affine else None,
                                              float(norm.eps), L.ptr(stats), L.stream_ptr()), "conv_in_finalize")
    return InFold(stats, C, relu)


SPARSE_STEM_MAX_CELLS = 40960
_SPARSE_OVERFLOW = {}


def sparse_stem_overflowed(device):
    t = _SPARSE_OVERFLOW.get(_dev_index(torch.device(device)))
    return bool(t is not None and int(t.item()) != 0)


def reset_sparse_stem_overflow(device):
    t = _SPARSE_OVERFLOW.get(_dev_index(torch.device(device)))
    if t is not None:
        t.zero_()


def _dev_index(dev):
    return dev.index if dev.index is not None else torch.cuda.current_device()


def _sparse_mode(el):
    return {L.ELEM_BF16: L.CONV_BF16, L.ELEM_F16: L.CONV_F16}.get(int(el), L.CONV_F32X3)


def _sparse_geometry(x_raw, weight, spec):
    if os.environ.get("LISO_SPARSE_STEM", "1") == "0" or spec.transposed or x_raw.dim() != 4:
        return None
    B, C, H, W = x_raw.shape
    geo = (spec.kh, spec.kw, spec.stride, spec.padding, weight.shape[0])
    bf = L.elem_code(x_raw.dtype) if x_raw.dtype in (torch.bfloat16, torch.float16) else 0
    if C != 64 or tuple(weight.shape[1:]) != (64, spec.kh, spec.kw) or H % 2 or W % 64:
        return None
    if geo == (7, 7, 2, 3, 32) and x_raw.dtype == torch.float32 and fp32_mode() == "x3":
# ... 225 lines not shown
```

Measured before the change: 999.7.

## Defer conv weight-gradients and launch them as grouped rs3 and reduce kernels

Conv weight-gradient calls whose targets are the parameter grads are recorded during backward instead of launched. They are then issued at the end as one grouped rs3 kernel plus one grouped reduce kernel, with per-layer descriptors looked up by block index. This replaces the optional side-stream wgrad path and cuts many small launches, letting small layers fill the GPU together. The cost is that wgrad work can no longer overlap with dgrad, and recorded tensors must stay alive until the grouped launch runs.

```diff
diff --git a/include/liso_conv.h b/include/liso_conv.h
--- a/include/liso_conv.h
+++ b/include/liso_conv.h
@@ -78,6 +78,21 @@
                     int dy_pix_stride, int transposed, float* dw, float* dbias, void* workspace, size_t workspace_bytes,
                     void* stream);
 
+#define LISO_CONV_WGRAD_GROUP_MAX 64
+typedef struct {
+    const liso_conv_desc* d;
+    const void* x;
+    const float* in_scale;
+    const float* in_shift;
+    const void* dy;
+    int dy_pix_stride;
+    int transposed;
+    float* dw;
+    float* dbias;
+} liso_conv_wgrad_item;
+size_t liso_conv_wgrad_grouped_workspace_bytes(const liso_conv_wgrad_item* items, int n_items);
+int liso_conv_wgrad_grouped(const liso_conv_wgrad_item* items, int n_items, void* workspace, size_t workspace_bytes, void* stream);
+
 int liso_conv_bn_finalize(const float* stats_partial, int rows, int co, int co_pad, long n, const float* stats_shift,
                           const float* gamma, const float* beta, float* running_mean, float* running_var, float momentum,
                           float eps, float* stats, void* stream);
diff --git a/liso_amd/_lib.py b/liso_amd/_lib.py
--- a/liso_amd/_lib.py
+++ b/liso_amd/_lib.py
@@ -236,6 +236,8 @@
     "liso_conv_plan_info": (_i, [_vp, _vp]),
     "liso_conv_wgrad_workspace_bytes": (_sz, [_vp]),
     "liso_conv_wgrad": (_i, [_vp, _vp, _vp, _vp, _vp, _i, _i, _vp, _vp, _vp, _sz, _vp]),
+    "liso_conv_wgrad_grouped_workspace_bytes": (_sz, [_vp, _i]),
+    "liso_conv_wgrad_grouped": (_i, [_vp, _i, _vp, _sz, _vp]),
     "liso_conv_wgrad_sparse_workspace_bytes": (_sz, [_vp]),
     "liso_conv_wgrad_sparse_f32": (_i, [_vp, _vp, _vp, _vp, _i, _vp, _vp, _vp, _sz, _vp]),
     "liso_conv_wgrad_smallci_workspace_bytes": (_sz, [_i, _i, _i, _i, _i]),
@@ -295,6 +297,14 @@
                 ("in_affine_batch_stride", _i), ("wgrad_co", _i)]
 
 
+class ConvWgradItem(ctypes.Structure):
+    _fields_ = [("d", _vp), ("x", _vp), ("in_scale", _vp), ("in_shift", _vp), ("dy", _vp), ("dy_pix_stride", _i), ("transposed", _i),
+                ("dw", _vp), ("dbias", _vp)]
+
+
+CONV_WGRAD_GROUP_MAX = 64
+
+
 class ConvPackJob(ctypes.Structure):
     _fields_ = [("src", _vp), ("dst", _vp), ("d0", _i), ("d1", _i), ("kh", _i), ("kw", _i), ("transposed", _i), ("for_dgrad", _i),
                 ("mode", _i)]
diff --git a/liso_amd/csrc/conv_wgrad.hip b/liso_amd/csrc/conv_wgrad.hip
--- a/liso_amd/csrc/conv_wgrad.hip
+++ b/liso_amd/csrc/conv_wgrad.hip
@@ -1,6 +1,8 @@
 #include <hip/hip_runtime.h>
 #include <stdint.h>
 #include <stdlib.h>
+
+#include <type_traits>
 
 #include "../../include/liso_conv.h"
 #include "../../include/liso_iou3d.h"
@@ -459,8 +461,42 @@
 constexpr int kRsThreads = 512;
 constexpr int RPS = 128;
 
-template <int MODE, int TH, int S, int CIW>
-__global__ __launch_bounds__(kRsThreads, 1) void conv_wgrad_rs3_kernel(const liso_conv_desc d, const WgArgs a) {
+struct Rs3Layer {
+    const void* x;
+    const float* in_scale;
+    const float* in_shift;
+    const void* dy;
+    float* slab;
+    float* bias_slab;
+#ifdef LISO_WGRAD_STAMPS
+    unsigned long long* stamps;
+#endif
+    int hi, wi, ci, x_pix_stride, ho, wo, co, dy_pix_stride, in_relu, wgrad_co, w_taps;
+    int ci_t, co_t, tiles_x, tiles_y, n_tiles, splits;
+    int first_block;
+    int tap_w[9];
+};
+struct Rs3One {
+    Rs3Layer l;
+    __device__ const Rs3Layer& layer(int block, int& local) const {
+        local = block;
+        return l;
+    }
+};
+constexpr int kRsGroupMax = 20;
+struct Rs3Group {
+    int n;
+    Rs3Layer l[kRsGroupMax];
+    __device__ const Rs3Layer& layer(int block, int& local) const {
+        int i = 0;
+        while (i + 1 < n && block >= l[i + 1].first_block) i++;
+        local = block - l[i].first_block;
+        return l[i];
+    }
+};
+
+template <int MODE, int TH, int S, int CIW, class Args>
+__global__ __launch_bounds__(kRsThreads, 1) void conv_wgrad_rs3_kernel(const Args args) {
     using E = typename liso_e16::Elem<MODE>::T;
     constexpr bool X3 = MODE == LISO_CONV_F32X3;
     constexpr int PLANES = X3 ? 2 : 1;
@@ -479,14 +515,15 @@
     constexpr int NE = X3 ? 4 : 8;
     extern __shared__ __attribute__((aligned(16))) unsigned char smem[];
     const int tid = threadIdx.x, wave = tid >> 6, lane = tid & 63;
-    int t = blockIdx.x;
-    const int split = t % a.splits;
-    t /= a.splits;
-    const int cot = t % a.co_t;
-    const int cit = t / a.co_t;
+    int t;
+    const Rs3Layer& L = args.layer(blockIdx.x, t);
+    const int split = t % L.splits;
+    t /= L.splits;
+    const int cot = t % L.co_t;
+    const int cit = t / L.co_t;
     const int ci0 = cit * CIW, co0 = cot * CT;
-    const long cip = (long)a.ci_t * CIW, cop = (long)a.co_t * CT;
-    const int n_mine = split < a.n_tiles ? (a.n_tiles - split + a.splits - 1) / a.splits : 0;
+    const long cip = (long)L.ci_t * CIW, cop = (long)L.co_t * CT;
+    const int n_mine = split < L.n_tiles ? (L.n_tiles - split + L.splits - 1) / L.splits : 0;
 
     if (wave >= 4) {
         const int ltid = tid - 256;
@@ -498,15 +535,15 @@
         float bsum[NE];
 #pragma unroll
         for (int e = 0; e < NE; e++) bsum[e] = 0.0f;
-        const bool want_bias = a.bias_slab != nullptr && cit == 0;
-        const bool pro = a.in_scale != nullptr;
+        const bool want_bias = L.bias_slab != nullptr && cit == 0;
+        const bool pro = L.in_scale != nullptr;
         const int ch = ci0 + ccx * NE, chy = co0 + cc * NE;
-        const bool ch_ok = ch < d.ci, chy_ok = chy < d.co;
+        const bool ch_ok = ch < L.ci, chy_ok = chy < L.co;
         if (pro) {
 #pragma unroll
             for (int e = 0; e < NE; e++) {
-                sc[e] = ch_ok ? a.in_scale[ch + e] : 0.0f;
-                sh[e] = ch_ok ? a.in_shift[ch + e] : 0.0f;
+                sc[e] = ch_ok ? L.in_scale[ch + e] : 0.0f;
+                sh[e] = ch_ok ? L.in_shift[ch + e] : 0.0f;
             }
         }
         int rel[XB];
@@ -515,45 +552,45 @@
         for (int u = 0; u < XB; u++) {
             const int pix = p0x + u * PSLX;
             const int ly = pix / IW, lx = pix - ly * IW;
-            rel[u] = (ly * d.wi + lx) * d.x_pix_stride;
+            rel[u] = (ly * L.wi + lx) * L.x_pix_stride;
             lyx[u] = (unsigned)ly | ((unsigned)lx << 8) | (pix < NPX && ch_ok ? 0x10000u : 0u);
         }
         auto load_tile = [&](int tile) {
-            const int tx = tile % a.tiles_x;
-            const int tq = tile / a.tiles_x;
-            const int ty = tq % a.tiles_y, b = tq / a.tiles_y;
+            const int tx = tile % L.tiles_x;
+            const int tq = tile / L.tiles_x;
+            const int ty = tq % L.tiles_y, b = tq / L.tiles_y;
             const int iy0 = ty * TH * S - 1, ix0 = tx * TW * S - 1;
-            const long xbase = (long)b * d.hi * d.wi * d.x_pix_stride + ch;
-            const int org = (iy0 * d.wi + ix0) * d.x_pix_stride;
-            const bool inner = iy0 >= 0 && iy0 + IH <= d.hi && ix0 >= 0 && ix0 + IW <= d.wi;
+            const long xbase = (long)b * L.hi * L.wi * L.x_pix_stride + ch;
+            const int org = (iy0 * L.wi + ix0) * L.x_pix_stride;
+            const bool inner = iy0 >= 0 && iy0 + IH <= L.hi && ix0 >= 0 && ix0 + IW <= L.wi;
             xok = 0u;
 #pragma unroll
             for (int u = 0; u < XB; u++) {
                 bool ok = (lyx[u] >> 16) != 0u;
                 if (!inner) {
                     const int iy = iy0 + (int)(lyx[u] & 0xffu), ix = ix0 + (int)((lyx[u] >> 8) & 0xffu);
-                    ok = ok && (unsigned)iy < (unsigned)d.hi && (unsigned)ix < (unsigned)d.wi;
+                    ok = ok && (unsigned)iy < (unsigned)L.hi && (unsigned)ix < (unsigned)L.wi;
                 }
                 xok |= ok ? (1u << u) : 0u;
                 const long off = xbase + (ok ? org + rel[u] : 0);
                 if constexpr (X3)
-                    xv[u] = *reinterpret_cast<const uint4*>((const float*)a.x + off);
+                    xv[u] = *reinterpret_cast<const uint4*>((const float*)L.x + off);
                 else
-                    xv[u] = *reinterpret_cast<const uint4*>((const unsigned short*)a.x + off);
-            }
-            const long ybase = (long)b * d.ho * d.wo * a.dy_pix_stride + chy;
+                    xv[u] = *reinterpret_cast<const uint4*>((const unsigned short*)L.x + off);
+            }
+            const long ybase = (long)b * L.ho * L.wo * L.dy_pix_stride + chy;
             yok = 0u;
 #pragma unroll
             for (int u = 0; u < YB; u++) {
                 const int m = p0 + u * PSL;
                 const int oy = ty * TH + (m >> 5), ox = tx * TW + (m & 31);
-                const bool ok = chy_ok && oy < d.ho && ox < d.wo;
+                const bool ok = chy_ok && oy < L.ho && ox < L.wo;
                 yok |= ok ? (1u << u) : 0u;
-                const long off = ybase + (ok ? (long)(oy * d.wo + ox) * a.dy_pix_stride : 0);
+                const long off = ybase + (ok ? (long)(oy * L.wo + ox) * L.dy_pix_stride : 0);
                 if constexpr (X3)
-                    yv[u] = *reinterpret_cast<const uint4*>((const float*)a.dy + off);
+                    yv[u] = *reinterpret_cast<const uint4*>((const float*)L.dy + off);
                 else
-                    yv[u] = *reinterpret_cast<const uint4*>((const unsigned short*)a.dy + off);
+                    yv[u] = *reinterpret_cast<const uint4*>((const unsigned short*)L.dy + off);
             }
         };
         auto store_tile = [&](unsigned char* buf) {
@@ -572,7 +609,7 @@
                     for (int e = 0; e < 4; e++) {
                         if (pro) {
                             f[e] = fmaf(f[e], sc[e], sh[e]);
-                            if (d.in_relu) f[e] = fmaxf(f[e], 0.0f);
+                            if (L.in_relu) f[e] = fmaxf(f[e], 0.0f);
                         }
                         if (!((xok >> u) & 1u)) f[e] = 0.0f;
                     }
@@ -592,7 +629,7 @@
                         for (int e = 0; e < 4; e++) {
                             float f0 = fmaf(E::lo(w[e]), sc[2 * e], sh[2 * e]);
                             float f1 = fmaf(E::hi(w[e]), sc[2 * e + 1], sh[2 * e + 1]);
-                            if (d.in_relu) {
+                            if (L.in_relu) {
                                 f0 = fmaxf(f0, 0.0f);
                                 f1 = fmaxf(f1, 0.0f);
                             }
@@ -650,7 +687,7 @@
         if (n_mine > 0) {
             load_tile(split);
             store_tile(smem);
-            if (n_mine > 1) load_tile(split + a.splits);
+            if (n_mine > 1) load_tile(split + L.splits);
         }
         __syncthreads();
 #ifdef LISO_WGRAD_STAMPS
@@ -661,15 +698,15 @@
             if (k + 1 < n_mine) {
                 store_tile(smem + ((k + 1) & 1) * BUF);
                 WSTAMP_END(ws_store)
-                if (k + 2 < n_mine) load_tile(split + (k + 2) * a.splits);
+                if (k + 2 < n_mine) load_tile(split + (k + 2) * L.splits);
                 WSTAMP_END(ws_load)
             }
             __syncthreads();
             WSTAMP_END(ws_bar)
         }
 #ifdef LISO_WGRAD_STAMPS
-        if (ltid == 0 && a.stamps) {
-            unsigned long long* o = a.stamps + (size_t)blockIdx.x * 16 + 8;
+        if (ltid == 0 && L.stamps) {
+            unsigned long long* o = L.stamps + (size_t)blockIdx.x * 16 + 8;
             o[0] = ws_k1 - ws_k0; o[1] = ws_store; o[2] = ws_load; o[3] = ws_bar; o[4] = (unsigned long long)n_mine;
         }
 #endif
@@ -684,7 +721,7 @@
             const int grp_c = ltid / NE, e = ltid % NE;
             float s_ = 0.0f;
             for (int pp = 0; pp < PSL; pp++) s_ += red[(pp * CPP + grp_c) * NE + e];
-            a.bias_slab[(long)split * cop + co0 + ltid] = s_;
+            L.bias_slab[(long)split * cop + co0 + ltid] = s_;
         }
         if constexpr (CIW == 32) __syncthreads();
         return;
@@ -789,10 +826,10 @@
     const int r = lane & 31, h = lane >> 5;
 #pragma unroll
     for (int i = 0; i < 9; i++) {
-        const int wt = d.tap_w[i];
-        float* base = a.slab + (((long)split * d.w_taps + wt) * cip + ci0 + ci_half * 32) * cop + co0 + co_half * 32 + r;
-        if (co0 + co_half * 32 + r < (d.wgrad_co > 0 ? d.wgrad_co : d.co)) {
-            const int rows_left = d.ci - (ci0 + ci_half * 32);
+        const int wt = L.tap_w[i];
+        float* base = L.slab + (((long)split * L.w_taps + wt) * cip + ci0 + ci_half * 32) * cop + co0 + co_half * 32 + r;
+        if (co0 + co_half * 32 + r < (L.wgrad_co > 0 ? L.wgrad_co : L.co)) {
+            const int rows_left = L.ci - (ci0 + ci_half * 32);
 #pragma unroll
             for (int e = 0; e < 16; e++) {
                 const int row = (e & 3) + 8 * (e >> 2) + 4 * h;
@@ -802,8 +839,8 @@
     }
 #ifdef LISO_WGRAD_STAMPS
     __builtin_amdgcn_s_waitcnt(0x0F70);
-    if (tid == 0 && a.stamps) {
-        unsigned long long* o = a.stamps + (size_t)blockIdx.x * 16;
+    if (tid == 0 && L.stamps) {
+        unsigned long long* o = L.stamps + (size_t)blockIdx.x * 16;
         const unsigned long long ms_k3 = __builtin_amdgcn_s_memtime();
         o[0] = ms_k1 - ms_k0; o[1] = ms_mul; o[2] = ms_bar; o[3] = ms_k2 - ms_k0; o[4] = ms_k3 - ms_k2; o[5] = ms_k3 - ms_k0;
     }
@@ -811,16 +848,14 @@
 }
 
 template <int PARTS>
-__global__ __launch_bounds__(256) void wgrad_reduce_kernel(const float* __restrict__ slab, const float* __restrict__ bias_slab,
-                                                           int splits, int bias_rows, int taps, int ci, int co, long cip, long cop,
-                                                           int transposed, float* __restrict__ dw, float* __restrict__ dbias) {
+__device__ __forceinline__ void wgrad_reduce_body(const long bid, const float* __restrict__ slab, const float* __restrict__ bias_slab,
+                                                  int splits, int bias_rows, int taps, int ci, int co, long cip, long cop, int transposed,
+                                                  float* __restrict__ dw, float* __restrict__ dbias, float4 (*red)[16]) {
     constexpr int RPB = 16 / PARTS;
-    __shared__ float4 red[16][16];
     const int c4 = threadIdx.x & 15, part = PARTS == 16 ? threadIdx.x >> 4 : 0, rib = PARTS == 16 ? 0 : threadIdx.x >> 4;
     const int n_tiles = (co + 63) / 64;
     const long rows = (long)taps * ci;
     const long row_blocks = (rows + RPB - 1) / RPB;
-    const long bid = blockIdx.x;
     const bool is_bias = bid >= row_blocks * n_tiles;
     if (is_bias && !dbias) return;
     const int ntile = (int)(is_bias ? bid - row_blocks * n_tiles : bid % n_tiles);
@@ -873,6 +908,49 @@
                 dw[transposed ? (((long)k * co + n + e) * taps + tap) : (((long)(n + e) * ci + k) * taps + tap)] = v[e];
         }
     }
+}
+
+template <int PARTS>
+__global__ __launch_bounds__(256) void wgrad_reduce_kernel(const float* __restrict__ slab, const float* __restrict__ bias_slab,
+                                                           int splits, int bias_rows, int taps, int ci, int co, long cip, long cop,
+                                                           int transposed, float* __restrict__ dw, float* __restrict__ dbias) {
+    __shared__ float4 red[16][16];
+    wgrad_reduce_body<PARTS>(blockIdx.x, slab, bias_slab, splits, bias_rows, taps, ci, co, cip, cop, transposed, dw, dbias, red);
+}
+
+long reduce_blocks(int splits, int taps, int ci, int co_w, bool bias) {
+    const long rows = (long)taps * ci;
+    const int n_tiles = (co_w + 63) / 64;
+    return splits > 16 ? (rows + (bias ? 1 : 0)) * n_tiles : ((rows + 15) / 16 + (bias ? 1 : 0)) * n_tiles;
+}
+
+struct RedLayer {
+    const float* slab;
+    const float* bias_slab;
+    float* dw;
+    float* dbias;
+    long cip, cop;
+    int splits, bias_rows, taps, ci, co, transposed;
+    long first_block;
+};
+constexpr int kRedGroupMax = 40;
+struct RedGroup {
+    int n;
+    RedLayer l[kRedGroupMax];
+};
+
+__global__ __launch_bounds__(256) void wgrad_reduce_grouped_kernel(const RedGroup g) {
+    __shared__ float4 red[16][16];
+    const long b = blockIdx.x;
+    int i = 0;
+    while (i + 1 < g.n && b >= g.l[i + 1].first_block) i++;
+    const RedLayer& r = g.l[i];
+    if (r.splits > 16)
+        wgrad_reduce_body<16>(b - r.first_block, r.slab, r.bias_slab, r.splits, r.bias_rows, r.taps, r.ci, r.co, r.cip, r.cop,
+                              r.transposed, r.dw, r.dbias, red);
+    else
+        wgrad_reduce_body<1>(b - r.first_block, r.slab, r.bias_slab, r.splits, r.bias_rows, r.taps, r.ci, r.co, r.cip, r.cop,
+                             r.transposed, r.dw, r.dbias, red);
 }
 
 int launch_reduce(const float* slab, const float* bias_slab, int splits, int bias_rows, int taps, int ci, int co_w, long cip, long cop,
@@ -1316,20 +1394,125 @@
 unsigned long long* g_wgrad_stamps = nullptr;
 #endif
 
-template <int MODE, int TH, int S, int CIW = 64>
-int launch_rs3(const liso_conv_desc& d, const Rs3Plan& p, hipStream_t st) {
+Rs3Layer rs3_layer(const liso_conv_desc& d, const WgArgs& a) {
+    Rs3Layer l;
+    l.x = a.x;
+    l.in_scale = a.in_scale;
+    l.in_shift = a.in_shift;
+    l.dy = a.dy;
+    l.slab = a.slab;
+    l.bias_slab = a.bias_slab;
+#ifdef LISO_WGRAD_STAMPS
+    l.stamps = nullptr;
+#endif
+    l.hi = d.hi;
+    l.wi = d.wi;
+    l.ci = d.ci;
+    l.x_pix_stride = d.x_pix_stride;
+    l.ho = d.ho;
+    l.wo = d.wo;
+    l.co = d.co;
+    l.dy_pix_stride = a.dy_pix_stride;
+    l.in_relu = d.in_relu;
+    l.wgrad_co = d.wgrad_co;
+    l.w_taps = d.w_taps;
+    l.ci_t = a.ci_t;
+    l.co_t = a.co_t;
+    l.tiles_x = a.tiles_x;
+    l.tiles_y = a.tiles_y;
+    l.n_tiles = a.n_tiles;
+    l.splits = a.splits;
+    l.first_block = 0;
+    for (int t = 0; t < 9; t++) l.tap_w[t] = d.tap_w[t];
+    return l;
+}
+
+template <int MODE, int TH, int S, int CIW, class Args>
+int launch_rs3_args(Args& args, int blocks, int lds, hipStream_t st) {
     static liso_dev::PerDeviceFlag attr_set;
-    if (!liso_dev::lds_opt_in(attr_set, (const void*)conv_wgrad_rs3_kernel<MODE, TH, S, CIW>, 160 * 1024)) return LISO_ELAUNCH;
+    if (!liso_dev::lds_opt_in(attr_set, (const void*)conv_wgrad_rs3_kernel<MODE, TH, S, CIW, Args>, 160 * 1024)) return LISO_ELAUNCH;
 #ifdef LISO_WGRAD_STAMPS
     if (!g_wgrad_stamps && hipMalloc((void**)&g_wgrad_stamps, 4096 * 16 * 8) != hipSuccess) return LISO_ELAUNCH;
     (void)hipMemsetAsync(g_wgrad_stamps, 0, 4096 * 16 * 8, st);
-    Rs3Plan q = p;
-    q.a.stamps = p.blocks <= 4096 ? g_wgrad_stamps : nullptr;
-    conv_wgrad_rs3_kernel<MODE, TH, S, CIW><<<q.blocks, kRsThreads, q.lds, st>>>(d, q.a);
+    if constexpr (std::is_same<Args, Rs3One>::value) {
+        args.l.stamps = blocks <= 4096 ? g_wgrad_stamps : nullptr;
+    } else {
+        for (int i = 0; i < args.n; i++) args.l[i].stamps = blocks <= 4096 ? g_wgrad_stamps : nullptr;
+    }
+#endif
+    conv_wgrad_rs3_kernel<MODE, TH, S, CIW, Args><<<blocks, kRsThreads, lds, st>>>(args);
     return hipGetLastError() == hipSuccess ? LISO_OK : LISO_ELAUNCH;
-#endif
-    conv_wgrad_rs3_kernel<MODE, TH, S, CIW><<<p.blocks, kRsThreads, p.lds, st>>>(d, p.a);
-    return hipGetLastError() == hipSuccess ? LISO_OK : LISO_ELAUNCH;
+}
+
+template <int MODE, int TH, int S, int CIW = 64>
+int launch_rs3(const liso_conv_desc& d, const Rs3Plan& p, hipStream_t st) {
+    Rs3One one;
+    one.l = rs3_layer(d, p.a);
+    return launch_rs3_args<MODE, TH, S, CIW>(one, p.blocks, p.lds, st);
+}
+
+struct GroupItemPlan {
+    Rs3Plan p;
+    int variant;
+    size_t slab_off, bias_off;
+};
+
+long group_tiles() {
+    const char* e = getenv("LISO_WGRAD_GROUP_TILES");
+    return e && atol(e) > 0 ? atol(e) : 0;
+}
+
+bool make_group_plan(const liso_conv_desc& d, GroupItemPlan* g) {
+    if (d.mode != LISO_CONV_BF16 && d.mode != LISO_CONV_F16 && d.mode != LISO_CONV_F32X3) return false;
+    if (d.wgrad_co < 0 || d.wgrad_co > d.co) return false;
+    Rs3Plan& p = g->p;
+    if (!make_rs3_plan(d, &p) || p.a.ci_w != CT) return false;
+    const long cc = (long)p.a.ci_t * p.a.co_t;
+    const long slab_per_part = 9l * p.a.ci_t * CT * p.a.co_t * CT * sizeof(float);
+    const long tiles = group_tiles();
+    long parts = p.a.splits;
+    if (tiles > 0) {
+        const long cap = (24l << 20) / slab_per_part;
+        parts = p.a.n_tiles / tiles;
+        parts = parts > cap ? cap : parts;
+        parts = parts < 1 ? 1 : parts;
+    }
+    p.a.splits = (int)parts;
+    p.blocks = (int)(cc * parts);
+    p.slab_bytes = (size_t)parts * slab_per_part;
+    p.bias_bytes = (size_t)parts * p.a.co_t * CT * sizeof(float);
+    g->variant = d.mode * 64 + p.th * 4 + p.stride;
+    return true;
+}
+
+size_t group_layout(const liso_conv_wgrad_item* items, int n, GroupItemPlan* plans) {
+    size_t o = 0;
+    for (int i = 0; i < n; i++) {
+        if (!items[i].d || !make_group_plan(*items[i].d, &plans[i])) return 0;
+        plans[i].slab_off = o;
+        o += (plans[i].p.slab_bytes + 255) / 256 * 256;
+        plans[i].bias_off = o;
+        o += (plans[i].p.bias_bytes + 255) / 256 * 256;
+    }
+    return o;
+}
+
+template <int MODE, int TH, int S>
+int launch_group_variant(Rs3Group& g, int blocks, int lds, hipStream_t st) {
+    return launch_rs3_args<MODE, TH, S, 64>(g, blocks, lds, st);
+}
+
+int launch_group(int variant, Rs3Group& g, int blocks, int lds, hipStream_t st) {
+    switch (variant) {
+        case LISO_CONV_BF16 * 64 + 8 * 4 + 1: return launch_group_variant<LISO_CONV_BF16, 8, 1>(g, blocks, lds, st);
+        case LISO_CONV_BF16 * 64 + 4 * 4 + 1: return launch_group_variant<LISO_CONV_BF16, 4, 1>(g, blocks, lds, st);
+        case LISO_CONV_BF16 * 64 + 3 * 4 + 2: return launch_group_variant<LISO_CONV_BF16, 3, 2>(g, blocks, lds, st);
+        case LISO_CONV_F16 * 64 + 8 * 4 + 1: return launch_group_variant<LISO_CONV_F16, 8, 1>(g, blocks, lds, st);
+        case LISO_CONV_F16 * 64 + 4 * 4 + 1: return launch_group_variant<LISO_CONV_F16, 4, 1>(g, blocks, lds, st);
+        case LISO_CONV_F16 * 64 + 3 * 4 + 2: return launch_group_variant<LISO_CONV_F16, 3, 2>(g, blocks, lds, st);
+        case LISO_CONV_F32X3 * 64 + 3 * 4 + 1: return launch_group_variant<LISO_CONV_F32X3, 3, 1>(g, blocks, lds, st);
+        default: return LISO_EINVAL;
+    }
 }
 
 }
@@ -1577,6 +1760,92 @@
                          (long)p.a.co_t * CT, transposed, dw, dbias, st);
 }
 
+size_t liso_conv_wgrad_grouped_workspace_bytes(const liso_conv_wgrad_item* items, int n) {
+    if (!items || n < 1 || n > LISO_CONV_WGRAD_GROUP_MAX) return 0;
+    GroupItemPlan plans[LISO_CONV_WGRAD_GROUP_MAX];
+    return group_layout(items, n, plans);
+}
+
+int liso_conv_wgrad_grouped(const liso_conv_wgrad_item* items, int n, void* workspace, size_t workspace_bytes, void* stream) {
+    if (!items || n < 1 || n > LISO_CONV_WGRAD_GROUP_MAX || !workspace) return LISO_EINVAL;
+    GroupItemPlan plans[LISO_CONV_WGRAD_GROUP_MAX];
+    const size_t need = group_layout(items, n, plans);
+    if (need == 0) return LISO_EINVAL;
+    for (int i = 0; i < n; i++) {
+        const liso_conv_wgrad_item& it = items[i];
+        const liso_conv_desc& d = *it.d;
+        const int vec = d.mode == LISO_CONV_F32X3 ? 4 : 8;
+        if (!it.x || !it.dy || !it.dw || (it.in_scale == nullptr) != (it.in_shift == nullptr)) return LISO_EINVAL;
+        if (it.dy_pix_stride % vec || it.dy_pix_stride < d.co || (((uintptr_t)it.x | (uintptr_t)it.dy) & 15)) return LISO_EINVAL;
+    }
+    if (workspace_bytes < need) return LISO_EWORKSPACE;
+    hipStream_t st = (hipStream_t)stream;
+    char* ws = (char*)workspace;
+    bool done[LISO_CONV_WGRAD_GROUP_MAX] = {};
+    for (int i = 0; i < n; i++) {
+        if (done[i]) continue;
+        Rs3Group g;
+        g.n = 0;
+        int blocks = 0, lds = 0;
+        for (int j = i; j <= n; j++) {
+            const bool take = j < n && !done[j] && plans[j].variant == plans[i].variant;
+            if (take) {
+                const liso_conv_wgrad_item& it = items[j];
+                WgArgs& a = plans[j].p.a;
+                a.x = it.x;
+                a.in_scale = it.in_scale;
+                a.in_shift = it.in_shift;
+                a.dy = it.dy;
+                a.dy_pix_stride = it.dy_pix_stride;
+                a.slab = (float*)(ws + plans[j].slab_off);
+                a.bias_slab = it.dbias ? (float*)(ws + plans[j].bias_off) : nullptr;
+                g.l[g.n] = rs3_layer(*it.d, a);
+                g.l[g.n].first_block = blocks;
+                blocks += plans[j].p.blocks;
+                lds = plans[j].p.lds > lds ? plans[j].p.lds : lds;
+                g.n++;
+                done[j] = true;
+            }
+            if (g.n > 0 && (g.n == kRsGroupMax || j == n)) {
+                const int rc = launch_group(plans[i].variant, g, blocks, lds, st);
+                if (rc != LISO_OK) return rc;
+                g.n = 0;
+                blocks = 0;
+                lds = 0;
+            }
+        }
+    }
+    RedGroup r;
+    r.n = 0;
+    long rblocks = 0;
+    for (int i = 0; i < n; i++) {
+        const liso_conv_wgrad_item& it = items[i];
+        const Rs3Plan& p = plans[i].p;
+        RedLayer& l = r.l[r.n++];
+        l.slab = (const float*)(ws + plans[i].slab_off);
+        l.bias_slab = it.dbias ? (const float*)(ws + plans[i].bias_off) : nullptr;
+        l.dw = it.dw;
+        l.dbias = it.dbias;
+        l.cip = (long)p.a.ci_t * CT;
+        l.cop = (long)p.a.co_t * CT;
+        l.splits = p.a.splits;
+        l.bias_rows = p.a.splits;
+        l.taps = 9;
+        l.ci = it.d->ci;
+        l.co = it.d->wgrad_co > 0 ? it.d->wgrad_co : it.d->co;
+        l.transposed = it.transposed;
+        l.first_block = rblocks;
+        rblocks += reduce_blocks(l.splits, 9, l.ci, l.co, it.dbias != nullptr);
+        if (r.n == kRedGroupMax || i == n - 1) {
+            wgrad_reduce_grouped_kernel<<<(int)rblocks, 256, 0, st>>>(r);
+            if (hipGetLastError() != hipSuccess) return LISO_ELAUNCH;
+            r.n = 0;
+            rblocks = 0;
+        }
+    }
+    return LISO_OK;
+}
+
 size_t liso_conv_wgrad_smallci_workspace_bytes(int batch, int h, int w, int co, int k) {
     int nblk, rpb, lds;
     size_t pb, bb;
diff --git a/liso_amd/trainer.py b/liso_amd/trainer.py
--- a/liso_amd/trainer.py
+++ b/liso_amd/trainer.py
@@ -99,7 +99,6 @@
             _MC._sparse_flag(device)
         self.use_graph = bool(use_graph) and device.type == "cuda"
         self._graph, self._graph2, self._graph_sig, self._capture_stream = None, None, None, None
-        self._wgrad_stream = None
         self.fused_loss = (fused_centerpoint.supports(cfg) and device.type == "cuda") if fused_loss is None else fused_loss
         self.net = BoxLearner(cfg).to(device)
         self.net.model.set_compute_dtype(compute_dtype)
@@ -265,8 +264,6 @@
             torch.autograd.graph.set_warn_on_accumulate_grad_stream_mismatch(False)
         if self._capture_stream is None:
             self._capture_stream = side_stream(dev, "flow")
-        if self._wgrad_stream is None and os.environ.get("LISO_WGRAD_SIDE", "0") == "1":
-            self._wgrad_stream = side_stream(dev, "wgrad")
         side = self._capture_stream
         side.wait_stream(torch.cuda.current_stream(dev))
 
@@ -298,11 +295,11 @@
                         total, _, _ = self.loss(None, self._static_targets, canvas=(self._static_bev, self._static_occ))
                     finally:
                         rpn.grad_cut = None
-                    with MC.wgrad_side(self._wgrad_stream):
+                    with MC.wgrad_group():
                         self._backward(total)
                     self._body_loss = total.detach()
                 if cut is not None and part in (None, 2):
-                    with MC.wgrad_side(self._wgrad_stream):
+                    with MC.wgrad_group():
                         cut.finish()
             finally:
                 det_cus.__exit__(None, None, None)
diff --git a/liso_amd/utils/mfma_conv.py b/liso_amd/utils/mfma_conv.py
--- a/liso_amd/utils/mfma_conv.py
+++ b/liso_amd/utils/mfma_conv.py
@@ -183,27 +183,40 @@
         return False
 
 
-_WGRAD_SIDE = None
-
-
-class wgrad_side:
-
-    def __init__(self, stream):
-        self.stream = stream
+_WGRAD_GROUP = None
+
+
+class wgrad_group:
 
     def __enter__(self):
-        global _WGRAD_SIDE
-        self.prev = _WGRAD_SIDE
-        _WGRAD_SIDE = {"stream": self.stream, "keep": [], "used": False} if self.stream is not None else None
+        global _WGRAD_GROUP
+        self.prev = _WGRAD_GROUP
+        on = os.environ.get("LISO_WGRAD_GROUPED", "1") != "0"
+        _WGRAD_GROUP = {"items": [], "keep": [], "flops": 0.0, "bytes": 0.0, "mode": None, "device": None} if on else None
         return self
 
-    def __exit__(self, *exc):
-        global _WGRAD_SIDE
-        st, _WGRAD_SIDE = _WGRAD_SIDE, self.prev
-        if st is not None and st["used"]:
-            torch.cuda.current_stream(st["stream"].device).wait_stream(st["stream"])
-            st["keep"].clear()
+    def __exit__(self, exc_type, *exc):
+        global _WGRAD_GROUP
+        grp, _WGRAD_GROUP = _WGRAD_GROUP, self.prev
+        if grp is not None and grp["items"] and exc_type is None:
+            _launch_wgrad_group(grp)
         return False
+
+
+def _launch_wgrad_group(grp):
+    lib = L.lib()
+    items = grp["items"]
+    for at in range(0, len(items), L.CONV_WGRAD_GROUP_MAX):
+        chunk = items[at:at + L.CONV_WGRAD_GROUP_MAX]
+        arr = (L.ConvWgradItem * len(chunk))(*chunk)
+        nbytes = lib.liso_conv_wgrad_grouped_workspace_bytes(arr, len(chunk))
+        if nbytes == 0:
+            raise RuntimeError("liso_conv_wgrad_grouped: a recorded layer is not covered")
+        ws = torch.empty(nbytes, dtype=torch.uint8, device=grp["device"])
+        with torch.cuda.device(grp["device"]):
+            L.check(L.TIMER.launch(_timer_name(grp["mode"], "wgrad"), lambda: lib.liso_conv_wgrad_grouped(
+                arr, len(chunk), L.ptr(ws), nbytes, L.stream_ptr()), units=grp["flops"] if at == 0 else 0.0,
+                nbytes=grp["bytes"] if at == 0 else 0.0), "conv_wgrad_grouped")
 
 
 class roles_cus:
@@ -417,7 +430,7 @@
 
 
 def conv_wgrad(x, dy, weight_shape, spec, in_scale=None, in_shift=None, in_relu=False, want_bias=True, out_dw=None, out_db=None,
-               co_true=None):
+               co_true=None, defer=False):
     L.require_cuda(x, dy)
     if (x.shape[1] == 4 and x.dtype == torch.float32 and not spec.transposed and spec.stride == 1 and spec.kh == spec.kw and spec.kh in (5, 7)
             and spec.padding == spec.kh // 2 and in_scale is None and tuple(weight_shape[1:]) == (4, spec.kh, spec.kw)
@@ -441,6 +454,19 @@
         d = L.ConvDesc.from_buffer_copy(d)
         d.wgrad_co = co_true
     lib = L.lib()
+    grp = _WGRAD_GROUP
+    if (defer and grp is not None and out_dw is not None and (out_db is not None or not want_bias)
+            and (grp["mode"] in (None, mode)) and (grp["device"] in (None, x.device))):
+        item = L.ConvWgradItem(ctypes.addressof(d), xv.data_ptr(), L.ptr(in_scale) if in_scale is not None else None,
+                               L.ptr(in_shift) if in_shift is not None else None, gv.data_ptr(), gps, int(spec.transposed),
+                               out_dw.data_ptr(), out_db.data_ptr() if want_bias else None)
+        if lib.liso_conv_wgrad_grouped_workspace_bytes(ctypes.byref(item), 1) > 0:
+            grp["items"].append(item)
+            grp["keep"].append((d, xv, gv, in_scale, in_shift, out_dw, out_db))
+            grp["flops"] += _flops(d)
+            grp["bytes"] += _bytes(d, True)
+            grp["mode"], grp["device"] = mode, x.device
+            return out_dw, out_db
     nbytes = lib.liso_conv_wgrad_workspace_bytes(ctypes.byref(d))
     if nbytes == 0:
         return None
@@ -746,19 +772,8 @@
                 res = conv_wgrad_sparse(x_raw, ctx.meta["occupancy"], dy, tuple(weight.shape), spec, want_bias=ctx.meta["has_bias"])
                 tw = None if res is not None else tw
             if res is None:
-                side = _WGRAD_SIDE if (tw is not None and dy.is_cuda) else None
-                if side is not None:
-                    ev = torch.cuda.Event()
-                    ev.record(torch.cuda.current_stream(dy.device))
-                    with torch.cuda.stream(side["stream"]):
-                        side["stream"].wait_event(ev)
-                        res = conv_wgrad(x_raw, dy, tuple(weight.shape), spec, sc, sh, in_relu=fold.relu if fold is not None else False,
-                                         want_bias=ctx.meta["has_bias"], out_dw=tw, out_db=tb, co_true=co_true)
-                    side["keep"].append((x_raw, dy, sc, sh))
-                    side["used"] = True
-                else:
-                    res = conv_wgrad(x_raw, dy, tuple(weight.shape), spec, sc, sh, in_relu=fold.relu if fold is not None else False,
-                                     want_bias=ctx.meta["has_bias"], out_dw=tw, out_db=tb, co_true=co_true)
+                res = conv_wgrad(x_raw, dy, tuple(weight.shape), spec, sc, sh, in_relu=fold.relu if fold is not None else False,
+                                 want_bias=ctx.meta["has_bias"], out_dw=tw, out_db=tb, co_true=co_true, defer=tw is not None)
             if res is None:
                 raise NotImplementedError(f"liso_amd: no device weight-gradient kernel for {tuple(weight.shape)} stride {spec.stride} "
                                           f"on {tuple(x_raw.shape)} {x_raw.dtype}")
```

New measurement: 1013 (median of 6 runs). 1.4% higher.
